# ZYM-PKU/UDiffText

Hardware: AMD Instinct MI355X
Metric: 512x512 50-step denoised images/sec (UDiffText hot path: conditioner + 50 CFG Euler steps + VAE decode) (higher is better)
Workload: dtype bf16; 1 GPU; 512x512, 50 Euler/DDIM(eta 0) steps, CFG 5.0, 9-char labels, noise_iters 0; global batch 4 per step sharded over 1 GPU(s) = 4 images per GPU in micro-batches of 4: every UNet call runs ONE batch of 4 (8 samples with CFG); 3 such batch(es) in flight per GPU on separate launch streams; BASELINE.json configs[1]; global_batch=4, weights=synthetic (name-keyed recipe), 1361.2 M parameters, launch=hipGraph replay of the sampler steps, in_flight=3, batches_per_unet_call=1

## Files before the change

### udifftext_amd/csrc/gemm.hip

```cpp
#include "common.h"
#include <stdio.h>
#include <stdlib.h>
#include <string.h>
#include <atomic>
#include <cmath>

hipError_t udt_lean_launch_gemm(int cfg, const void* lparams, int smem, int G, int geglu, int ln, hipStream_t s);
hipError_t udt_lean_launch_conv3(const void* c3params, hipStream_t s);

namespace {
#include "tile_common.h"

struct GemmParams {
  const uint16_t* a;
  const uint16_t* a2;
  const uint16_t* w;
  const uint16_t* zero;
  const float* bias;
  const uint16_t* res;
  const float* rowvec;
  void* out;
  const float* colscale;
  const float* in_scsh;
  float* colstats;
// ... 587 lines not shown

template <int WGM, int WGN, int TM, int TN, bool GN, bool STATS, bool UPS = false>
hipError_t launch3p(const c3p::CParams& cp, const TilePlan& t, hipStream_t s) {
  constexpr int BN = WGN * TN * 32;
  constexpr int smem = g8::NSTAGE * BN * ROW_BYTES + 2 * c3p::patch_rows(TN, GN) * ROW_BYTES + (GN ? c3p::SCSH_BYTES : 0);
  static_assert(smem <= 160 * 1024, "one workgroup per CU: at most the CU's 160 KiB of LDS");
  static AttrOnce once;
  auto kern = c3p::conv3p_kernel<WGM, WGN, TM, TN, GN, STATS, UPS>;
  hipError_t e = once.ensure(reinterpret_cast<const void*>(kern), smem);
  if (e != hipSuccess) return e;
  hipLaunchKernelGGL(kern, dim3(t.G), dim3(g8::NTHREADS), smem, s, cp);
  return hipGetLastError();
}

struct LeanPlan;
bool lean_stats_probe(const udt_gemm_desc* d, int& rows, int& slots);
int colstats_rows(const udt_gemm_desc* d) {
  if (d->flags & (UDT_GEMM_OUT_F32 | UDT_GEMM_GEGLU | UDT_GEMM_TRANSPOSED)) return 0;
  if ((d->batch > 1) || d->M <= 0 || d->N <= 0 || d->K <= 0 || d->K % BK != 0) return 0;
  int rows = 0, slots = 0;
  if (lean_stats_probe(d, rows, slots)) return rows;
  c3p::Geo ge;
  if (conv3p_geometry(d, ge, d->in_scsh != nullptr)) {
    rows = (d->N % 160 == 0 && d->N % 128 != 0) ? 32 : 64;
    if ((ge.TW * ge.TH) % rows != 0) return 0;
  } else if (use_gemm8(d) && g_rows_epi.load(std::memory_order_relaxed)) {
    rows = (plan_tiles8(d).bn == 160) ? 32 : 64;
  } else {
    return 0;
  }
  const int rpb = d->rows_per_batch > 0 ? d->rows_per_batch : d->M;
  return (rpb % rows == 0) ? rows : 0;
}

int colstats_slots(const udt_gemm_desc* d) {
  const int rows = colstats_rows(d);
  if (rows == 0) return 0;
  int lrows = 0, lslots = 0;
  if (lean_stats_probe(d, lrows, lslots)) return lslots;
  c3p::Geo ge;
  if (conv3p_geometry(d, ge, d->in_scsh != nullptr)) return ge.img_groups * ge.tiles_y * ge.tiles_x * (256 / rows);
  return ((d->M + 255) / 256) * (256 / rows);
}


std::atomic<int> g_lean{-1};
std::atomic<int> g_lean_splitk{-2};
int lean_splitk_knob() {
  int v = g_lean_splitk.load(std::memory_order_relaxed);
  if (v == -2) {
    const char* e = getenv("UDT_LEAN_SPLITK");
    v = e ? atoi(e) : -1;
    g_lean_splitk.store(v, std::memory_order_relaxed);
  }
  return v;
}
std::atomic<int> g_share_splitk{-2};
int share_splitk() {
  int v = g_share_splitk.load(std::memory_order_relaxed);
  if (v == -2) {
    const char* e = getenv("UDT_SHARE_SPLITK");
    v = e ? (atoi(e) != 0) : 1;
    g_share_splitk.store(v, std::memory_order_relaxed);
  }
  return v;
}
int share_of(const udt_gemm_desc* d) { return (share_splitk() && d->cu_share > 1) ? d->cu_share : 1; }
bool lean_stats_enabled() { return true; }

struct LeanPlan {
  int stats_rows = 0;
  int cfg;
  int bm, bn, nw, smem;
  int tiles_m, tiles_n, tiles, nkt, splitk, kt_per, G, n_block;
};

int lean_mode() {
  int v = g_lean.load(std::memory_order_relaxed);
  if (v == -1) {
    const char* e = getenv("UDT_LEAN");
    v = e ? atoi(e) : -2;
    g_lean.store(v, std::memory_order_relaxed);
  }
  return v;
}

std::atomic<int> g_rowres{-2};
bool rowres_on() {
  int v = g_rowres.load(std::memory_order_relaxed);
  if (v == -2) {
    const char* e = getenv("UDT_ROWRES");
    v = e ? (atoi(e) != 0) : 1;
    g_rowres.store(v, std::memory_order_relaxed);
  }
  return v != 0;
}
std::atomic<int> g_lean256_lanes{-2};
bool lean256_under_lanes() {
  int v = g_lean256_lanes.load(std::memory_order_relaxed);
  if (v == -2) {
    const char* e = getenv("UDT_LEAN256_LANES");
    v = e ? (atoi(e) != 0) : 1;
    g_lean256_lanes.store(v, std::memory_order_relaxed);
  }
  return v != 0;
}

std::atomic<int> g_conv_n4{-2};
bool conv_n4_applies(const udt_gemm_desc* d) {
  int v = g_conv_n4.load(std::memory_order_relaxed);
  if (v == -2) {
    const char* e = getenv("UDT_CONV_N4");
    v = e ? (atoi(e) != 0) : 1;
    g_conv_n4.store(v, std::memory_order_relaxed);
  }
  if (!v) return false;
  if (d->flags != (UDT_GEMM_CONV | UDT_GEMM_OUT_F32) || d->ksize != 3 || d->stride != 1 || d->pad_t != 1 || d->pad_l != 1 || d->upsample)
    return false;
  if (d->N != 4 || d->C2 != 0 || d->C1 % 64 != 0 || d->C1 > 512 || d->Hout != d->Hin || d->Wout != d->Win || d->ldo % 4 != 0) return false;
  if (d->residual || d->rowvec || d->in_scsh || d->colstats || d->colscale || d->batch > 1 || d->alpha != 1.0f) return false;
  if ((d->ldw > 0 ? d->ldw : d->K) % 8 != 0 || (d->ldw > 0 && d->ldw < d->K)) return false;
  if (d->K != 9 * d->C1 || (d->lda != 0 && d->lda != d->C1) || d->q8_out || d->q8_scale || d->rowstat_out || d->in_act != 0) return false;
  if ((reinterpret_cast<uintptr_t>(d->a) | reinterpret_cast<uintptr_t>(d->w) | reinterpret_cast<uintptr_t>(d->out)) & 15) return false;
  return true;
}

bool lean_plan(const udt_gemm_desc* d, LeanPlan& t, bool want_stats) {
  const int mode = lean_mode();
  if (mode == 0) return false;
  constexpr int unsupported = UDT_GEMM_OUT_F32 | UDT_GEMM_RELU | UDT_GEMM_TRANSPOSED | UDT_GEMM_SILU_OUT;
  if (d->flags & unsupported) return false;
  const bool conv1 = (d->flags & UDT_GEMM_CONV) != 0;
  if (conv1 && (d->ksize != 1 || d->stride != 1 || d->upsample || d->pad_t != 0 || d->pad_l != 0 || d->Hout != d->Hin ||
                d->Wout != d->Win || d->C1 % BK != 0 || d->C2 % BK != 0 || d->ln_colsum || (d->flags & UDT_GEMM_GEGLU)))
    return false;
  const bool mx8 = (d->flags & UDT_GEMM_MX8) != 0;
  const bool emit = d->q8_out != nullptr;
  if (d->batch > 1 || d->in_scsh || (d->colscale != nullptr) != mx8) return false;
  const bool geglu = (d->flags & UDT_GEMM_GEGLU) != 0;
  const bool ln = d->ln_colsum != nullptr;
  if (want_stats && (geglu || ln || !lean_stats_enabled())) return false;
  if (mx8 || emit) {
    if (conv1 || d->rowvec || mode == 0 || (mode > 0 && mode != 1)) return false;
    if (mx8 && (!d->a_scale || d->K % 128 != 0 || d->lda % 16 != 0 || (d->ldw > 0 && d->ldw % 16 != 0))) return false;
    if (mx8 && ln && (!d->rowstat_in || d->rowstat_in_parts <= 0)) return false;
    if (!mx8 && geglu) return false;
    if (mx8 && geglu && !(ln && emit)) return false;
    if (mx8 && !geglu && ln && emit && d->rowstat_out) return false;
    if (emit && (want_stats || !d->q8_scale || d->ld_q8 % 8 != 0 || d->N % (geglu ? 64 : 32) != 0)) return false;
    if (d->rowstat_out && (!emit || geglu)) return false;
    if (d->q8_fixed_col > 0 && (!emit || geglu || d->q8_fixed_col % 32 != 0 || !(d->q8_fixed_mul > 0.f))) return false;
    if ((reinterpret_cast<uintptr_t>(d->q8_out) | reinterpret_cast<uintptr_t>(d->colscale)) & 15) return false;
  } else if (d->rowstat_out || d->rowstat_in) {
    return false;
  }
  const int KT = mx8 ? 128 : BK;
  if (d->N <= 64 || d->N % 8 != 0 || d->K % KT != 0 || (!conv1 && d->lda % 8 != 0) || (d->ldo % 8 != 0 && d->out)) return false;
  if (d->residual && d->ldr % 8 != 0) return false;
  if (geglu && (d->N % 64 != 0 || d->residual || d->rowvec)) return false;
  const long long ldw = d->ldw > 0 ? d->ldw : d->K;
  const long long lda_eff = conv1 ? (d->C1 > d->C2 ? d->C1 : d->C2) : d->lda;
  if ((long long)d->M * lda_eff * 2 >= (1LL << 31) || (long long)d->N * ldw * 2 >= (1LL << 31)) return false;
  if (d->M >= (1 << 28)) return false;
  if ((reinterpret_cast<uintptr_t>(d->out) | reinterpret_cast<uintptr_t>(d->residual) | reinterpret_cast<uintptr_t>(d->bias) |
       reinterpret_cast<uintptr_t>(d->rowvec) | reinterpret_cast<uintptr_t>(d->ln_colsum)) & 15) return false;
  if (d->rowvec && ((d->ld_rowvec > 0 ? d->ld_rowvec : d->N) % 4 != 0)) return false;
  if (mode > 0 && mode != 1 && mode != 6 && mode != 7) return false;
  if (!mx8 && (!emit || (ln && !geglu && !d->rowstat_out)) && (mode == 7 || (mode < 0 && rowres_on()))) {
    const bool emit_fits = !emit || ((d->q8_fixed_col <= 0 || d->q8_fixed_col % 64 == 0) && (long long)d->M * d->ld_q8 < (1LL << 31) &&
                                     (long long)d->M * (d->out ? d->ldo : 0) * 2 < (1LL << 31) && (long long)((d->N + 127) / 128) * d->M * 4 < (1LL << 31));
    if (ln && !want_stats && d->K == 320 && d->N % 64 == 0 && !d->residual && !d->rowvec && !conv1 && emit_fits &&
        (reinterpret_cast<uintptr_t>(d->a) & 15) == 0) {
      const int tiles_m = (d->M + 255) / 256, chunks = d->N / 64;
      int ns = (device_cus() + tiles_m - 1) / tiles_m;
      if (ns > chunks / 4) ns = chunks / 4;
      const int cmax = geglu ? 20 : 16;
      const int ns_min = (chunks + cmax - 1) / cmax;
      if (ns < ns_min) ns = ns_min;
      const long long wgs = (long long)tiles_m * ns;
      if (ns >= 1 && (mode == 7 || emit || (geglu ? wgs * 4 >= 3LL * device_cus() : wgs >= device_cus()))) {
        t.cfg = 7; t.stats_rows = 0; t.nw = 4; t.bm = 256; t.bn = 64; t.smem = 0;
        t.tiles_m = tiles_m; t.kt_per = (chunks + ns - 1) / ns; t.tiles_n = (chunks + t.kt_per - 1) / t.kt_per;
        t.tiles = t.tiles_m * t.tiles_n; t.nkt = d->K / BK; t.splitk = 1; t.n_block = 1;
        t.G = round_workgroups(t.tiles);
        return true;
      }
    }
    if (mode == 7 || (emit && ln)) return false;
  }
  t.cfg = (mode > 0) ? mode : 1;
  if (!mx8 && !emit) {
  if (!geglu && d->N % 160 == 0 && d->N % 128 != 0 && t.cfg == 1) t.cfg = 5;
  if (mode <= 0 && d->N >= 768 && (long long)((d->M + 255) / 256) * ((d->N + 255) / 256) >= 2LL * device_cus() &&
      (d->cu_share <= 1 || lean256_under_lanes())) t.cfg = 6;
  }
  t.stats_rows = 0;
  if (want_stats) {
    if (t.cfg != 1 && t.cfg != 5) {
      if (mode > 0) return false;
      t.cfg = (d->N % 160 == 0 && d->N % 128 != 0) ? 5 : 1;
    }
    if (mx8) t.cfg = 1;
    t.stats_rows = t.cfg == 1 ? 64 : 32;
    const int rpb = d->rows_per_batch > 0 ? d->rows_per_batch : d->M;
    if (rpb % t.stats_rows != 0) return false;
  }
  switch (t.cfg) {
    case 1: t.nw = 4; t.bm = 128; t.bn = 128; t.smem = 2 * (128 + 128) * ROW_BYTES; break;
    case 5: t.nw = 4; t.bm = 128; t.bn = 160; t.smem = 128 * 160 * 4; break;
    case 6: t.nw = 8; t.bm = 256; t.bn = 256; t.smem = 2 * (256 + 256) * ROW_BYTES; break;
    default: return false;
  }
  {
    const int epi = (t.cfg == 6 ? t.bm * t.bn : t.bm * t.bn * 4) + ((ln && t.cfg != 5) ? t.bm * 8 : 0);
    if (t.smem < epi) t.smem = epi;
  }
  t.tiles_m = (d->M + t.bm - 1) / t.bm;
  t.tiles_n = (d->N + t.bn - 1) / t.bn;
  t.tiles = t.tiles_m * t.tiles_n;
  t.nkt = d->K / KT;
  int slots = device_cus() * ((t.cfg == 1 || t.cfg == 5) ? 2 : 1) / share_of(d);
  if (slots < 1) slots = 1;
  int sk = 1;
  const int knob = lean_splitk_knob();
  if (!ln && t.tiles <= 1023) {
    if (knob > 1) sk = knob;
    else if (knob < 0 && t.tiles * 2 <= slots && t.nkt >= (mx8 ? 20 : 40)) { sk = slots / t.tiles; if (sk > t.nkt / (mx8 ? 8 : 16)) sk = t.nkt / (mx8 ? 8 : 16); }
    if (sk > t.nkt / 4) sk = t.nkt / 4;
    while (sk > 1 && (long long)t.tiles * sk * t.bm * t.bn * 4 > (64LL << 20)) --sk;
    if (sk < 1) sk = 1;
  }
  t.kt_per = (t.nkt + sk - 1) / sk;
  t.splitk = (t.nkt + t.kt_per - 1) / t.kt_per;
  const int units = t.tiles * t.splitk;
  t.G = round_workgroups(units);
  int nb = g_n_block.load(std::memory_order_relaxed);
  if (nb <= 0) nb = (t.tiles_m <= 8) ? t.tiles_n : 8;
  if (nb > t.tiles_n) nb = t.tiles_n;
  t.n_block = nb;
  return true;
}

size_t lean_workspace(const LeanPlan& t) {
  return t.splitk > 1 ? G8_HEADER_BYTES + (size_t)t.tiles * t.splitk * t.bm * t.bn * sizeof(float) : 0;
}

std::atomic<int> g_lean_conv{-1};
std::atomic<int> g_wide_conv{-2};
int wide_conv_mode() {
  int v = g_wide_conv.load(std::memory_order_relaxed);
  if (v == -2) {
    const char* e = getenv("UDT_WIDE_CONV");
    v = e ? atoi(e) : -1;
    g_wide_conv.store(v, std::memory_order_relaxed);
  }
  return v;
}
#ifdef UDT_MEASURE
std::atomic<int> g_lconv_dbg{0};
#endif

std::atomic<int> g_wide_lanes_eff{-2};
double wide_lanes_eff() {
  int v = g_wide_lanes_eff.load(std::memory_order_relaxed);
  if (v == -2) {
    const char* e = getenv("UDT_WIDE_LANES_EFF");
    v = e ? atoi(e) : 70;
    g_wide_lanes_eff.store(v, std::memory_order_relaxed);
  }
  return v / 100.0;
}

int conv_chunk_slices(long long tiles, int slots, int chunks, int knob) {
  long long sk = 1;
  if (tiles <= 1023) {
    if (knob > 1) { sk = knob; if (sk > chunks) sk = chunks; }
    else if (knob < 0 && tiles * 2 <= slots && chunks >= 10) { sk = slots / tiles; if (sk > chunks / 4) sk = chunks / 4; }
    if (sk < 1) sk = 1;
  }
  return (int)sk;
}

bool lean_conv_plan(const udt_gemm_desc* d, lg::C3Params& c, bool want_stats) {
  int on = g_lean_conv.load(std::memory_order_relaxed);
  if (on < 0) {
    const char* e = getenv("UDT_LEAN_CONV");
    on = (e && e[0] == '0') ? 0 : 1;
    g_lean_conv.store(on, std::memory_order_relaxed);
  }
  if (!on || lean_mode() == 0) return false;
  if (d->flags != UDT_GEMM_CONV || d->ksize != 3 || d->stride != 1 || d->pad_t != 1 || d->pad_l != 1) return false;
  if (d->C2 != 0 || d->in_scsh || d->colscale || d->batch > 1) return false;
  if (want_stats && !lean_stats_enabled()) return false;
  if (d->N < 128 || d->N % 8 != 0 || d->C1 <= 0 || d->C1 % 64 != 0) return false;
  if (d->upsample != 0 && d->upsample != 1 && d->upsample != 2) return false;
  const bool phase = d->upsample == 2, ups = d->upsample == 1;
  const int nph = phase ? 4 : 1;
  if (d->Hout != (d->Hin << (d->upsample ? 1 : 0)) || d->Wout != (d->Win << (d->upsample ? 1 : 0))) return false;
  if (phase && d->ldw > 0 && d->ldw < 4 * d->C1) return false;
  const int Ht = phase ? d->Hin : d->Hout, Wt = phase ? d->Win : d->Wout;
  c.bn = 128; c.wgm = 2;
  bool wide = false;
  int wide_slots = device_cus();
  {
    const int wm = wide_conv_mode();
    if (wm != 0 && !ups && d->N % 160 == 0 && Wt % 16 == 0 && Ht % 16 == 0) {
      const int cus = device_cus(), share = d->cu_share > 1 ? d->cu_share : 1;
      wide_slots = cus / share > 0 ? cus / share : 1;
      const long long wt = (long long)(d->M / 256) * (d->N / 160);
      const long long sk = conv_chunk_slices(wt, wide_slots, d->C1 / 64, lean_splitk_knob());
      const long long units = wt * sk;
      const long long rounds = (units + cus - 1) / cus;
      const double eff = units > cus ? (double)units / (double)(rounds * cus) : ((double)units * share >= cus ? 1.0 : (double)units * share / cus);
      wide = (wm > 0) || (sk <= 2 && eff >= ((share >= 3 && share_of(d) >= 3) ? wide_lanes_eff() : 0.85));
    }
  }
  if (wide) { c.geo = phase ? 6 : 3; c.tw = 16; c.th = 16; c.bn = 160; c.wgm = 4; }
  else if (Wt % 16 == 0 && Ht % 8 == 0) { c.geo = ups ? 2 : phase ? 4 : 0; c.tw = 16; c.th = 8; }
  else if (!ups && Wt % 8 == 0 && Ht % 8 == 0) { c.geo = phase ? 5 : 1; c.tw = 8; c.th = 8; }
  else return false;
  if (d->ldo % 8 != 0 || (d->residual && d->ldr % 8 != 0)) return false;
  const long long ldw = d->ldw > 0 ? d->ldw : (phase ? 4LL * d->C1 : (long long)d->K);
  if (ldw % 8 != 0) return false;
  c.w_phase = phase ? (d->stride_w > 0 ? d->stride_w : (long long)d->N * ldw) : 0;
  if (phase && (c.w_phase < (long long)d->N * ldw || c.w_phase % 8 != 0)) return false;
  if ((long long)d->M * d->C1 * 2 >= (1LL << 31) || (long long)d->N * ldw * 2 >= (1LL << 31)) return false;
  if ((reinterpret_cast<uintptr_t>(d->out) | reinterpret_cast<uintptr_t>(d->residual) | reinterpret_cast<uintptr_t>(d->bias) |
       reinterpret_cast<uintptr_t>(d->rowvec)) & 15) return false;
  if (d->rowvec && ((d->ld_rowvec > 0 ? d->ld_rowvec : d->N) % 4 != 0)) return false;
  c.dbg = 0;
#ifdef UDT_MEASURE
  c.dbg = g_lconv_dbg.load(std::memory_order_relaxed);
#endif
  c.N = d->N; c.C = d->C1; c.H = d->Hin; c.W = d->Win; c.B = d->M / (d->Hout * d->Wout);
  c.ldw = (int)ldw; c.ldo = d->ldo; c.ldr = d->ldr; c.ldrv = d->ld_rowvec > 0 ? d->ld_rowvec : d->N;
  c.alpha = d->alpha;
  c.tiles_x = Wt / c.tw; c.tiles_y = Ht / c.th;
  c.tiles_m = c.B * c.tiles_x * c.tiles_y;
  c.tiles_n = (d->N + c.bn - 1) / c.bn;
  c.tiles = c.tiles_m * c.tiles_n;
  c.chunks = c.C / 64;
  const int slots = wide ? wide_slots : (2 * device_cus() / share_of(d) > 0 ? 2 * device_cus() / share_of(d) : 1);
  int sk = conv_chunk_slices((long long)c.tiles * nph, slots, c.chunks, lean_splitk_knob());
  while (sk > 1 && (long long)c.tiles * nph * sk * c.tw * c.th * c.bn * 4 > (64LL << 20)) --sk;
  c.ch_per = (c.chunks + sk - 1) / sk;
  c.splitk = (c.chunks + c.ch_per - 1) / c.ch_per;
  c.G = round_workgroups(c.tiles * nph * c.splitk);
  {
    const double patch = (double)((ups ? c.tw / 2 : c.tw) + 2) * ((ups ? c.th / 2 : c.th) + 2) * c.C * 2.0, wtile = (phase ? 4.0 : 9.0) * c.bn * c.C * 2.0;
    int nb = g_n_block.load(std::memory_order_relaxed);
    if (nb <= 0) nb = (int)(std::sqrt(64.0 * patch / wtile) + 0.5);
    if (nb < 1) nb = 1;
    if (nb > c.tiles_n) nb = c.tiles_n;
    c.n_block = nb;
  }
  c.a_bytes = (unsigned)((long long)c.B * d->Hin * d->Win * d->C1 * 2);
  c.w_bytes = (unsigned)((long long)d->N * ldw * 2);
  c.counters = nullptr; c.slabs = nullptr;
  return true;
}

int lean_conv_phases(const lg::C3Params& c) { return c.geo >= 4 ? 4 : 1; }

size_t lean_conv_workspace(const lg::C3Params& c) {
  return c.splitk > 1 ? G8_HEADER_BYTES + (size_t)c.tiles * lean_conv_phases(c) * c.splitk * c.tw * c.th * c.bn * sizeof(float) : 0;
}

bool lean_stats_probe(const udt_gemm_desc* d, int& rows, int& slots) {
  if (d->in_scsh) return false;
  {
    lg::C3Params c3;
    if (lean_conv_plan(d, c3, true)) {
      rows = c3.tw * c3.th / c3.wgm;
      slots = c3.tiles_m * c3.wgm * lean_conv_phases(c3);
      return true;
    }
  }
  if ((d->flags & UDT_GEMM_CONV) && d->ksize == 3) return false;
  LeanPlan lt;
  if (lean_plan(d, lt, true)) {
    rows = lt.stats_rows;
    slots = lt.tiles_m * (lt.bm / lt.stats_rows);
    return true;
  }
  return false;
}
}

extern "C" int udt_debug_set(const char* key, int32_t value) {
  if (!key) return UDT_ERR_BAD_ARG;
  if (!strcmp(key, "n_block")) { g_n_block.store(value); return UDT_OK; }
  if (!strcmp(key, "rows_epi")) { g_rows_epi.store(value ? 1 : 0); return UDT_OK; }
  if (!strcmp(key, "lean")) { g_lean.store(value < 0 ? -2 : value); return UDT_OK; }
  if (!strcmp(key, "rowres")) { g_rowres.store(value < 0 ? 1 : (value ? 1 : 0)); return UDT_OK; }
  if (!strcmp(key, "wide_lanes_eff")) { g_wide_lanes_eff.store(value < 0 ? -2 : value); return UDT_OK; }
  if (!strcmp(key, "conv_n4")) { g_conv_n4.store(value < 0 ? -2 : (value ? 1 : 0)); return UDT_OK; }
  if (!strcmp(key, "lean256_lanes")) { g_lean256_lanes.store(value < 0 ? -2 : (value ? 1 : 0)); return UDT_OK; }
  if (!strcmp(key, "lean_splitk")) { g_lean_splitk.store(value); return UDT_OK; }
  if (!strcmp(key, "share_splitk")) { g_share_splitk.store(value < 0 ? -2 : (value ? 1 : 0)); return UDT_OK; }
  if (!strcmp(key, "lean_conv")) { g_lean_conv.store(value < 0 ? -1 : (value ? 1 : 0)); return UDT_OK; }
  if (!strcmp(key, "wide_conv")) { g_wide_conv.store(value < 0 ? -1 : (value ? 1 : 0)); return UDT_OK; }
#ifdef UDT_MEASURE
  if (!strcmp(key, "lconv_dbg")) { g_lconv_dbg.store(value); return UDT_OK; }
  static const struct { const char* k; int bit; } bits[] = {{"no_xchg", 28}, {"no_epi", 27}, {"no_store", 26}, {"no_res", 25},
                                                            {"no_bias", 24}, {"no_fast", 22}};
  for (const auto& b : bits)
    if (!strcmp(key, b.k)) {
      int cur = g_dbg_bits.load();
      g_dbg_bits.store((cur & ~(1 << b.bit)) | (value ? (1 << b.bit) : 0));
      return UDT_OK;
    }
#endif
  return UDT_ERR_BAD_ARG;
}

extern "C" int udt_check_async_error(void* workspace, size_t workspace_bytes, void* stream) {
  if (!workspace || workspace_bytes < G8_HEADER_BYTES) return UDT_ERR_BAD_ARG;
  hipStream_t s = reinterpret_cast<hipStream_t>(stream);
  int err = 0;
  hipError_t e = hipMemcpyAsync(&err, reinterpret_cast<int*>(workspace) + 1023, sizeof(int), hipMemcpyDeviceToHost, s);
  if (e == hipSuccess) e = hipStreamSynchronize(s);
  if (e != hipSuccess) return udt_set_hip_error(e);
  if (err == 0) return UDT_OK;
  e = hipMemsetAsync(workspace, 0, G8_HEADER_BYTES, s);
  if (e == hipSuccess) e = hipStreamSynchronize(s);
  if (e != hipSuccess) return udt_set_hip_error(e);
  return UDT_ERR_ASYNC;
}

extern "C" int32_t udt_gemm_colstats_rows(const udt_gemm_desc* d) { return d ? colstats_rows(d) : 0; }
extern "C" int32_t udt_gemm_colstats_slots(const udt_gemm_desc* d) { return d ? colstats_slots(d) : 0; }
extern "C" int32_t udt_gemm_q8_ok(const udt_gemm_desc* d) {
  if (!d || !d->q8_out || d->M <= 0 || d->N <= 0 || d->K <= 0) return 0;
  LeanPlan lt;
  return lean_plan(d, lt, d->colstats != nullptr) ? 1 : 0;
}

extern "C" int32_t udt_gemm_rowstat_parts(const udt_gemm_desc* d) {
  if (!d || d->M <= 0 || d->N <= 0 || d->K <= 0) return 0;
  udt_gemm_desc t = *d;
  alignas(16) static const uint64_t probe_dst[2] = {0, 0};
  if (!t.q8_out) { t.q8_out = const_cast<uint64_t*>(probe_dst); t.q8_scale = const_cast<uint64_t*>(probe_dst); if (t.ld_q8 <= 0) t.ld_q8 = (t.N + 15) / 16 * 16; }
  LeanPlan lt;
  if (!lean_plan(&t, lt, false) || lt.cfg != 1 || (d->flags & UDT_GEMM_GEGLU)) return 0;
  return (d->N + 63) / 64;
}
extern "C" int32_t udt_gemm_in_scsh_ok(const udt_gemm_desc* d) {
  if (!d || d->K <= 0 || d->K % BK != 0) return 0;
  c3p::Geo ge;
  return conv3p_geometry(d, ge, true) ? 1 : 0;
}

extern "C" int32_t udt_gemm_up4_ok(const udt_gemm_desc* d) {
  if (!d || d->upsample != 2) return 0;
  lg::C3Params c3;
  return lean_conv_plan(d, c3, d->colstats != nullptr) ? 1 : 0;
}

extern "C" int udt_gn_silu_conv3x3_fwd(const udt_gemm_desc* d, void* workspace, size_t workspace_bytes, void* stream) {
  if (!d || !(d->flags & UDT_GEMM_CONV) || d->ksize != 3 || d->stride != 1 || d->pad_t != 1 || d->pad_l != 1 || !d->in_scsh)
    return UDT_ERR_BAD_ARG;
  return udt_gemm(d, workspace, workspace_bytes, stream);
}

extern "C" int udt_ln_gemm_fwd(const udt_gemm_desc* d, void* workspace, size_t workspace_bytes, void* stream) {
  if (!d || !d->ln_colsum || !d->bias || !(d->ln_eps > 0.f)) return UDT_ERR_BAD_ARG;
  LeanPlan lt;
  if (!lean_plan(d, lt, false)) return UDT_ERR_BAD_SHAPE;
  return udt_gemm(d, workspace, workspace_bytes, stream);
}

extern "C" size_t udt_gemm_workspace_bytes(const udt_gemm_desc* d) {
  if (!d || d->K <= 0 || d->M <= 0 || d->N <= 0 || d->K % k_tile(d) != 0) return 0;
  if (conv_n4_applies(d)) return 0;
  {
    LeanPlan lt;
    if (lean_plan(d, lt, d->colstats != nullptr)) return lean_workspace(lt);
    lg::C3Params c3;
    if (lean_conv_plan(d, c3, d->colstats != nullptr)) return lean_conv_workspace(c3);
  }
  {
    c3p::Geo ge;
    if (conv3p_geometry(d, ge, d->in_scsh != nullptr)) {
      TilePlan t3 = plan_tiles3p(d, ge);
      if (!t3.fixup) return 0;
      return G8_HEADER_BYTES + (size_t)t3.G * t3.bm * t3.bn * sizeof(float);
    }
  }
  if (use_gemm8(d)) {
    TilePlan t8 = plan_tiles8(d);
    if (!t8.fixup) return 0;
    return G8_HEADER_BYTES + (size_t)t8.G * t8.bm * t8.bn * sizeof(float);
  }
  TilePlan t = plan_tiles(d);
  if (t.bm != 256 || !t.fixup) return 0;
  return G8_HEADER_BYTES + (size_t)t.G * 2 * SLAB_FLOATS * sizeof(float);
}

extern "C" int udt_gemm(const udt_gemm_desc* d, void* workspace, size_t workspace_bytes, void* stream) {
  if (!d || !d->a || !d->w) return UDT_ERR_BAD_ARG;
  if (d->M <= 0 || d->N <= 0 || d->K <= 0) return UDT_ERR_BAD_SHAPE;
  if (d->K % k_tile(d) != 0) return UDT_ERR_BAD_SHAPE;
  if (d->N % 4 != 0) return UDT_ERR_BAD_SHAPE;
  const bool mx8 = (d->flags & UDT_GEMM_MX8) != 0;
  if (mx8 || d->q8_out || d->rowstat_out || d->rowstat_in) {
    LeanPlan lt8;
    if (!lean_plan(d, lt8, d->colstats != nullptr)) return UDT_ERR_BAD_ARG;
  } else if (d->colscale) {
    return UDT_ERR_BAD_ARG;
  }
  const bool conv = (d->flags & UDT_GEMM_CONV) != 0;
  const bool trans = (d->flags & UDT_GEMM_TRANSPOSED) != 0;
  const int batch = d->batch > 0 ? d->batch : 1;
  if (conv) {
    if (d->ksize != 1 && d->ksize != 3) return UDT_ERR_BAD_SHAPE;
    if (d->C1 <= 0 || d->C1 % BK != 0 || d->C2 % BK != 0) return UDT_ERR_BAD_SHAPE;
    if (d->C2 > 0 && !d->a2) return UDT_ERR_BAD_ARG;
    if (d->K != d->ksize * d->ksize * (d->C1 + d->C2)) return UDT_ERR_BAD_SHAPE;
    if (d->Hout <= 0 || d->Wout <= 0 || d->M % (d->Hout * d->Wout) != 0) return UDT_ERR_BAD_SHAPE;
    if (d->stride != 1 && d->stride != 2) return UDT_ERR_BAD_SHAPE;
    if (trans || batch != 1) return UDT_ERR_BAD_ARG;
  } else {
    if (d->lda < d->K || d->lda % 8 != 0) return UDT_ERR_BAD_SHAPE;
  }
  if (!d->out && !d->q8_out) return UDT_ERR_BAD_ARG;
  if (trans) {
    if (d->rows_per_batch <= 0 || d->rows_per_batch % 4 != 0 || d->M % d->rows_per_batch != 0)
      return UDT_ERR_BAD_SHAPE;
    if (d->flags & (UDT_GEMM_OUT_F32 | UDT_GEMM_GEGLU | UDT_GEMM_RELU | UDT_GEMM_SILU_OUT)) return UDT_ERR_BAD_ARG;
    if (d->residual || d->rowvec || batch != 1) return UDT_ERR_BAD_ARG;
  } else {
    if (d->ldo % 4 != 0) return UDT_ERR_BAD_SHAPE;
    if (d->residual && d->ldr % 4 != 0) return UDT_ERR_BAD_SHAPE;
  }
  if (d->flags & UDT_GEMM_GEGLU) {
    if (d->N % 64 != 0 || (d->flags & UDT_GEMM_OUT_F32) || d->residual || d->rowvec) return UDT_ERR_BAD_ARG;
  }
  if (d->rowvec && d->rows_per_batch <= 0) return UDT_ERR_BAD_ARG;

  hipStream_t s = reinterpret_cast<hipStream_t>(stream);
  if (conv_n4_applies(d)) {
    cn4::Params cp;
    cp.a = reinterpret_cast<const uint16_t*>(d->a); cp.w = reinterpret_cast<const uint16_t*>(d->w); cp.bias = d->bias;
    cp.out = reinterpret_cast<float*>(d->out);
    cp.B = d->M / (d->Hout * d->Wout); cp.H = d->Hin; cp.W = d->Win; cp.C = d->C1;
    cp.ldw = d->ldw > 0 ? d->ldw : d->K; cp.ldo = d->ldo;
    cp.tiles_x = (d->Win + 7) / 8; cp.tiles_y = (d->Hin + 7) / 8;
    const size_t smem = (size_t)100 * (d->C1 + 8) * 2 + (size_t)4 * 9 * d->C1 * 2;
    static AttrOnce once;
    hipError_t ea = once.ensure(reinterpret_cast<const void*>(cn4::conv3x3_n4_kernel), 100 * (512 + 8) * 2 + 4 * 9 * 512 * 2);
    if (ea != hipSuccess) return udt_set_hip_error(ea);
    UdtProfScope profn(0, s);
    if (profn.rec) {
      char tag[96];
      snprintf(tag, sizeof(tag), "conv_n4 M=%d N=%d K=%d %dx%d", d->M, d->N, d->K, d->Hin, d->Win);
      udt_prof_tag(profn.rec, tag);
    }
    hipLaunchKernelGGL(cn4::conv3x3_n4_kernel, dim3((unsigned)(cp.B * cp.tiles_x * cp.tiles_y)), dim3(256), smem, s, cp);
    UDT_CHECK_LAUNCH();
    return UDT_OK;
  }
  TilePlan t = plan_tiles(d);

  GemmParams p;
  p.a = reinterpret_cast<const uint16_t*>(d->a);
  p.a2 = reinterpret_cast<const uint16_t*>(d->a2);
  p.w = reinterpret_cast<const uint16_t*>(d->w);
  p.zero = udt_zero_page();
  if (!p.zero) return UDT_ERR_HIP;
  p.bias = d->bias;
  p.res = reinterpret_cast<const uint16_t*>(d->residual);
  p.rowvec = d->rowvec;
  p.out = d->out;
  p.colscale = d->colscale;
  p.in_scsh = d->in_scsh;
  p.in_act = d->in_act;
  p.colstats = d->colstats;
  p.slabs = nullptr;
  if (d->colstats && colstats_rows(d) == 0) return UDT_ERR_BAD_ARG;
  if (d->in_scsh && !udt_gemm_in_scsh_ok(d)) return UDT_ERR_BAD_ARG;
  if (d->in_act != 0 && d->in_act != 1) return UDT_ERR_BAD_ARG;
  p.M = d->M; p.N = d->N; p.K = d->K;
  p.lda = d->lda; p.ldo = d->ldo; p.ldr = d->ldr;
  p.ldw = d->ldw > 0 ? d->ldw : d->K;
  if (d->upsample == 2) {
    if (!udt_gemm_up4_ok(d)) return UDT_ERR_BAD_SHAPE;
  } else if (p.ldw < d->K || p.ldw % 8 != 0) return UDT_ERR_BAD_SHAPE;
  if (mx8 && d->lda < d->K) return UDT_ERR_BAD_SHAPE;
  p.sA = d->stride_a; p.sW = d->stride_w; p.sO = d->stride_out; p.sR = d->stride_res;
  p.Hin = d->Hin; p.Win = d->Win; p.C1 = d->C1; p.C2 = d->C2; p.Hout = d->Hout; p.Wout = d->Wout;
  p.ksz = d->ksize; p.stride = d->stride; p.pad_t = d->pad_t; p.pad_l = d->pad_l; p.ups = d->upsample ? 1 : 0;
  p.rows_per_batch = d->rows_per_batch > 0 ? d->rows_per_batch : d->M;
  p.ldrv = d->ld_rowvec > 0 ? d->ld_rowvec : d->N;
// ... 206 lines not shown
```

### udifftext_amd/csrc/lean.h

```cpp
#pragma once

namespace lg {

using g8::wait_vm;
UDT_DEVINL void raw_barrier() {
  asm volatile("s_waitcnt lgkmcnt(0)" ::: "memory");
  __builtin_amdgcn_s_barrier();
  asm volatile("" ::: "memory");
}
using g8::buf_lds16;
using g8::OOB;

typedef __attribute__((ext_vector_type(2))) __bf16 bf2_t;
UDT_DEVINL float dot2_bf16(uint32_t a, uint32_t b, float c) {
  return __builtin_amdgcn_fdot2_f32_bf16(__builtin_bit_cast(bf2_t, a), __builtin_bit_cast(bf2_t, b), c, false);
}

template <int CPR, int RPI>
UDT_DEVINL void wave_colstats(char* wl, int lane, const float (&cs)[8], const float (&cq)[8], float* dst, bool col_ok) {
#pragma unroll
  for (int h = 0; h < 2; ++h) {
    f32x4 a = {cs[4 * h + 0], cs[4 * h + 1], cs[4 * h + 2], cs[4 * h + 3]};
    f32x4 b = {cq[4 * h + 0], cq[4 * h + 1], cq[4 * h + 2], cq[4 * h + 3]};
    *reinterpret_cast<f32x4*>(wl + lane * 64 + h * 16) = a;
    *reinterpret_cast<f32x4*>(wl + lane * 64 + 32 + h * 16) = b;
  }
  asm volatile("s_waitcnt lgkmcnt(0)" ::: "memory");
  if (lane < CPR && col_ok) {
    float ts[8], tq[8];
#pragma unroll
    for (int j = 0; j < 8; ++j) ts[j] = tq[j] = 0.f;
#pragma unroll
    for (int r = 0; r < RPI; ++r) {
      const char* src = wl + (r * CPR + lane) * 64;
#pragma unroll
      for (int h = 0; h < 2; ++h) {
        const f32x4 a = *reinterpret_cast<const f32x4*>(src + h * 16);
        const f32x4 b = *reinterpret_cast<const f32x4*>(src + 32 + h * 16);
#pragma unroll
        for (int e = 0; e < 4; ++e) { ts[4 * h + e] += a[e]; tq[4 * h + e] += b[e]; }
      }
    }
#pragma unroll
    for (int h = 0; h < 4; ++h) {
      f32x4 v = {ts[2 * h], tq[2 * h], ts[2 * h + 1], tq[2 * h + 1]};
      *reinterpret_cast<f32x4*>(dst + h * 4) = v;
    }
  }
}

template <int NW, int WGM, int WGN, int TM, int TN, int NST, bool GEGLU, bool LN, int TMB = TM, bool STATS = false, bool FP8 = false,
          bool EMIT = false>
__global__ void __launch_bounds__(NW * 64, 2) lgemm_kernel(const LParams p) {
  static_assert(!STATS || (!GEGLU && !LN), "statistics-emitting epilogue: plain linears / 1x1 convolutions");
  static_assert(!FP8 || NST == 2, "the fp8 loop is written for the two-stage ring");
  static_assert(!EMIT || (TN * 4) % 4 == 0, "a 32-column block = 4 lanes of the row layout");
  constexpr int EB = FP8 ? 1 : 2;
  static_assert(TM % TMB == 0, "epilogue passes of TMB row tiles");
  static_assert(WGM * WGN == NW, "wave grid");
  static_assert(!GEGLU || TN == 2, "GEGLU pairs the two 32-column tiles of a wave");
  constexpr int BM = WGM * TM * 32, BN = WGN * TN * 32;
  constexpr int A_BYTES = BM * ROW_BYTES, B_BYTES = BN * ROW_BYTES, STAGE_BYTES = A_BYTES + B_BYTES;
  constexpr int A_PIECES = BM / 8, B_PIECES = BN / 8;
  constexpr int A_INSTR = (A_PIECES + NW - 1) / NW, B_INSTR = (B_PIECES + NW - 1) / NW;
  constexpr int LPT = A_INSTR + B_INSTR;
  constexpr int WROWS = TM * 32, WCOLS = TN * 32;
  constexpr int EROW = WCOLS * 4;
  constexpr int EPI_WAVE = TMB * 32 * EROW;
  extern __shared__ __attribute__((aligned(16))) char smem[];

  const int tid = threadIdx.x;
  const int wave = __builtin_amdgcn_readfirstlane(tid >> 6);
  const int lane = tid & 63;
  const int l31 = lane & 31;
  const int hi = lane >> 5;
  const int l3 = lane >> 3;
  const int pslot = lane & 7;
  const int wm = wave / WGN;
  const int wn = wave - wm * WGN;
  const int row0 = wm * WROWS;
  const int col0 = wn * WCOLS;
  const int swz = (l31 >> 1) & 7;

  const int unit = range_index(blockIdx.x, p.G);
  if (unit >= p.tiles * p.splitk) return;
  const int tile = unit / p.splitk;
  const int slice = unit - tile * p.splitk;
  int m0, n0;
  {
    const int per_block = p.tiles_m * p.n_block;
    const int blk = tile / per_block;
    const int r = tile - blk * per_block;
    int nbw = p.tiles_n - blk * p.n_block;
    if (nbw > p.n_block) nbw = p.n_block;
    const int tmi = r / nbw;
    m0 = tmi * BM;
    n0 = (blk * p.n_block + (r - tmi * nbw)) * BN;
  }
  const int kt0 = slice * p.kt_per;
  int kt1 = kt0 + p.kt_per;
  if (kt1 > p.nkt) kt1 = p.nkt;
  const int nk = kt1 - kt0;
  auto kreal = [&](int i) { return kt0 + i; };
  const __amdgpu_buffer_rsrc_t rsrc_a = __builtin_amdgcn_make_buffer_rsrc(const_cast<uint16_t*>(p.a), 0, p.a_bytes, 0x00020000);
  const __amdgpu_buffer_rsrc_t rsrc_w = __builtin_amdgcn_make_buffer_rsrc(const_cast<uint16_t*>(p.w), 0, p.w_bytes, 0x00020000);
  const __amdgpu_buffer_rsrc_t rsrc_a2 =
      __builtin_amdgcn_make_buffer_rsrc(const_cast<uint16_t*>(p.a2 ? p.a2 : p.a), 0, p.a2 ? p.a2_bytes : 0u, 0x00020000);
  unsigned a_voff[A_INSTR], a2_voff[A_INSTR], w_voff[B_INSTR];
  int a_piece[A_INSTR], w_piece[B_INSTR];
#pragma unroll
  for (int i = 0; i < A_INSTR; ++i) {
    int idx = wave + NW * i;
    while (idx >= A_PIECES) idx -= NW;
    a_piece[i] = idx;
    const int row = idx * 8 + l3;
    const int koff = (pslot ^ ((row >> 1) & 7)) * 8;
    const int m = m0 + row;
    a_voff[i] = (m < p.M) ? (unsigned)((long long)m * p.lda * EB + koff * 2) : OOB;
    a2_voff[i] = (m < p.M) ? (unsigned)(((long long)m * p.lda2 + koff) * 2) : OOB;
  }
#pragma unroll
  for (int i = 0; i < B_INSTR; ++i) {
    int idx = wave + NW * i;
    while (idx >= B_PIECES) idx -= NW;
    w_piece[i] = idx;
    const int row = idx * 8 + l3;
    const int koff = (pslot ^ ((row >> 1) & 7)) * 8;
    const int n = n0 + row;
    w_voff[i] = (n < p.N) ? (unsigned)((long long)n * p.ldw * EB + koff * 2) : OOB;
  }
  auto stage = [&](int st, int kt) {
    char* abuf = smem + st * STAGE_BYTES;
    char* bbuf = abuf + A_BYTES;
    if (kt < p.kt_split) {
#pragma unroll
      for (int i = 0; i < A_INSTR; ++i) buf_lds16(rsrc_a, abuf + a_piece[i] * 1024, a_voff[i], kt * ROW_BYTES);
    } else {
#pragma unroll
      for (int i = 0; i < A_INSTR; ++i) buf_lds16(rsrc_a2, abuf + a_piece[i] * 1024, a2_voff[i], (kt - p.kt_split) * ROW_BYTES);
    }
#pragma unroll
    for (int i = 0; i < B_INSTR; ++i) buf_lds16(rsrc_w, bbuf + w_piece[i] * 1024, w_voff[i], kt * ROW_BYTES);
  };

#pragma unroll
  for (int s = 0; s < NST - 1; ++s)
    if (s < nk) stage(s, kreal(s));
  const uint32_t* asp[TM];
  uint32_t asc_nxt[TM];
  if constexpr (FP8) {
#pragma unroll
    for (int tm = 0; tm < TM; ++tm) {
      int m = m0 + row0 + tm * 32 + l31;
      if (m >= p.M) m = p.M - 1;
      asp[tm] = p.a_scale + m;
      asc_nxt[tm] = (nk > 0) ? asp[tm][(long long)kreal(0) * p.M] : 0x7f7f7f7fu;
    }
  }

  f32x16 acc[TM][TN];
#pragma unroll
  for (int i = 0; i < TM; ++i)
#pragma unroll
    for (int j = 0; j < TN; ++j)
#pragma unroll
      for (int r = 0; r < 16; ++r) acc[i][j][r] = 0.f;
  float rs[TM], rq[TM];
#pragma unroll
  for (int i = 0; i < TM; ++i) rs[i] = rq[i] = 0.f;
  if constexpr (LN && FP8) {
    if (WGN == 1 || wn == 0) {
#pragma unroll
      for (int tm = 0; tm < TM; ++tm) {
        int m = m0 + row0 + tm * 32 + l31;
        if (m >= p.M) m = p.M - 1;
        const f32x2* sp = reinterpret_cast<const f32x2*>(p.rowstat_in) + m;
        for (int pp = hi; pp < p.rowstat_in_parts; pp += 2) {
          const f32x2 v = sp[(long long)pp * p.M];
          rs[tm] += v[0];
          rq[tm] += v[1];
        }
      }
    }
  }

  const int a_frag_row = (row0 + l31) * ROW_BYTES;
  const int b_frag_row = (col0 + l31) * ROW_BYTES;
  int st = 0;
  for (int kt = 0; kt < nk; ++kt) {
    if (NST > 2 && kt + NST - 2 < nk) wait_vm<LPT*(NST > 2 ? NST - 2 : 0)>();
    else wait_vm<0>();
    raw_barrier();
    int asc[TM];
    if constexpr (FP8) {
#pragma unroll
      for (int tm = 0; tm < TM; ++tm) asc[tm] = (int)(asc_nxt[tm] >> (8 * hi));
    }
    if (kt + NST - 1 < nk) {
      int s2 = st + NST - 1;
      if (s2 >= NST) s2 -= NST;
      const int kn = kreal(kt + NST - 1);
      stage(s2, kn);
      if constexpr (FP8) {
#pragma unroll
        for (int tm = 0; tm < TM; ++tm) asc_nxt[tm] = asp[tm][(long long)kn * p.M];
      }
    }
    const char* abuf = smem + st * STAGE_BYTES;
    const char* bbuf = abuf + A_BYTES;
    if constexpr (FP8) {
      i32x8_t xf[2][TM], wf[2][TN];
#pragma unroll
      for (int ks = 0; ks < 2; ++ks) {
        const int slot0 = ((ks * 4 + hi) ^ swz) << 4, slot1 = ((ks * 4 + 2 + hi) ^ swz) << 4;
#pragma unroll
        for (int t = 0; t < TM; ++t)
          xf[ks][t] = lds_read_frag32(abuf + a_frag_row + t * 32 * ROW_BYTES + slot0, abuf + a_frag_row + t * 32 * ROW_BYTES + slot1);
#pragma unroll
        for (int t = 0; t < TN; ++t)
          wf[ks][t] = lds_read_frag32(bbuf + b_frag_row + t * 32 * ROW_BYTES + slot0, bbuf + b_frag_row + t * 32 * ROW_BYTES + slot1);
      }
#pragma unroll
      for (int tm = 0; tm < TM; ++tm)
#pragma unroll
        for (int tn = 0; tn < TN; ++tn) acc[tm][tn] = mfma32_mx8<0>(wf[0][tn], xf[0][tm], acc[tm][tn], asc[tm]);
#pragma unroll
      for (int tm = 0; tm < TM; ++tm)
#pragma unroll
        for (int tn = 0; tn < TN; ++tn) acc[tm][tn] = mfma32_mx8<2>(wf[1][tn], xf[1][tm], acc[tm][tn], asc[tm]);
      if constexpr (TM * TN <= 5) {
        __builtin_amdgcn_sched_group_barrier(0x100, 4 * (TM + TN), 0);
        __builtin_amdgcn_sched_group_barrier(0x008, 2 * TM * TN, 0);
      }
    } else {
    bf16x8_t xf[4][TM], wf[4][TN];
#pragma unroll
    for (int ks = 0; ks < 4; ++ks) {
      const int slot = ((ks * 2 + hi) ^ swz) << 4;
#pragma unroll
      for (int t = 0; t < TM; ++t) xf[ks][t] = lds_read_frag(abuf + a_frag_row + t * 32 * ROW_BYTES + slot);
#pragma unroll
      for (int t = 0; t < TN; ++t) wf[ks][t] = lds_read_frag(bbuf + b_frag_row + t * 32 * ROW_BYTES + slot);
    }
#pragma unroll
    for (int ks = 0; ks < 4; ++ks) {
#pragma unroll
      for (int tm = 0; tm < TM; ++tm)
#pragma unroll
        for (int tn = 0; tn < TN; ++tn) acc[tm][tn] = mfma32(wf[ks][tn], xf[ks][tm], acc[tm][tn]);
      if constexpr (LN) {
        if (wn == 0) {
#pragma unroll
          for (int tm = 0; tm < TM; ++tm) {
            const u32x4 v = __builtin_bit_cast(u32x4, xf[ks][tm]);
#pragma unroll
            for (int j = 0; j < 4; ++j) {
              rs[tm] = dot2_bf16(v[j], 0x3f803f80u, rs[tm]);
              rq[tm] = dot2_bf16(v[j], v[j], rq[tm]);
            }
          }
        }
      }
    }
    if constexpr (TM * TN <= 5) {
      __builtin_amdgcn_sched_group_barrier(0x100, 4 * (TM + TN), 0);
      __builtin_amdgcn_sched_group_barrier(0x008, 4 * TM * TN, 0);
    }
    }
    st = st + 1;
    if (st >= NST) st = 0;
  }
  raw_barrier();

  if (p.splitk > 1) {
    f32x4* slab = reinterpret_cast<f32x4*>(p.slabs + (long long)unit * (BM * BN));
#pragma unroll
    for (int tm = 0; tm < TM; ++tm)
#pragma unroll
      for (int tn = 0; tn < TN; ++tn)
#pragma unroll
        for (int q = 0; q < 4; ++q) {
          f32x4 v = {acc[tm][tn][q * 4 + 0], acc[tm][tn][q * 4 + 1], acc[tm][tn][q * 4 + 2], acc[tm][tn][q * 4 + 3]};
          store16_sc1(slab + ((tm * TN + tn) * 4 + q) * (NW * 64) + tid, v);
        }
    asm volatile("s_waitcnt vmcnt(0)" ::: "memory");
    __syncthreads();
    int* const bcast = reinterpret_cast<int*>(smem);
    if (tid == 0) {
      const int t = __hip_atomic_fetch_add(p.counters + tile, 1, __ATOMIC_RELAXED, __HIP_MEMORY_SCOPE_AGENT);
      const int last = (t == p.splitk - 1) ? 1 : 0;
      if (last) {
        __builtin_amdgcn_fence(__ATOMIC_ACQUIRE, "agent");
        __hip_atomic_store(p.counters + tile, 0, __ATOMIC_RELAXED, __HIP_MEMORY_SCOPE_AGENT);
      }
      *bcast = last;
    }
    __syncthreads();
    const bool last = *bcast != 0;
    __syncthreads();
    if (!last) return;
#pragma unroll
    for (int i = 0; i < TM; ++i)
#pragma unroll
      for (int j = 0; j < TN; ++j)
#pragma unroll
        for (int r = 0; r < 16; ++r) acc[i][j][r] = 0.f;
    for (int s = 0; s < p.splitk; ++s) {
      const f32x4* sl = reinterpret_cast<const f32x4*>(p.slabs + ((long long)tile * p.splitk + s) * (BM * BN));
#pragma unroll
      for (int tm = 0; tm < TM; ++tm)
#pragma unroll
        for (int tn = 0; tn < TN; ++tn)
#pragma unroll
          for (int q = 0; q < 4; ++q) {
            const f32x4 v = sl[((tm * TN + tn) * 4 + q) * (NW * 64) + tid];
#pragma unroll
            for (int r = 0; r < 4; ++r) acc[tm][tn][q * 4 + r] += v[r];
          }
    }
  }

  float ln_mean[TM], ln_rstd[TM];
#pragma unroll
  for (int tm = 0; tm < TM; ++tm) ln_mean[tm] = 0.f, ln_rstd[tm] = 1.f;
  if constexpr (LN) {
    float* const rst = reinterpret_cast<float*>(smem + NW * EPI_WAVE);
    if (WGN == 1 || wn == 0) {
#pragma unroll
      for (int tm = 0; tm < TM; ++tm) {
        const float s = xor32_sum(rs[tm]), q = xor32_sum(rq[tm]);
        const float mean = s / (float)p.K;
        const float var = fmaxf(q / (float)p.K - mean * mean, 0.f);
        ln_mean[tm] = mean;
        ln_rstd[tm] = __builtin_amdgcn_rsqf(var + p.ln_eps);
        if constexpr (WGN > 1) {
          if (hi == 0) {
            f32x2 o = {ln_mean[tm], ln_rstd[tm]};
            *reinterpret_cast<f32x2*>(rst + (row0 + tm * 32 + l31) * 2) = o;
          }
        }
      }
    }
    if constexpr (WGN > 1) __syncthreads();
  }
  auto row_stats = [&](int row, float& mean, float& rstd) {
    if constexpr (WGN == 1) {
      mean = __shfl(ln_mean[0], row & 31);
      rstd = __shfl(ln_rstd[0], row & 31);
#pragma unroll
      for (int tm = 1; tm < TM; ++tm) {
        const float m2 = __shfl(ln_mean[tm], row & 31), r2 = __shfl(ln_rstd[tm], row & 31);
        if ((row >> 5) == tm) mean = m2, rstd = r2;
      }
    } else {
      const f32x2 ms = *reinterpret_cast<const f32x2*>(reinterpret_cast<const float*>(smem + NW * EPI_WAVE) + (row0 + row) * 2);
      mean = ms[0];
      rstd = ms[1];
    }
  };

  if constexpr (GEGLU) {
    if constexpr (LN && WGN > 1) {
      if (wn != 0) {
        const float* rst = reinterpret_cast<const float*>(smem + NW * EPI_WAVE);
#pragma unroll
        for (int tm = 0; tm < TM; ++tm) {
          const f32x2 ms = *reinterpret_cast<const f32x2*>(rst + (row0 + tm * 32 + l31) * 2);
          ln_mean[tm] = ms[0];
          ln_rstd[tm] = ms[1];
        }
      }
    }
    char* const wb = smem + wave * (WROWS * 64);
#pragma unroll
    for (int q = 0; q < 4; ++q) {
      const int n = n0 + col0 + q * 8 + hi * 4;
      f32x4 bx = {0.f, 0.f, 0.f, 0.f}, bg = bx, sx = bx, sg = bx;
      f32x4 wx = {1.f, 1.f, 1.f, 1.f}, wg = wx;
      if (n < p.N) {
        if constexpr (FP8) {
          wx = *reinterpret_cast<const f32x4*>(p.colscale + n);
          wg = *reinterpret_cast<const f32x4*>(p.colscale + n + 32);
        }
        if (p.bias) {
          bx = *reinterpret_cast<const f32x4*>(p.bias + n);
          bg = *reinterpret_cast<const f32x4*>(p.bias + n + 32);
        }
        if constexpr (LN) {
          sx = *reinterpret_cast<const f32x4*>(p.ln_s + n);
          sg = *reinterpret_cast<const f32x4*>(p.ln_s + n + 32);
        }
      }
#pragma unroll
      for (int r = 0; r < 4; ++r) bx[r] *= GEGLU_XS, bg[r] *= GEGLU_GS;
#pragma unroll
      for (int tm = 0; tm < TM; ++tm) {
        const int row = tm * 32 + l31;
        const float xm = ln_rstd[tm] * p.alpha * GEGLU_XS, gm = ln_rstd[tm] * p.alpha * GEGLU_GS;
        const float xa = -ln_mean[tm] * xm, ga = -ln_mean[tm] * gm;
        float o[4];
#pragma unroll
        for (int r = 0; r < 4; ++r) {
          float x, g;
// ... 21 lines not shown
      const int m = m0 + row0 + row;
      const u32x4 v = *reinterpret_cast<const u32x4*>(wb + row * 64 + ((ch ^ (row & 3)) << 4));
      if constexpr (EMIT) {
        const float f[8] = {bf16_lo(v[0]), bf16_hi(v[0]), bf16_lo(v[1]), bf16_hi(v[1]), bf16_lo(v[2]), bf16_hi(v[2]), bf16_lo(v[3]), bf16_hi(v[3])};
        uint32_t sb;
        const u32x2 q8 = mx8_quant_row8(f, sb);
        if (m < p.M && col_ok) {
          *reinterpret_cast<u32x2*>(p.q8_out + (long long)m * p.ld_q8 + n_out) = q8;
          if (ch == 0) reinterpret_cast<uint8_t*>(p.q8_scale)[((long long)(n_out >> 7) * p.M + m) * 4 + ((n_out >> 5) & 3)] = (uint8_t)sb;
          if (p.out) *reinterpret_cast<u32x4*>(p.out + (long long)m * p.ldo + n_out) = v;
        }
      } else {
        if (m < p.M && col_ok) *reinterpret_cast<u32x4*>(p.out + (long long)m * p.ldo + n_out) = v;
      }
    }
  } else {
    char* const wl = smem + wave * EPI_WAVE;
    constexpr int PROWS = TMB * 32;
    constexpr int CPR = TN * 4;
    constexpr int RPI = 64 / CPR;
    constexpr int NIT = (PROWS + RPI - 1) / RPI;
    const int rl = lane / CPR;
    const int c8 = lane - rl * CPR;
    const int n = n0 + col0 + c8 * 8;
    const bool col_ok = (rl < RPI) && (n < p.N);
    f32x4 b0 = {0.f, 0.f, 0.f, 0.f}, b1 = b0, s0 = b0, s1 = b0;
    if (p.bias && col_ok) {
      b0 = *reinterpret_cast<const f32x4*>(p.bias + n);
      b1 = *reinterpret_cast<const f32x4*>(p.bias + n + 4);
    }
    if constexpr (LN) {
      if (col_ok) {
        s0 = *reinterpret_cast<const f32x4*>(p.ln_s + n);
        s1 = *reinterpret_cast<const f32x4*>(p.ln_s + n + 4);
      }
    }
    f32x4 w0 = {1.f, 1.f, 1.f, 1.f}, w1 = w0;
    if constexpr (FP8) {
      if (col_ok) {
        w0 = *reinterpret_cast<const f32x4*>(p.colscale + n);
        w1 = *reinterpret_cast<const f32x4*>(p.colscale + n + 4);
      }
    }
    float cs[8], cq[8];
#pragma unroll
    for (int j = 0; j < 8; ++j) cs[j] = cq[j] = 0.f;
#pragma unroll
    for (int pass = 0; pass < TM / TMB; ++pass) {
      const int prow0 = pass * PROWS;
      u32x4 rv[NIT];
      if (p.res) {
#pragma unroll
        for (int i = 0; i < NIT; ++i) {
          const int row = i * RPI + rl;
          const int m = m0 + row0 + prow0 + row;
          u32x4 z = {0u, 0u, 0u, 0u};
          rv[i] = z;
          if (col_ok && row < PROWS && m < p.M) rv[i] = *reinterpret_cast<const u32x4*>(p.res + (long long)m * p.ldr + n);
        }
      }
#pragma unroll
      for (int tb = 0; tb < TMB; ++tb) {
        const int row = tb * 32 + l31;
#pragma unroll
        for (int tn = 0; tn < TN; ++tn)
#pragma unroll
          for (int q = 0; q < 4; ++q) {
            const int chunk = (tn * 8 + q * 2 + hi) ^ (row & 7);
            const f32x16& a16 = acc[pass * TMB + tb][tn];
            f32x4 v = {a16[q * 4 + 0], a16[q * 4 + 1], a16[q * 4 + 2], a16[q * 4 + 3]};
            *reinterpret_cast<f32x4*>(wl + row * EROW + chunk * 16) = v;
          }
      }
#pragma unroll
      for (int i = 0; i < NIT; ++i) {
        const int row = i * RPI + rl;
        const int m = m0 + row0 + prow0 + row;
        const bool ok = col_ok && row < PROWS && m < p.M;
        const int rr = row < PROWS ? row : 0;
        const char* rp = wl + rr * EROW;
        const int sw = rr & 7;
        const f32x4 v0 = *reinterpret_cast<const f32x4*>(rp + (((2 * c8) ^ sw) << 4));
        const f32x4 v1 = *reinterpret_cast<const f32x4*>(rp + (((2 * c8 + 1) ^ sw) << 4));
        float o[8];
#pragma unroll
        for (int j = 0; j < 4; ++j) {
          o[j] = v0[j];
          o[4 + j] = v1[j];
        }
        if constexpr (FP8) {
#pragma unroll
          for (int j = 0; j < 4; ++j) o[j] *= w0[j], o[4 + j] *= w1[j];
        }
        if constexpr (LN) {
          float mean, rstd;
          row_stats(prow0 + rr, mean, rstd);
#pragma unroll
          for (int j = 0; j < 4; ++j) {
            o[j] = rstd * (o[j] - mean * s0[j]);
            o[4 + j] = rstd * (o[4 + j] - mean * s1[j]);
          }
        }
#pragma unroll
        for (int j = 0; j < 4; ++j) {
          o[j] = o[j] * p.alpha + b0[j];
          o[4 + j] = o[4 + j] * p.alpha + b1[j];
        }
        if (p.rowvec && ok) {
          const float* rvp = p.rowvec + (long long)(m / p.rows_per_batch) * p.ldrv + n;
          const f32x4 r0 = *reinterpret_cast<const f32x4*>(rvp);
          const f32x4 r1 = *reinterpret_cast<const f32x4*>(rvp + 4);
#pragma unroll
          for (int j = 0; j < 4; ++j) {
            o[j] += r0[j];
            o[4 + j] += r1[j];
          }
        }
        if (p.res) {
#pragma unroll
          for (int j = 0; j < 4; ++j) {
            o[2 * j] += bf16_lo(rv[i][j]);
            o[2 * j + 1] += bf16_hi(rv[i][j]);
          }
        }
        if constexpr (EMIT) {
          {
            const u32x4 rb = {pack_bf16x2(o[0], o[1]), pack_bf16x2(o[2], o[3]), pack_bf16x2(o[4], o[5]), pack_bf16x2(o[6], o[7])};
#pragma unroll
            for (int j = 0; j < 4; ++j) o[2 * j] = bf16_lo(rb[j]), o[2 * j + 1] = bf16_hi(rb[j]);
          }
          uint32_t sb;
          u32x2 q8 = mx8_quant_row8(o, sb);
          if (n >= p.q8_fixed_col) {
            q8 = e4m3_fixed_row8(o, p.q8_fixed_mul);
            sb = 127u;
          }
          float ps = 0.f, pq = 0.f;
          if (p.rowstat_out) {
            static_assert(CPR == 8 || CPR == 16, "row statistics: 64- or 128-column wave blocks");
#pragma unroll
            for (int j = 0; j < 8; ++j) ps += o[j], pq += o[j] * o[j];
            ps = dpp_add<0xB1>(ps); pq = dpp_add<0xB1>(pq);
            ps = dpp_add<0x4E>(ps); pq = dpp_add<0x4E>(pq);
            ps = dpp_add<0x141>(ps); pq = dpp_add<0x141>(pq);
            if constexpr (CPR == 16) { ps = dpp_add<0x140>(ps); pq = dpp_add<0x140>(pq); }
          }
          if (ok) {
            *reinterpret_cast<u32x2*>(p.q8_out + (long long)m * p.ld_q8 + n) = q8;
            if ((c8 & 3) == 0) reinterpret_cast<uint8_t*>(p.q8_scale)[((long long)(n >> 7) * p.M + m) * 4 + ((n >> 5) & 3)] = (uint8_t)sb;
            if (p.rowstat_out && c8 == 0) {
              f32x2 st2 = {ps, pq};
              reinterpret_cast<f32x2*>(p.rowstat_out)[(long long)((n0 + col0) / WCOLS) * p.M + m] = st2;
            }
          }
        }
        if (ok) {
          u32x4 pk = {pack_bf16x2(o[0], o[1]), pack_bf16x2(o[2], o[3]), pack_bf16x2(o[4], o[5]), pack_bf16x2(o[6], o[7])};
          if (!EMIT || p.out) *reinterpret_cast<u32x4*>(p.out + (long long)m * p.ldo + n) = pk;
          if constexpr (STATS) {
#pragma unroll
            for (int j = 0; j < 4; ++j) {
              const float a = bf16_lo(pk[j]), bb = bf16_hi(pk[j]);
              cs[2 * j] += a; cq[2 * j] += a * a;
              cs[2 * j + 1] += bb; cq[2 * j + 1] += bb * bb;
            }
          }
        }
      }
    }
    if constexpr (STATS) {
      const int slot = (m0 + row0) / WROWS;
      wave_colstats<CPR, RPI>(wl, lane, cs, cq, p.colstats + ((long long)slot * p.N + n) * 2, col_ok);
    }
  }
}


template <int MAXN>
UDT_DEVINL void wait_vm_upto(int n) {
  if constexpr (MAXN == 0) wait_vm<0>();
  else {
    if (n >= MAXN) wait_vm<MAXN>();
    else wait_vm_upto<MAXN - 1>(n);
  }
}

template <int TW, int TH, bool UPS>
struct C3Geo {
  static constexpr int PX = TW * TH;
  static constexpr int TM = PX / 64;
  static constexpr int PW = (UPS ? TW / 2 : TW) + 2, PH = (UPS ? TH / 2 : TH) + 2;
  static constexpr int PROWS = PW * PH;
  static constexpr int PIECES = (PROWS + 7) / 8;
  static constexpr int PATCH_BYTES = PIECES * 1024;
  static constexpr int W_BYTES = 128 * ROW_BYTES;
  static constexpr int NRING = (3 * W_BYTES + 2 * PATCH_BYTES <= 80 * 1024) ? 3 : 2;
  static constexpr int RING = NRING * W_BYTES + 2 * PATCH_BYTES;
  static constexpr int STAGING = 4 * TM * 32 * 256;
  static constexpr int SMEM = RING > STAGING ? RING : STAGING;
  static_assert(PX == 128 || PX == 64, "128 or 64 output pixels per workgroup");
  static_assert(SMEM <= 80 * 1024, "two workgroups per CU");
};

template <int TW, int TH, bool UPS, bool STATS = false, bool PHASE = false>
__global__ void __launch_bounds__(256, 2) lconv3_kernel(const C3Params p) {
  static_assert(!(UPS && PHASE), "the phase form runs on the low-resolution geometries");
  using Geo = C3Geo<TW, TH, UPS>;
  constexpr int NT = PHASE ? 4 : 9;
  constexpr int NW = 4, TM = Geo::TM, TN = 2, BN = 128, BMPX = Geo::PX;
  constexpr int C3_PW = Geo::PW, C3_PROWS = Geo::PROWS, C3_PIECES = Geo::PIECES, C3_PATCH_BYTES = Geo::PATCH_BYTES;
  constexpr int C3_W_BYTES = Geo::W_BYTES, C3_TW = TW, C3_TH = TH;
  constexpr int WROWS = TM * 32;
  constexpr int WP = 4;
  constexpr int PP = (C3_PIECES + NW - 1) / NW;
  constexpr int EROW = 64 * 4;
  extern __shared__ __attribute__((aligned(16))) char smem[];
  char* const wring = smem;
  constexpr int NR = Geo::NRING;
  char* const patches = smem + NR * C3_W_BYTES;

  const int tid = threadIdx.x;
  const int wave = __builtin_amdgcn_readfirstlane(tid >> 6);
  const int lane = tid & 63;
  const int l31 = lane & 31;
  const int hi = lane >> 5;
  const int l3 = lane >> 3;
  const int pslot = lane & 7;
  const int wm = wave >> 1, wn = wave & 1;
  const int row0 = wm * WROWS, col0 = wn * 64;
  const int swz_w = (l31 >> 1) & 7;
  const int w_frag_row = (col0 + l31) * ROW_BYTES;

  const int unit = range_index(blockIdx.x, p.G);
  if (unit >= p.tiles * p.splitk * (PHASE ? 4 : 1)) return;
  const int phase = PHASE ? unit / (p.tiles * p.splitk) : 0;
  const int pha = phase >> 1, phb = phase & 1;
  const int ptile = unit / p.splitk;
  const int slice = unit - ptile * p.splitk;
  const int tile = ptile - phase * p.tiles;
  int tile_m, n0;
  {
    const int per_block = p.tiles_m * p.n_block;
    const int blk = tile / per_block;
    const int r = tile - blk * per_block;
    int nbw = p.tiles_n - blk * p.n_block;
    if (nbw > p.n_block) nbw = p.n_block;
    tile_m = r / nbw;
    n0 = (blk * p.n_block + (r - tile_m * nbw)) * BN;
  }
  const int per_img = p.tiles_x * p.tiles_y;
  const int b = tile_m / per_img;
  const int rt = tile_m - b * per_img;
  const int ty = rt / p.tiles_x;
  const int y0 = ty * C3_TH, x0 = (rt - ty * p.tiles_x) * C3_TW;
  const int c0 = slice * p.ch_per;
  int c1 = c0 + p.ch_per;
  if (c1 > p.chunks) c1 = p.chunks;

  const __amdgpu_buffer_rsrc_t rsrc_a = __builtin_amdgcn_make_buffer_rsrc(const_cast<uint16_t*>(p.a), 0, p.a_bytes, 0x00020000);
  const __amdgpu_buffer_rsrc_t rsrc_w =
      __builtin_amdgcn_make_buffer_rsrc(const_cast<uint16_t*>(p.w) + (PHASE ? (long long)phase * p.w_phase : 0LL), 0, p.w_bytes, 0x00020000);
  auto patch_swz = [](int prow, int yy) { return ((prow - 2 * yy) >> 1) & 7; };
  unsigned w_voff[WP], p_voff[PP];
  int p_piece[PP];
#pragma unroll
  for (int i = 0; i < WP; ++i) {
    const int row = (wave + NW * i) * 8 + l3;
    const int kw = (pslot ^ ((row >> 1) & 7)) * 8;
    const int n = n0 + row;
    w_voff[i] = (n < p.N) ? (unsigned)(((long long)n * p.ldw + kw) * 2) : OOB;
  }
#pragma unroll
  for (int i = 0; i < PP; ++i) {
    int idx = wave + NW * i;
    while (idx >= C3_PIECES) idx -= NW;
    p_piece[i] = idx;
    const int prow = idx * 8 + l3;
    const int yy = prow / C3_PW;
    const int xx = prow - yy * C3_PW;
    const int gy = (UPS ? (y0 >> 1) : y0) + yy - 1, gx = (UPS ? (x0 >> 1) : x0) + xx - 1;
    const bool ok = (prow < C3_PROWS) && ((unsigned)gy < (unsigned)p.H) && ((unsigned)gx < (unsigned)p.W);
    const int koff = (pslot ^ patch_swz(prow, yy)) * 8;
    p_voff[i] = ok ? (unsigned)(((((long long)b * p.H + gy) * p.W + gx) * p.C + koff) * 2) : OOB;
  }
  int a_prow[TM], a_py[TM];
#pragma unroll
  for (int tm = 0; tm < TM; ++tm) {
    const int ml = row0 + tm * 32 + l31;
    const int py = ml / TW, px = ml - py * TW;
    a_py[tm] = PHASE ? py + pha : py;
    a_prow[tm] = UPS ? (py | (px << 16)) : PHASE ? ((py + pha) * C3_PW + px + phb) : (py * C3_PW + px);
  }
  auto issue_w = [&](int st, int c, int tap) {
    const int soff = (tap * p.C + c * 64) * 2;
    char* wbuf = wring + st * C3_W_BYTES;
#pragma unroll
    for (int i = 0; i < WP; ++i) buf_lds16(rsrc_w, wbuf + (wave + NW * i) * 1024, w_voff[i], soff);
  };
  auto issue_patch = [&](int c) {
    char* pbuf = patches + (c & 1) * C3_PATCH_BYTES;
#pragma unroll
    for (int i = 0; i < PP; ++i) buf_lds16(rsrc_a, pbuf + p_piece[i] * 1024, p_voff[i], c * 128);
  };

  f32x16 acc[TM][TN];
#pragma unroll
// ... 217 lines not shown
```

### udifftext_amd/csrc/lean.hip

```cpp
#include "common.h"
#include <stdio.h>
#include <stdlib.h>
#include <atomic>

namespace {
#include "tile_common.h"
#include "lean_params.h"
#include "lean.h"
#include "wide.h"
#include "rowres.h"

template <int NW, int WGM, int WGN, int TM, int TN, int NST, int TMB = TM>
hipError_t launch_lean(const lg::LParams& lp, int smem, int G, bool geglu, bool ln, hipStream_t s) {
  static AttrOnce once[5];
  const void* fn;
  const bool stats = lp.colstats != nullptr;
  if constexpr (NW == 4 && NST == 2) {
    if (stats) {
      fn = (const void*)lg::lgemm_kernel<NW, WGM, WGN, TM, TN, NST, false, false, TMB, true>;
      hipError_t e = once[4].ensure(fn, smem);
      if (e != hipSuccess) return e;
      void* args[] = {const_cast<lg::LParams*>(&lp)};
      return hipLaunchKernel(fn, dim3(G), dim3(NW * 64), args, smem, s);
    }
  }
  if (stats) return hipErrorInvalidValue;
  if constexpr (TN == 2) {
    fn = geglu ? (ln ? (const void*)lg::lgemm_kernel<NW, WGM, WGN, TM, TN, NST, true, true, TMB> : (const void*)lg::lgemm_kernel<NW, WGM, WGN, TM, TN, NST, true, false, TMB>)
               : (ln ? (const void*)lg::lgemm_kernel<NW, WGM, WGN, TM, TN, NST, false, true, TMB> : (const void*)lg::lgemm_kernel<NW, WGM, WGN, TM, TN, NST, false, false, TMB>);
  } else {
    fn = ln ? (const void*)lg::lgemm_kernel<NW, WGM, WGN, TM, TN, NST, false, true, TMB> : (const void*)lg::lgemm_kernel<NW, WGM, WGN, TM, TN, NST, false, false, TMB>;
  }
  hipError_t e = once[(geglu ? 2 : 0) + (ln ? 1 : 0)].ensure(fn, smem);
  if (e != hipSuccess) return e;
  void* args[] = {const_cast<lg::LParams*>(&lp)};
  return hipLaunchKernel(fn, dim3(G), dim3(NW * 64), args, smem, s);
}

template <bool GEGLU, bool LN, bool STATS, bool FP8, bool EMIT>
hipError_t launch_lean_mx8_k(const lg::LParams& lp, int smem, int G, hipStream_t s) {
  static AttrOnce once;
  const void* fn = (const void*)lg::lgemm_kernel<4, 2, 2, 2, 2, 2, GEGLU, LN, 2, STATS, FP8, EMIT>;
  hipError_t e = once.ensure(fn, smem);
  if (e != hipSuccess) return e;
  void* args[] = {const_cast<lg::LParams*>(&lp)};
  return hipLaunchKernel(fn, dim3(G), dim3(256), args, smem, s);
}
hipError_t launch_lean_mx8(const lg::LParams& lp, int smem, int G, bool geglu, bool ln, bool fp8, bool emit, hipStream_t s) {
  const bool stats = lp.colstats != nullptr;
  if (!fp8) {
    if (emit && !geglu && !ln && !stats) return launch_lean_mx8_k<false, false, false, false, true>(lp, smem, G, s);
    return hipErrorInvalidValue;
  }
  if (geglu) return (ln && emit && !stats) ? launch_lean_mx8_k<true, true, false, true, true>(lp, smem, G, s) : hipErrorInvalidValue;
  if (ln) return stats ? hipErrorInvalidValue
                 : emit ? launch_lean_mx8_k<false, true, false, true, true>(lp, smem, G, s)
                        : launch_lean_mx8_k<false, true, false, true, false>(lp, smem, G, s);
  if (stats) return emit ? hipErrorInvalidValue : launch_lean_mx8_k<false, false, true, true, false>(lp, smem, G, s);
  return emit ? launch_lean_mx8_k<false, false, false, true, true>(lp, smem, G, s) : launch_lean_mx8_k<false, false, false, true, false>(lp, smem, G, s);
}

template <int TW, int TH, bool UPS, bool STATS, bool PHASE>
hipError_t launch_lconv3s(const lg::C3Params& c3, hipStream_t s) {
  static AttrOnce once;
  constexpr int smem = lg::C3Geo<TW, TH, UPS>::SMEM;
  hipError_t e = once.ensure(reinterpret_cast<const void*>(lg::lconv3_kernel<TW, TH, UPS, STATS, PHASE>), smem);
  if (e != hipSuccess) return e;
  hipLaunchKernelGGL((lg::lconv3_kernel<TW, TH, UPS, STATS, PHASE>), dim3(c3.G), dim3(256), smem, s, c3);
  return hipGetLastError();
}
template <int TW, int TH, bool UPS, bool PHASE = false>
hipError_t launch_lconv3(const lg::C3Params& c3, hipStream_t s) {
  return c3.colstats ? launch_lconv3s<TW, TH, UPS, true, PHASE>(c3, s) : launch_lconv3s<TW, TH, UPS, false, PHASE>(c3, s);
}

template <bool STATS, bool PHASE>
hipError_t launch_wconv3s(const lg::C3Params& c3, hipStream_t s) {
  static AttrOnce once;
  constexpr int smem = wd::WGeo::SMEM;
  hipError_t e = once.ensure(reinterpret_cast<const void*>(wd::wconv3_kernel<STATS, PHASE>), smem);
  if (e != hipSuccess) return e;
  hipLaunchKernelGGL((wd::wconv3_kernel<STATS, PHASE>), dim3(c3.G), dim3(256), smem, s, c3);
  return hipGetLastError();
}
template <int KT, bool GEGLU, bool EMIT = false>
hipError_t launch_rowres(const lg::LParams& lp, int G, hipStream_t s) {
  static AttrOnce once;
  constexpr int smem = rr::RGeo<KT, GEGLU>::SMEM;
  hipError_t e = once.ensure(reinterpret_cast<const void*>(rr::rgemm_kernel<KT, GEGLU, EMIT>), smem);
  if (e != hipSuccess) return e;
  hipLaunchKernelGGL((rr::rgemm_kernel<KT, GEGLU, EMIT>), dim3(G), dim3(256), smem, s, lp);
  return hipGetLastError();
}

template <bool PHASE>
hipError_t launch_wconv3(const lg::C3Params& c3, hipStream_t s) {
  return c3.colstats ? launch_wconv3s<true, PHASE>(c3, s) : launch_wconv3s<false, PHASE>(c3, s);
}

}

hipError_t udt_lean_launch_gemm(int cfg, const void* lparams, int smem, int G, int geglu, int ln, hipStream_t s) {
  const lg::LParams& lp = *static_cast<const lg::LParams*>(lparams);
  const bool fp8 = lp.a_scale != nullptr, emit = lp.q8_out != nullptr;
  if (cfg == 7 && emit && !fp8 && !geglu && ln && lp.K == 320) return launch_rowres<5, false, true>(lp, G, s);
  if (fp8 || emit) return cfg == 1 ? launch_lean_mx8(lp, smem, G, geglu != 0, ln != 0, fp8, emit, s) : hipErrorInvalidValue;
  switch (cfg) {
    case 1: return launch_lean<4, 2, 2, 2, 2, 2>(lp, smem, G, geglu != 0, ln != 0, s);
    case 6: return launch_lean<8, 2, 4, 4, 2, 2, 1>(lp, smem, G, geglu != 0, ln != 0, s);
    case 5: return geglu ? hipErrorInvalidValue : launch_lean<4, 4, 1, 1, 5, 2>(lp, smem, G, false, ln != 0, s);
    case 7:
      if (!ln || lp.K != 320) return hipErrorInvalidValue;
      return geglu ? launch_rowres<5, true>(lp, G, s) : launch_rowres<5, false>(lp, G, s);
    default: return hipErrorInvalidValue;
  }
}

hipError_t udt_lean_launch_conv3(const void* c3params, hipStream_t s) {
  const lg::C3Params& c3 = *static_cast<const lg::C3Params*>(c3params);
  return c3.geo == 3 ? launch_wconv3<false>(c3, s) : c3.geo == 6 ? launch_wconv3<true>(c3, s) : c3.geo == 2 ? launch_lconv3<16, 8, true>(c3, s)
         : c3.geo == 4 ? launch_lconv3<16, 8, false, true>(c3, s) : c3.geo == 5 ? launch_lconv3<8, 8, false, true>(c3, s)
         : c3.geo == 1 ? launch_lconv3<8, 8, false>(c3, s) : launch_lconv3<16, 8, false>(c3, s);
}
```

### udifftext_amd/csrc/tattn.hip

```cpp
#include "common.h"
#include <stdio.h>
#include <stdlib.h>

namespace {

constexpr int TA_THREADS = 512;
constexpr int TA_WAVES = TA_THREADS / 64;

struct TattnParams {
  const uint16_t* x;
  uint16_t* out;
  const uint16_t* A;
  const float* sc;
  const uint16_t* BmT;
  const float* bias;
  const uint16_t* zero;
  int M, C, hp, n_tok, zero_samples;
  int nsplit;
  float eps;
  uint8_t* q8_out;
  uint32_t* q8_scale;
  float* rowstat_out;
};

UDT_DEVINL f32x16 zero16() {
  f32x16 z;
#pragma unroll
  for (int r = 0; r < 16; ++r) z[r] = 0.f;
  return z;
}

template <int TT, int NKT, int NKS, bool Q8 = false>
__global__ void __launch_bounds__(TA_THREADS) tattn_fused_kernel(const TattnParams p) {
  extern __shared__ __attribute__((aligned(16))) char smem[];
  constexpr int C = NKT * 64, hp = NKS * 16;
  constexpr int nkt = NKT;
  constexpr int TA_AHEAD = NKT <= 10 ? NKT : 8;
  char* const xs = smem;
  float* const stats = reinterpret_cast<float*>(smem + (size_t)nkt * TT * 128);
  const int prs = hp * 2 + 16;
  char* const pl = reinterpret_cast<char*>(stats + TT * 2);
  const int tid = threadIdx.x;
  const int wave = __builtin_amdgcn_readfirstlane(tid >> 6);
  const int lane = tid & 63;
  const int l31 = lane & 31, hi = lane >> 5;
  const long long tok0 = (long long)blockIdx.x * TT;
  const int b = (int)(tok0 / p.n_tok);
  const uint16_t* xg = p.x + tok0 * C;
  uint16_t* og = p.out + tok0 * C;
  float* const rst = reinterpret_cast<float*>(pl + (size_t)TT * prs);
  const int ct_lo = (int)blockIdx.y * (C >> 5) / p.nsplit, ct_hi = ((int)blockIdx.y + 1) * (C >> 5) / p.nsplit;
  auto q8_row_stats = [&]() {
    __syncthreads();
    if (tid < TT && tok0 + tid < p.M) {
      float s = 0.f, q = 0.f;
      for (int ct = ct_lo; ct < ct_hi; ++ct) {
        const f32x2 v = *reinterpret_cast<const f32x2*>(rst + ((size_t)tid * (C >> 5) + ct) * 2);
        s += v[0];
        q += v[1];
      }
      f32x2 o = {s, q};
      reinterpret_cast<f32x2*>(p.rowstat_out)[(long long)blockIdx.y * p.M + tok0 + tid] = o;
    }
  };


  const uint16_t* Ab = p.A + (long long)b * hp * C;
  constexpr int jt = hp >> 5;
  constexpr int tiles1 = jt * (TT / 32);
  bf16x8_t ar[TA_AHEAD][4];
  const bool live = b >= p.zero_samples;
  if (live && wave < tiles1) {
    const uint16_t* arow = Ab + (long long)(wave / (TT / 32)) * (32 * C) + lane * 8;
#pragma unroll
    for (int u = 0; u < TA_AHEAD; ++u)
#pragma unroll
      for (int ks = 0; ks < 4; ++ks) ar[u][ks] = *reinterpret_cast<const bf16x8_t*>(arow + (u * 4 + ks) * 512);
  }

  {
    const int pieces = nkt * (TT / 8);
    const int l3 = lane >> 3, ps = lane & 7;
    for (int pc = wave; pc < pieces; pc += TA_WAVES) {
      const int kt = pc / (TT / 8), rg = pc - kt * (TT / 8);
      const int row = rg * 8 + l3;
      const int slot = ps ^ ((row >> 1) & 7);
      const uint16_t* src = (tok0 + row < p.M) ? (xg + (long long)row * C + kt * 64 + slot * 8) : p.zero;
      glds16(src, xs + (size_t)pc * 1024);
    }
    wait_vmcnt0();
  }
  __syncthreads();

  if (b < p.zero_samples) {
    const int ch_lo = ct_lo * 4, ch_hi = ct_hi * 4;
    const int nch = ch_hi - ch_lo;
    for (int i0 = 0; i0 < TT * nch; i0 += TA_THREADS) {
      const int i = i0 + tid;
      const bool act = i < TT * nch;
      const int row = act ? i / nch : 0, ch = ch_lo + (act ? i - row * nch : 0);
      const bool ok = act && tok0 + row < p.M;
      const int kt = ch >> 3, s = ch & 7;
      const u32x4 v = *reinterpret_cast<const u32x4*>(xs + ((size_t)kt * TT + row) * 128 + ((s ^ ((row >> 1) & 7)) << 4));
      const f32x4 b0 = *reinterpret_cast<const f32x4*>(p.bias + ch * 8), b1 = *reinterpret_cast<const f32x4*>(p.bias + ch * 8 + 4);
      const float f[8] = {bf16_lo(v[0]) + b0[0], bf16_hi(v[0]) + b0[1], bf16_lo(v[1]) + b0[2], bf16_hi(v[1]) + b0[3],
                          bf16_lo(v[2]) + b1[0], bf16_hi(v[2]) + b1[1], bf16_lo(v[3]) + b1[2], bf16_hi(v[3]) + b1[3]};
      u32x4 o = {pack_bf16x2(f[0], f[1]), pack_bf16x2(f[2], f[3]), pack_bf16x2(f[4], f[5]), pack_bf16x2(f[6], f[7])};
      if (ok) *reinterpret_cast<u32x4*>(og + (long long)row * C + ch * 8) = o;
      if constexpr (Q8) {
        uint32_t sb;
        const u32x2 q8 = mx8_quant_row8(f, sb);
        float ps = 0.f, pq = 0.f;
#pragma unroll
        for (int j = 0; j < 8; ++j) ps += f[j], pq += f[j] * f[j];
        ps = dpp_add<0xB1>(ps); pq = dpp_add<0xB1>(pq);
        ps = dpp_add<0x4E>(ps); pq = dpp_add<0x4E>(pq);
        if (ok) {
          const long long m = tok0 + row;
          *reinterpret_cast<u32x2*>(p.q8_out + m * C + ch * 8) = q8;
          if ((ch & 3) == 0) {
            reinterpret_cast<uint8_t*>(p.q8_scale)[((long long)(ch >> 4) * p.M + m) * 4 + ((ch >> 2) & 3)] = (uint8_t)sb;
            f32x2 st2 = {ps, pq};
            *reinterpret_cast<f32x2*>(rst + ((size_t)row * (C >> 5) + (ch >> 2)) * 2) = st2;
          }
        }
      }
    }
    if constexpr (Q8) q8_row_stats();
    return;
  }

  {
    constexpr int TPR = TA_THREADS / TT;
    const int row = tid / TPR, part = tid - row * TPR;
    const int swz = (row >> 1) & 7;
    float s = 0.f, q = 0.f;
    for (int ch = part; ch < nkt * 8; ch += TPR) {
      const int kt = ch >> 3, sl = ch & 7;
      const u32x4 v = *reinterpret_cast<const u32x4*>(xs + ((size_t)kt * TT + row) * 128 + ((sl ^ swz) << 4));
#pragma unroll
      for (int j = 0; j < 4; ++j) {
        const float a = bf16_lo(v[j]), bb = bf16_hi(v[j]);
        s += a + bb;
        q += a * a + bb * bb;
      }
    }
    s = dpp_add<0xB1>(s); q = dpp_add<0xB1>(q);
    s = dpp_add<0x4E>(s); q = dpp_add<0x4E>(q);
    s += __shfl_xor(s, 4); q += __shfl_xor(q, 4);
    if (TPR == 16) { s += __shfl_xor(s, 8); q += __shfl_xor(q, 8); }
    if (part == 0) {
      const float mean = s / (float)C;
      float var = q / (float)C - mean * mean;
      if (var < 0.f) var = 0.f;
      stats[row * 2] = mean;
      stats[row * 2 + 1] = rsqrtf(var + p.eps);
    }
  }
  __syncthreads();

  const float* scb = p.sc + (long long)b * hp * 2;
  for (int t = wave; t < tiles1; t += TA_WAVES) {
    const int rt = t % (TT / 32), ct = t / (TT / 32);
    const int row = rt * 32 + l31;
    const int swz = (l31 >> 1) & 7;
    const uint16_t* arow = Ab + (long long)ct * (32 * C) + lane * 8;
    f32x16 acc = zero16();
    if (t != wave) {
#pragma unroll
      for (int u = 0; u < TA_AHEAD; ++u)
#pragma unroll
        for (int ks = 0; ks < 4; ++ks) ar[u][ks] = *reinterpret_cast<const bf16x8_t*>(arow + (u * 4 + ks) * 512);
    }
#pragma unroll
    for (int kt = 0; kt < nkt; ++kt) {
      const int u = kt % TA_AHEAD;
      const char* xrow = xs + ((size_t)kt * TT + row) * 128;
      bf16x8_t af[4], xf[4];
#pragma unroll
      for (int ks = 0; ks < 4; ++ks) {
        af[ks] = ar[u][ks];
        xf[ks] = lds_read_frag(xrow + (((ks * 2 + hi) ^ swz) << 4));
      }
      if (kt + TA_AHEAD < nkt) {
#pragma unroll
        for (int ks = 0; ks < 4; ++ks) ar[u][ks] = *reinterpret_cast<const bf16x8_t*>(arow + ((kt + TA_AHEAD) * 4 + ks) * 512);
      }
#pragma unroll
      for (int ks = 0; ks < 4; ++ks) acc = mfma32(af[ks], xf[ks], acc);
    }
    const float mean = stats[row * 2], rstd = stats[row * 2 + 1];
    float sv[16];
#pragma unroll
    for (int r4 = 0; r4 < 4; ++r4) {
      const int j = ct * 32 + 8 * r4 + 4 * hi;
      const f32x4 c0 = *reinterpret_cast<const f32x4*>(scb + j * 2), c1 = *reinterpret_cast<const f32x4*>(scb + j * 2 + 4);
      sv[r4 * 4 + 0] = rstd * (acc[r4 * 4 + 0] - mean * c0[0]) + c0[1];
      sv[r4 * 4 + 1] = rstd * (acc[r4 * 4 + 1] - mean * c0[2]) + c0[3];
      sv[r4 * 4 + 2] = rstd * (acc[r4 * 4 + 2] - mean * c1[0]) + c1[1];
      sv[r4 * 4 + 3] = rstd * (acc[r4 * 4 + 3] - mean * c1[2]) + c1[3];
    }
#pragma unroll
    for (int h2 = 0; h2 < 2; ++h2) {
      float mx = sv[h2 * 8];
#pragma unroll
      for (int r = 1; r < 8; ++r) mx = fmaxf(mx, sv[h2 * 8 + r]);
      mx = fmaxf(mx, __shfl_xor(mx, 32));
      float sum = 0.f;
#pragma unroll
      for (int r = 0; r < 8; ++r) {
        sv[h2 * 8 + r] = __expf(sv[h2 * 8 + r] - mx);
        sum += sv[h2 * 8 + r];
      }
      sum += __shfl_xor(sum, 32);
      const float inv = 1.0f / sum;
#pragma unroll
      for (int r = 0; r < 8; ++r) sv[h2 * 8 + r] *= inv;
    }
#pragma unroll
    for (int r4 = 0; r4 < 4; ++r4) {
      const int j = ct * 32 + 8 * r4 + 4 * hi;
      u32x2 pk = {pack_bf16x2(sv[r4 * 4], sv[r4 * 4 + 1]), pack_bf16x2(sv[r4 * 4 + 2], sv[r4 * 4 + 3])};
      *reinterpret_cast<u32x2*>(pl + (size_t)row * prs + j * 2) = pk;
    }
  }
  __syncthreads();

  const uint16_t* Bb = p.BmT + (long long)b * C * hp;
  const int tiles2 = (ct_hi - ct_lo) * (TT / 32);
  constexpr int nks = NKS;
  for (int t = wave; t < tiles2; t += TA_WAVES) {
    const int rt = t % (TT / 32), ct = ct_lo + t / (TT / 32);
    const int row = rt * 32 + l31;
    const uint16_t* brow = Bb + (long long)ct * (32 * hp) + lane * 8;
    const char* prow = pl + (size_t)row * prs + hi * 16;
    f32x16 acc = zero16();
    bf16x8_t bn[NKS];
#pragma unroll
    for (int i = 0; i < NKS; ++i) bn[i] = *reinterpret_cast<const bf16x8_t*>(brow + i * 512);
#pragma unroll
    for (int ks = 0; ks < nks; ++ks) {
      const bf16x8_t pf = *reinterpret_cast<const bf16x8_t*>(prow + ks * 32);
      acc = mfma32(bn[ks], pf, acc);
    }
    {
      const bool rok = tok0 + row < p.M;
      const int swz = (row >> 1) & 7;
      float v[16];
#pragma unroll
      for (int r4 = 0; r4 < 4; ++r4) {
        const int c = ct * 32 + 8 * r4 + 4 * hi;
        const f32x4 bv = *reinterpret_cast<const f32x4*>(p.bias + c);
        const int kt = c >> 6, sl = (c & 63) >> 3;
        const u32x2 xr = *reinterpret_cast<const u32x2*>(xs + ((size_t)kt * TT + row) * 128 + ((sl ^ swz) << 4) + (c & 7) * 2);
        v[r4 * 4 + 0] = acc[r4 * 4 + 0] + bv[0] + bf16_lo(xr[0]);
        v[r4 * 4 + 1] = acc[r4 * 4 + 1] + bv[1] + bf16_hi(xr[0]);
        v[r4 * 4 + 2] = acc[r4 * 4 + 2] + bv[2] + bf16_lo(xr[1]);
        v[r4 * 4 + 3] = acc[r4 * 4 + 3] + bv[3] + bf16_hi(xr[1]);
        u32x2 pk = {pack_bf16x2(v[r4 * 4 + 0], v[r4 * 4 + 1]), pack_bf16x2(v[r4 * 4 + 2], v[r4 * 4 + 3])};
        if (rok) *reinterpret_cast<u32x2*>(og + (long long)row * C + c) = pk;
      }
      if constexpr (Q8) {
        uint32_t q[4], sb;
        mx8_quant_acc16(v, q, sb);
        float ps = 0.f, pq = 0.f;
#pragma unroll
        for (int r = 0; r < 16; ++r) ps += v[r], pq += v[r] * v[r];
        ps = xor32_sum(ps);
        pq = xor32_sum(pq);
        if (rok) {
          const long long m = tok0 + row;
#pragma unroll
          for (int r4 = 0; r4 < 4; ++r4) *reinterpret_cast<uint32_t*>(p.q8_out + m * C + ct * 32 + 8 * r4 + 4 * hi) = q[r4];
          if (hi == 0) {
            reinterpret_cast<uint8_t*>(p.q8_scale)[((long long)(ct >> 2) * p.M + m) * 4 + (ct & 3)] = (uint8_t)sb;
            f32x2 st2 = {ps, pq};
            *reinterpret_cast<f32x2*>(rst + ((size_t)row * (C >> 5) + ct) * 2) = st2;
          }
        }
      }
    }
  }
  if constexpr (Q8) q8_row_stats();
}

__global__ void __launch_bounds__(256) tattn_prepare_a_kernel(const uint16_t* __restrict__ kv, int ldkv, const uint16_t* __restrict__ wq,
                                                              int ldwq, const float* __restrict__ gamma, const float* __restrict__ beta,
                                                              uint16_t* __restrict__ A, float* __restrict__ sc, int L, int C, int hp,
                                                              int heads, float scale) {
  __shared__ float kvec[64];
  __shared__ float red[2][4];
  const int j = blockIdx.x, b = blockIdx.y, t = threadIdx.x;
  const int h = j >> 4, i = j & 15;
  uint16_t* const Ab = A + (long long)b * hp * C;
  const int nkt = C >> 6;
  auto aoff = [&](int k) {
    return ((((long long)(j >> 5) * nkt + (k >> 6)) * 4 + ((k >> 4) & 3)) * 64 + ((k >> 3) & 1) * 32 + (j & 31)) * 8 + (k & 7);
  };
  float* scj = sc + ((long long)b * hp + j) * 2;
  if (h >= heads || i >= L) {
    for (int k = t; k < C; k += 256) Ab[aoff(k)] = 0;
    if (t == 0) { scj[0] = 0.f; scj[1] = -1e30f; }
    return;
  }
  if (t < 64) kvec[t] = bf16_bits_to_f32(kv[((long long)b * L + i) * ldkv + h * 64 + t]) * scale;
  __syncthreads();
  float s = 0.f, c = 0.f;
  for (int k = t; k < C; k += 256) {
    float a = 0.f;
#pragma unroll 8
    for (int d = 0; d < 64; ++d) a += bf16_bits_to_f32(wq[(long long)(h * 64 + d) * ldwq + k]) * kvec[d];
    const uint32_t pk = pack_bf16x2(a * gamma[k], 0.f);
    Ab[aoff(k)] = (uint16_t)(pk & 0xffffu);
    s += bf16_lo(pk);
    c += beta[k] * a;
  }
#pragma unroll
  for (int off = 32; off > 0; off >>= 1) { s += __shfl_xor(s, off); c += __shfl_xor(c, off); }
  if ((t & 63) == 0) { red[0][t >> 6] = s; red[1][t >> 6] = c; }
  __syncthreads();
  if (t == 0) {
    scj[0] = red[0][0] + red[0][1] + red[0][2] + red[0][3];
    scj[1] = red[1][0] + red[1][1] + red[1][2] + red[1][3];
  }
}

__global__ void __launch_bounds__(256) tattn_prepare_b_kernel(const uint16_t* __restrict__ kv, int ldkv, int v_off,
                                                              const uint16_t* __restrict__ wo, int ldwo, uint16_t* __restrict__ BmT,
                                                              int B, int L, int C, int hp, int heads) {
  const long long idx = (long long)blockIdx.x * 256 + threadIdx.x;
  if (idx >= (long long)B * C * hp) return;
  const int j = (int)(idx % hp);
  const long long bc = idx / hp;
  const int c = (int)(bc % C), b = (int)(bc / C);
  const int h = j >> 4, i = j & 15;
  float a = 0.f;
  if (h < heads && i < L) {
    const uint16_t* vr = kv + ((long long)b * L + i) * ldkv + v_off + h * 64;
    const uint16_t* wr = wo + (long long)c * ldwo + h * 64;
#pragma unroll 8
    for (int d = 0; d < 64; ++d) a += bf16_bits_to_f32(vr[d]) * bf16_bits_to_f32(wr[d]);
  }
  const long long off = ((((long long)(c >> 5) * (hp >> 4) + (j >> 4)) * 64) + ((j >> 3) & 1) * 32 + (c & 31)) * 8 + (j & 7);
  BmT[(long long)b * C * hp + off] = (uint16_t)(pack_bf16x2(a, 0.f) & 0xffffu);
}

}

extern "C" int32_t udt_tattn_hp(int32_t heads) { return ((heads * 16 + 31) / 32) * 32; }

extern "C" int udt_tattn_prepare(const void* kv, int32_t ldkv, const void* wq, int32_t ldwq, const void* wo, int32_t ldwo,
                                 const float* gamma, const float* beta, void* A, float* sc, void* BmT, int32_t B, int32_t L,
                                 int32_t C, int32_t heads, float scale, void* stream) {
  if (!kv || !wq || !wo || !gamma || !beta || !A || !sc || !BmT) return UDT_ERR_BAD_ARG;
  if (B <= 0 || L <= 0 || L > 12 || heads <= 0 || C != heads * 64 || ldkv < 2 * C || ldwq < C || ldwo < C) return UDT_ERR_BAD_SHAPE;
  const int hp = udt_tattn_hp(heads);
  hipStream_t s = reinterpret_cast<hipStream_t>(stream);
  UdtProfScope prof(3, s);
  hipLaunchKernelGGL(tattn_prepare_a_kernel, dim3(hp, B), dim3(256), 0, s, reinterpret_cast<const uint16_t*>(kv), ldkv,
                     reinterpret_cast<const uint16_t*>(wq), ldwq, gamma, beta, reinterpret_cast<uint16_t*>(A), sc, L, C, hp, heads, scale);
  UDT_CHECK_LAUNCH();
  const long long n = (long long)B * C * hp;
  hipLaunchKernelGGL(tattn_prepare_b_kernel, dim3((unsigned)((n + 255) / 256)), dim3(256), 0, s,
                     reinterpret_cast<const uint16_t*>(kv), ldkv, C, reinterpret_cast<const uint16_t*>(wo), ldwo,
                     reinterpret_cast<uint16_t*>(BmT), B, L, C, hp, heads);
  UDT_CHECK_LAUNCH();
  return UDT_OK;
}

namespace {
int tattn_tt(int C) { return C >= 640 ? 32 : 64; }
int tattn_nsplit(int M, int TT) {
  const unsigned grid = (unsigned)(M / TT);
  constexpr unsigned target = 256u;
  int nsplit = 1;
  while (nsplit < 8 && grid * nsplit < target) nsplit *= 2;
  return nsplit;
}

int tattn_launch(const void* x, void* out, const void* A, const float* sc, const void* BmT, const float* bias, int32_t B, int32_t n_tok,
                 int32_t C, int32_t heads, int32_t zero_samples, float eps, void* q8_out, void* q8_scale, float* rowstat_out, void* stream) {
  if (!x || !out || !bias || (zero_samples < B && (!A || !sc || !BmT))) return UDT_ERR_BAD_ARG;
  if (B <= 0 || n_tok <= 0 || heads <= 0 || C != heads * 64 || C > 1280 || zero_samples < 0 || zero_samples > B) return UDT_ERR_BAD_SHAPE;
  const int TT = tattn_tt(C);
  if (n_tok % TT != 0) return UDT_ERR_BAD_SHAPE;
  const bool q8 = q8_out != nullptr;
  if (q8 && (!q8_scale || !rowstat_out || C % 128 != 0)) return UDT_ERR_BAD_ARG;
  TattnParams p;
  p.x = reinterpret_cast<const uint16_t*>(x); p.out = reinterpret_cast<uint16_t*>(out);
  p.A = reinterpret_cast<const uint16_t*>(A); p.sc = sc; p.BmT = reinterpret_cast<const uint16_t*>(BmT); p.bias = bias;
  p.zero = udt_zero_page();
  if (!p.zero) return UDT_ERR_HIP;
  p.M = B * n_tok; p.C = C; p.hp = udt_tattn_hp(heads); p.n_tok = n_tok; p.zero_samples = zero_samples; p.eps = eps;
  p.q8_out = reinterpret_cast<uint8_t*>(q8_out); p.q8_scale = reinterpret_cast<uint32_t*>(q8_scale); p.rowstat_out = rowstat_out;
  const size_t smem = (size_t)TT * C * 2 + (size_t)TT * 2 * sizeof(float) + (size_t)TT * (p.hp * 2 + 16) + (q8 ? (size_t)TT * (C / 32) * 8 : 0);
  hipStream_t s = reinterpret_cast<hipStream_t>(stream);
  UdtProfScope prof(3, s);
  if (prof.rec) {
    char tag[96];
    snprintf(tag, sizeof(tag), "tattn_fused%s B=%d n=%d C=%d zero=%d", q8 ? "+q8" : "", B, n_tok, C, zero_samples);
    udt_prof_tag(prof.rec, tag);
  }
  static bool attr_done[5] = {false, false, false, false, false};
  const unsigned grid = (unsigned)(p.M / TT);
  p.nsplit = tattn_nsplit(p.M, TT);
  const void* fn = nullptr;
  int which = -1;
  if (C == 320 && p.hp == 96 && !q8) { fn = reinterpret_cast<const void*>(tattn_fused_kernel<64, 5, 6>); which = 0; }
  else if (C == 640 && p.hp == 160) { fn = q8 ? reinterpret_cast<const void*>(tattn_fused_kernel<32, 10, 10, true>) : reinterpret_cast<const void*>(tattn_fused_kernel<32, 10, 10>); which = q8 ? 3 : 1; }
  else if (C == 1280 && p.hp == 320) { fn = q8 ? reinterpret_cast<const void*>(tattn_fused_kernel<32, 20, 20, true>) : reinterpret_cast<const void*>(tattn_fused_kernel<32, 20, 20>); which = q8 ? 4 : 2; }
  else return UDT_ERR_BAD_SHAPE;
  if (!attr_done[which]) {
    hipError_t e = hipFuncSetAttribute(fn, hipFuncAttributeMaxDynamicSharedMemorySize, 128 * 1024);
    if (e != hipSuccess) return udt_set_hip_error(e);
    attr_done[which] = true;
  }
  void* args[] = {&p};
  hipError_t el = hipLaunchKernel(fn, dim3(grid, p.nsplit), dim3(TA_THREADS), args, smem, s);
  if (el != hipSuccess) return udt_set_hip_error(el);
  UDT_CHECK_LAUNCH();
  return UDT_OK;
}
}

extern "C" int udt_tattn_fused(const void* x, void* out, const void* A, const float* sc, const void* BmT, const float* bias,
                               int32_t B, int32_t n_tok, int32_t C, int32_t heads, int32_t zero_samples, float eps, void* stream) {
  return tattn_launch(x, out, A, sc, BmT, bias, B, n_tok, C, heads, zero_samples, eps, nullptr, nullptr, nullptr, stream);
}

extern "C" int32_t udt_tattn_rowstat_parts(int32_t B, int32_t n_tok, int32_t C) {
  if (B <= 0 || n_tok <= 0 || (C != 640 && C != 1280)) return 0;
  const int TT = tattn_tt(C);
  if (n_tok % TT != 0) return 0;
  return tattn_nsplit(B * n_tok, TT);
}

extern "C" int udt_tattn_fused_q8(const void* x, void* out, const void* A, const float* sc, const void* BmT, const float* bias,
                                  int32_t B, int32_t n_tok, int32_t C, int32_t heads, int32_t zero_samples, float eps, void* q8_out,
                                  void* q8_scale, float* rowstat_out, void* stream) {
  if (!q8_out) return UDT_ERR_BAD_ARG;
  return tattn_launch(x, out, A, sc, BmT, bias, B, n_tok, C, heads, zero_samples, eps, q8_out, q8_scale, rowstat_out, stream);
}
```

### udifftext_amd/ops.py

```python
from __future__ import annotations

import contextlib
import ctypes as C
import os
import threading
from typing import NamedTuple, Optional, Sequence

import torch

from . import lib as L

WORKSPACE_BYTES = 96 << 20


class Workspace:

    def __init__(self, device, nbytes: int = WORKSPACE_BYTES):
        if torch.device(device).type != "cuda":
            raise L.UdtError("udifftext_amd workspaces live on the GPU (no CPU fallback)")
        self.buf = torch.zeros(nbytes, dtype=torch.uint8, device=device)

    def check(self, stream: Optional[int] = None) -> None:
        L.check(L.load().udt_check_async_error(self.buf.data_ptr(), self.buf.numel(), _stream() if stream is None else stream),
                "udt_check_async_error")


class _Ctx(threading.local):
    cu_share = 1
    workspace: Optional[Workspace] = None


_ctx = _Ctx()
_default_ws: dict = {}


@contextlib.contextmanager
def launch_context(cu_share: Optional[int] = None, workspace: Optional[Workspace] = None):
    prev = (_ctx.cu_share, _ctx.workspace)
    if cu_share is not None:
        _ctx.cu_share = max(1, int(cu_share))
    if workspace is not None:
        _ctx.workspace = workspace
    try:
        yield
    finally:
        _ctx.cu_share, _ctx.workspace = prev


def _stream() -> int:
    return torch.cuda.current_stream().cuda_stream


def _ptr(t: Optional[torch.Tensor]) -> Optional[int]:
    if t is None:
        return None
    if not t.is_cuda:
        raise L.UdtError("udifftext_amd ops need device tensors (no CPU fallback)")
    return t.data_ptr()


def _ws(nbytes: int, device) -> torch.Tensor:
    ws = _ctx.workspace
    if ws is None:
        key = (device.type, device.index, _stream())
        ws = _default_ws.get(key)
        if ws is None:
            ws = _default_ws[key] = Workspace(device)
    if ws.buf.numel() < nbytes:
        raise L.UdtError(f"stream-K workspace of {ws.buf.numel()} bytes is too small for this launch ({nbytes})")
    return ws.buf


def check_async_errors() -> None:
    for (_, _, stream), ws in list(_default_ws.items()):
        ws.check(stream)


WORK_COUNTER: Optional[dict] = None


def count_work(kind: str, amount: float) -> None:
    if WORK_COUNTER is not None:
        WORK_COUNTER[kind] = WORK_COUNTER.get(kind, 0.0) + amount


def _bf16(t: torch.Tensor) -> None:
    if t.dtype != torch.bfloat16:
        raise ValueError(f"expected bf16 tensor, got {t.dtype}")


def gemm_desc(**kw) -> L.GemmDesc:
    d = L.GemmDesc()
    d.batch = 1
    d.alpha = 1.0
    d.cu_share = _ctx.cu_share
    for k, v in kw.items():
        setattr(d, k, v)
    return d


def run_gemm(d: L.GemmDesc, device, fused_gn: bool = False) -> None:
    lib = L.load()
    need = lib.udt_gemm_workspace_bytes(C.byref(d))
    ws_ptr, ws_bytes = None, 0
    if need:
        ws = _ws(need, device)
        ws_ptr, ws_bytes = ws.data_ptr(), ws.numel()
    if fused_gn:
        L.check(lib.udt_gn_silu_conv3x3_fwd(C.byref(d), ws_ptr, ws_bytes, _stream()), "udt_gn_silu_conv3x3_fwd")
    else:
        L.check(lib.udt_gemm(C.byref(d), ws_ptr, ws_bytes, _stream()), "udt_gemm")


GN_STRIP = True


class GnStats(NamedTuple):
    data: torch.Tensor
    slots_per_sample: int


def gn_stats_of(t: Optional[torch.Tensor]) -> Optional[GnStats]:
    return getattr(t, "gn_stats", None) if t is not None else None


def _attach_colstats(d: L.GemmDesc, out: torch.Tensor, n_cols: int, rows_per_batch: int) -> bool:
    lib = L.load()
    rows = lib.udt_gemm_colstats_rows(C.byref(d))
    if rows <= 0:
        return False
    slots = lib.udt_gemm_colstats_slots(C.byref(d))
    st = torch.empty((slots, n_cols, 2), dtype=torch.float32, device=out.device)
    d.colstats = st.data_ptr()
    out.gn_stats = GnStats(st, rows_per_batch // rows)
    return True


def _drop_stale_stats(out: Optional[torch.Tensor]) -> None:
    if out is not None and getattr(out, "gn_stats", None) is not None:
        del out.gn_stats


class Mx8Act(NamedTuple):
    data: torch.Tensor
    scale: torch.Tensor
    stats: Optional[torch.Tensor] = None


def mx8_of(t: Optional[torch.Tensor]) -> Optional[Mx8Act]:
    return getattr(t, "mx8", None) if t is not None else None


def _mx8_alloc(M: int, cols: int, device) -> Mx8Act:
    return Mx8Act(torch.empty((M, cols), dtype=torch.uint8, device=device),
                  torch.empty(((cols + 127) // 128, M), dtype=torch.int32, device=device))


def _attach_q8(d: L.GemmDesc, M: int, cols: int, device, rowstats: bool, fixed: Optional[tuple] = None) -> Optional[Mx8Act]:
    q = _mx8_alloc(M, cols, device)
    d.q8_out, d.q8_scale, d.ld_q8 = q.data.data_ptr(), q.scale.data_ptr(), cols
    if fixed is not None:
        d.q8_fixed_col, d.q8_fixed_mul = int(fixed[0]), float(fixed[1])
    lib = L.load()
    parts = lib.udt_gemm_rowstat_parts(C.byref(d)) if rowstats else 0
    if not lib.udt_gemm_q8_ok(C.byref(d)) or (rowstats and parts <= 0):
        d.q8_out, d.q8_scale, d.ld_q8, d.q8_fixed_col = None, None, 0, 0
        return None
    if rowstats:
        st = torch.empty((parts, M, 2), dtype=torch.float32, device=device)
        d.rowstat_out = st.data_ptr()
        q = Mx8Act(q.data, q.scale, st)
    return q


def linear(x: torch.Tensor, w: torch.Tensor, bias: Optional[torch.Tensor] = None, *, out: Optional[torch.Tensor] = None,
           residual: Optional[torch.Tensor] = None, rowvec: Optional[torch.Tensor] = None, rows_per_batch: int = 0,
           flags: int = 0, alpha: float = 1.0, n_out: Optional[int] = None, colstats: bool = False,
           emit_q8: bool = False, emit_rowstats: bool = False) -> torch.Tensor:
    _bf16(x); _bf16(w)
    K = x.shape[-1]
    x2 = x.reshape(-1, K) if x.is_contiguous() else x
    assert x2.dim() == 2 and x2.stride(1) == 1
    M = x2.shape[0]
    N = w.shape[0] if n_out is None else n_out
    assert w.shape[1] == K and w.is_contiguous()
    n_cols = N // 2 if (flags & L.GEMM_GEGLU) else N
    if out is None:
        dt = torch.float32 if (flags & L.GEMM_OUT_F32) else torch.bfloat16
        if flags & L.GEMM_TRANSPOSED:
            assert rows_per_batch > 0
            out = torch.empty((M // rows_per_batch, N, rows_per_batch), dtype=dt, device=x.device)
        else:
            out = torch.empty((M, n_cols), dtype=dt, device=x.device)
    ldo = out.stride(0) if not (flags & L.GEMM_TRANSPOSED) else 0
    d = gemm_desc(a=_ptr(x2), w=_ptr(w), bias=_ptr(bias), residual=_ptr(residual), rowvec=_ptr(rowvec), out=_ptr(out),
                  M=M, N=N, K=K, lda=x2.stride(0), ldo=ldo, ldr=(residual.stride(0) if residual is not None else 0),
                  rows_per_batch=rows_per_batch, ld_rowvec=(rowvec.stride(0) if rowvec is not None else 0), flags=flags,
                  alpha=alpha)
    if not (colstats and rows_per_batch > 0 and out.is_contiguous() and _attach_colstats(d, out, n_cols, rows_per_batch)):
        _drop_stale_stats(out)
    q8 = None
    if emit_q8 and not (flags & (L.GEMM_OUT_F32 | L.GEMM_TRANSPOSED | L.GEMM_GEGLU)) and d.colstats is None and rowvec is None:
        q8 = _attach_q8(d, M, n_cols, x.device, emit_rowstats)
    run_gemm(d, x.device)
    if getattr(out, "mx8", None) is not None:
        del out.mx8
    if q8 is not None:
        out.mx8 = q8
    if WORK_COUNTER is not None:
        count_work("gemm", 2.0 * M * N * K)
        count_work("gemm_bytes", 2.0 * (M * K + N * K) + out.numel() * out.element_size()
                   + (2.0 * M * n_cols if residual is not None else 0.0))
        count_work("gemm_launches", 1.0)
    return out


def linear_mx8(x: Mx8Act, wq: torch.Tensor, colscale: torch.Tensor, bias: Optional[torch.Tensor] = None, *,
               out: Optional[torch.Tensor] = None, residual: Optional[torch.Tensor] = None, rows_per_batch: int = 0,
               flags: int = 0, n_out: Optional[int] = None, colstats: bool = False, emit_q8: bool = False,
               emit_rowstats: bool = False, ln_c: Optional[torch.Tensor] = None, ln_s: Optional[torch.Tensor] = None,
               eps: float = 1e-5, want_bf16: bool = True, q8_fixed: Optional[tuple] = None):
    xq = x.data
    assert xq.dtype == torch.uint8 and wq.dtype == torch.uint8 and xq.is_contiguous() and wq.is_contiguous()
    M, K = xq.shape
    N = wq.shape[0] if n_out is None else n_out
    assert wq.shape[1] == K and K % 128 == 0 and colscale.dtype == torch.float32 and colscale.numel() >= N
    assert x.scale.dtype == torch.int32 and x.scale.shape == (K // 128, M) and x.scale.is_contiguous()
    geglu = bool(flags & L.GEMM_GEGLU)
    n_cols = N // 2 if geglu else N
    only_q8 = emit_q8 and not want_bf16
    if out is None and not only_q8:
        out = torch.empty((M, n_cols), dtype=torch.bfloat16, device=xq.device)
    d = gemm_desc(a=_ptr(xq), w=_ptr(wq), bias=_ptr(ln_c if ln_c is not None else bias), residual=_ptr(residual),
                  out=_ptr(out), M=M, N=N, K=K, lda=K, ldo=(out.stride(0) if out is not None else 0),
                  ldr=(residual.stride(0) if residual is not None else 0), rows_per_batch=rows_per_batch,
                  flags=flags | L.GEMM_MX8, colscale=_ptr(colscale), a_scale=_ptr(x.scale))
    if ln_s is not None:
        if x.stats is None:
            raise L.UdtError("linear_mx8: a LayerNorm-folded MX8 GEMM needs the row statistics of its input (Mx8Act.stats)")
        assert x.stats.dtype == torch.float32 and x.stats.is_contiguous() and x.stats.shape[1:] == (M, 2)
        d.ln_colsum, d.ln_eps = _ptr(ln_s), eps
        d.rowstat_in, d.rowstat_in_parts = _ptr(x.stats), x.stats.shape[0]
    if out is not None and not (colstats and rows_per_batch > 0 and out.is_contiguous()
                                and _attach_colstats(d, out, n_cols, rows_per_batch)):
        _drop_stale_stats(out)
    q8 = None
    if emit_q8:
        q8 = _attach_q8(d, M, n_cols, xq.device, emit_rowstats and not geglu, fixed=q8_fixed)
        if q8 is None:
            raise L.UdtError(f"udt_gemm has no MX8-emitting plan for M={M} N={N} K={K} flags={flags:#x}")
    run_gemm(d, xq.device)
    if out is not None and getattr(out, "mx8", None) is not None:
        del out.mx8
    if WORK_COUNTER is not None:
        count_work("gemm_fp8", 2.0 * M * N * K)
        count_work("gemm_fp8_launches", 1.0)
    if only_q8:
        return q8
    if q8 is not None:
        out.mx8 = q8
    return out


def ln_linear(x: torch.Tensor, w_folded: torch.Tensor, c: torch.Tensor, s: torch.Tensor, *, eps: float = 1e-5,
              out: Optional[torch.Tensor] = None, residual: Optional[torch.Tensor] = None, flags: int = 0,
              n_out: Optional[int] = None, emit_q8: bool = False, want_bf16: bool = True, q8_fixed: Optional[tuple] = None,
              q8_or_none: bool = False):
    _bf16(x); _bf16(w_folded)
    K = x.shape[-1]
    x2 = x.reshape(-1, K) if x.is_contiguous() else x
    assert x2.dim() == 2 and x2.stride(1) == 1 and w_folded.shape[1] == K and w_folded.is_contiguous()
    M = x2.shape[0]
    N = w_folded.shape[0] if n_out is None else n_out
    n_cols = N // 2 if (flags & L.GEMM_GEGLU) else N
    only_q8 = emit_q8 and not want_bf16
    if out is None and not only_q8:
        out = torch.empty((M, n_cols), dtype=torch.bfloat16, device=x.device)
    d = gemm_desc(a=_ptr(x2), w=_ptr(w_folded), bias=_ptr(c), residual=_ptr(residual), out=_ptr(out), M=M, N=N, K=K,
                  lda=x2.stride(0), ldo=(out.stride(0) if out is not None else 0),
                  ldr=(residual.stride(0) if residual is not None else 0), flags=flags, ln_colsum=_ptr(s), ln_eps=eps)
    q8 = None
    if emit_q8:
        q8 = _attach_q8(d, M, n_cols, x.device, False, fixed=q8_fixed)
        if q8 is None:
            if q8_or_none:
                return None
            raise L.UdtError(f"udt_ln_gemm_fwd has no MX8-emitting plan for M={M} N={N} K={K}")
    lib = L.load()
    need = lib.udt_gemm_workspace_bytes(C.byref(d))
    ws_ptr, ws_bytes = None, 0
    if need:
        ws = _ws(need, x.device)
        ws_ptr, ws_bytes = ws.data_ptr(), ws.numel()
    rc = lib.udt_ln_gemm_fwd(C.byref(d), ws_ptr, ws_bytes, _stream())
    if rc in (-1, -2) and x.is_cuda:
        raise L.UdtError(f"udt_ln_gemm_fwd declined M={M} N={N} K={K} flags={flags:#x} (status {rc}): the LayerNorm-folded GEMM "
                         "needs the lean kernel family (UDT_LEAN / udt_debug_set('lean') != 0) and 16-byte aligned operands; "
                         "set UDT_LN_GEMM=0 to run layernorm + GEMM instead")
    L.check(rc, "udt_ln_gemm_fwd")
    if WORK_COUNTER is not None:
        count_work("gemm", 2.0 * M * N * K)
        count_work("gemm_bytes", 2.0 * (M * K + N * K) + (2.0 if out is not None else 0.0) * M * n_cols
                   + (1.0 * M * n_cols if q8 is not None else 0.0) + (2.0 * M * n_cols if residual is not None else 0.0))
        count_work("gemm_launches", 1.0)
    if only_q8:
        return q8
    if q8 is not None:
        out.mx8 = q8
    return out


def bmm_nt(a: torch.Tensor, w: torch.Tensor, *, out: Optional[torch.Tensor] = None, alpha: float = 1.0) -> torch.Tensor:
    _bf16(a); _bf16(w)
    B, M, K = a.shape
    N = w.shape[1]
    assert a.stride(2) == 1 and w.stride(2) == 1 and w.shape[0] == B and w.shape[2] == K
    if out is None:
        out = torch.empty((B, M, N), dtype=torch.bfloat16, device=a.device)
    d = gemm_desc(a=_ptr(a), w=_ptr(w), out=_ptr(out), M=M, N=N, K=K, lda=a.stride(1), ldw=w.stride(1),
                  ldo=out.stride(1), batch=B, stride_a=a.stride(0), stride_w=w.stride(0), stride_out=out.stride(0),
                  alpha=alpha)
    run_gemm(d, a.device)
    if WORK_COUNTER is not None:
        count_work("gemm", 2.0 * B * M * N * K)
        count_work("gemm_bytes", 2.0 * B * (M * K + N * K + M * N))
        count_work("gemm_launches", 1.0)
    return out


def conv2d(x: torch.Tensor, w: torch.Tensor, bias: Optional[torch.Tensor] = None, *, ksize: int = 3, stride: int = 1,
           pad: Optional[tuple] = None, upsample: bool = False, x2: Optional[torch.Tensor] = None,
           out_hw: Optional[tuple] = None, residual: Optional[torch.Tensor] = None,
           rowvec: Optional[torch.Tensor] = None, flags: int = 0, n_out: Optional[int] = None,
           out: Optional[torch.Tensor] = None, colstats: bool = False, in_scsh: Optional[torch.Tensor] = None,
           in_act: int = 0, probe_in_scsh: bool = False, w_up4: Optional[torch.Tensor] = None):
    _bf16(x); _bf16(w)
    assert x.is_contiguous() and w.is_contiguous()
    B, H, W_, C1 = x.shape
    C2 = 0
    if x2 is not None:
        _bf16(x2)
        assert x2.is_contiguous() and x2.shape[:3] == x.shape[:3]
        C2 = x2.shape[3]
    Hv, Wv = (H * 2, W_ * 2) if upsample else (H, W_)
    if pad is None:
        pad = (ksize // 2, ksize // 2)
    if out_hw is None:
        out_hw = ((Hv + 2 * pad[0] - ksize) // stride + 1, (Wv + 2 * pad[1] - ksize) // stride + 1)
    Ho, Wo = out_hw
    N = w.shape[0] if n_out is None else n_out
    K = ksize * ksize * (C1 + C2)
    assert w.shape[1] == K, (w.shape, K)
    M = B * Ho * Wo
    if out is None and not probe_in_scsh:
        dt = torch.float32 if (flags & L.GEMM_OUT_F32) else torch.bfloat16
        out = torch.empty((B, Ho, Wo, N), dtype=dt, device=x.device)
    d = gemm_desc(a=_ptr(x), a2=_ptr(x2), w=_ptr(w), bias=_ptr(bias), residual=_ptr(residual), rowvec=_ptr(rowvec),
                  out=_ptr(out), M=M, N=N, K=K, lda=0, ldo=(out.stride(2) if out is not None else N),
                  ldr=(residual.stride(2) if residual is not None else 0),
                  Hin=H, Win=W_, C1=C1, C2=C2, Hout=Ho, Wout=Wo, ksize=ksize, stride=stride, pad_t=pad[0], pad_l=pad[1],
                  upsample=1 if upsample else 0, rows_per_batch=Ho * Wo,
                  ld_rowvec=(rowvec.stride(0) if rowvec is not None else 0), flags=flags | L.GEMM_CONV)
    if probe_in_scsh:
        return bool(L.load().udt_gemm_in_scsh_ok(C.byref(d)))
    if w_up4 is not None and upsample and ksize == 3 and x2 is None and in_scsh is None:
        _bf16(w_up4)
        assert w_up4.is_contiguous() and w_up4.dim() == 3 and w_up4.shape[0] == 4 and w_up4.shape[1] >= N and w_up4.shape[2] == 4 * C1, \
            (w_up4.shape, N, C1)
        d.upsample, d.w, d.ldw, d.stride_w = 2, _ptr(w_up4), w_up4.shape[2], w_up4.stride(0)
        if not L.load().udt_gemm_up4_ok(C.byref(d)):
            d.upsample, d.w, d.ldw, d.stride_w = 1, _ptr(w), 0, 0
    if in_scsh is not None:
        assert in_scsh.dtype == torch.float32 and in_scsh.is_contiguous() and in_scsh.numel() == B * (C1 + C2) * 2
        d.in_scsh = in_scsh.data_ptr()
        d.in_act = int(in_act)
    if not (colstats and _attach_colstats(d, out, N, Ho * Wo)):
        _drop_stale_stats(out)
    if in_scsh is not None:
        run_gemm(d, x.device, fused_gn=True)
    else:
        run_gemm(d, x.device)
    return out


def attention(q: torch.Tensor, k: torch.Tensor, vt: torch.Tensor, heads: int, scale: float,
              out: Optional[torch.Tensor] = None) -> torch.Tensor:
    _bf16(q); _bf16(k); _bf16(vt)
    B, Nq = q.shape[0], q.shape[1]
    Nk = k.shape[1]
    assert q.stride(2) == 1 and k.stride(2) == 1 and vt.stride(2) == 1
    if out is None:
        out = torch.empty((B, Nq, heads * 64), dtype=torch.bfloat16, device=q.device)
    L.check(L.load().udt_attn_fwd(_ptr(q), _ptr(k), _ptr(vt), _ptr(out), B, heads, Nq, Nk,
                                  q.stride(1), k.stride(1), vt.stride(1), out.stride(1),
                                  q.stride(0), k.stride(0), vt.stride(0), out.stride(0), scale, _stream()),
            "udt_attn_fwd")
    if WORK_COUNTER is not None:
        count_work("attn", 4.0 * B * heads * Nq * Nk * 64)
        count_work("attn_bytes", 2.0 * B * heads * 64 * (2 * Nq + 2 * Nk))
        count_work("attn_launches", 1.0)
    return out


def attention_rowv(q: torch.Tensor, k: torch.Tensor, v: torch.Tensor, heads: int, scale: float,
                   out: Optional[torch.Tensor] = None, emit_q8: bool = False) -> torch.Tensor:
    _bf16(q); _bf16(k); _bf16(v)
    B, Nq = q.shape[0], q.shape[1]
    Nk = k.shape[1]
    assert q.stride(2) == 1 and k.stride(2) == 1 and v.stride(2) == 1 and v.shape[1] == Nk
    if out is None:
        out = torch.empty((B, Nq, heads * 64), dtype=torch.bfloat16, device=q.device)
    if getattr(out, "mx8", None) is not None:
        del out.mx8
    if emit_q8 and heads % 2 == 0 and out.is_contiguous():
        q8 = _mx8_alloc(B * Nq, heads * 64, q.device)
        L.check(L.load().udt_attn_rowv_q8_fwd(_ptr(q), _ptr(k), _ptr(v), _ptr(out), B, heads, Nq, Nk,
                                              q.stride(1), k.stride(1), v.stride(1), out.stride(1),
                                              q.stride(0), k.stride(0), v.stride(0), out.stride(0), scale,
                                              _ptr(q8.data), _ptr(q8.scale), heads * 64, _stream()), "udt_attn_rowv_q8_fwd")
        out.mx8 = q8
    else:
        L.check(L.load().udt_attn_rowv_fwd(_ptr(q), _ptr(k), _ptr(v), _ptr(out), B, heads, Nq, Nk,
                                           q.stride(1), k.stride(1), v.stride(1), out.stride(1),
                                           q.stride(0), k.stride(0), v.stride(0), out.stride(0), scale, _stream()),
                "udt_attn_rowv_fwd")
    if WORK_COUNTER is not None:
        count_work("attn", 4.0 * B * heads * Nq * Nk * 64)
        count_work("attn_bytes", 2.0 * B * heads * 64 * (2 * Nq + 2 * Nk))
        count_work("attn_launches", 1.0)
    return out


def attention_mx8(qkv: Mx8Act, batch: int, heads: int, scale: float, v_mul: float, out: Optional[torch.Tensor] = None,
                  emit_q8: bool = False) -> torch.Tensor:
    C_ = heads * 64
    M, ld8 = qkv.data.shape
    assert qkv.data.dtype == torch.uint8 and qkv.data.is_contiguous() and ld8 >= 3 * C_ and M % batch == 0
    assert qkv.scale.dtype == torch.int32 and qkv.scale.is_contiguous() and qkv.scale.shape == ((ld8 + 127) // 128, M)
    N = M // batch
    if out is None:
        out = torch.empty((batch, N, C_), dtype=torch.bfloat16, device=qkv.data.device)
    assert out.is_contiguous()
    if getattr(out, "mx8", None) is not None:
        del out.mx8
    q8 = _mx8_alloc(M, C_, qkv.data.device) if emit_q8 else None
    L.check(L.load().udt_attn_mx8_fwd(_ptr(qkv.data), _ptr(qkv.scale), _ptr(out), batch, heads, N, ld8, out.stride(1), scale,
                                      1.0 / v_mul, _ptr(q8.data) if q8 else None, _ptr(q8.scale) if q8 else None, C_, _stream()),
            "udt_attn_mx8_fwd")
    if q8 is not None:
        out.mx8 = q8
    if WORK_COUNTER is not None:
        count_work("attn_fp8", 4.0 * batch * heads * N * N * 64)
        count_work("attn_fp8_bytes", 1.0 * batch * heads * 64 * 3 * N + 2.0 * batch * heads * 64 * N)
        count_work("attn_fp8_launches", 1.0)
    return out


def attention_d512(q: torch.Tensor, k: torch.Tensor, v: torch.Tensor, scale: float,
                   out: Optional[torch.Tensor] = None, key_split: bool = True) -> torch.Tensor:
    _bf16(q); _bf16(k); _bf16(v)
    B, Nq = q.shape[0], q.shape[1]
    Nk = k.shape[1]
    assert q.shape[2] == 512 and k.shape[2] == 512 and v.shape[2] == 512 and v.shape[1] == Nk
    assert q.stride(2) == 1 and k.stride(2) == 1 and v.stride(2) == 1
    if out is None:
        out = torch.empty((B, Nq, 512), dtype=torch.bfloat16, device=q.device)
    lib = L.load()
    need = int(lib.udt_attn512_workspace_bytes(B, Nq, Nk)) if key_split else 0
    if need:
        scratch = torch.empty((need,), dtype=torch.uint8, device=q.device)
        L.check(lib.udt_attn512_split_fwd(_ptr(q), _ptr(k), _ptr(v), _ptr(out), B, Nq, Nk,
                                          q.stride(1), k.stride(1), v.stride(1), out.stride(1),
                                          q.stride(0), k.stride(0), v.stride(0), out.stride(0), scale, _ptr(scratch), need, _stream()),
                "udt_attn512_split_fwd")
    else:
        L.check(lib.udt_attn512_fwd(_ptr(q), _ptr(k), _ptr(v), _ptr(out), B, Nq, Nk,
                                    q.stride(1), k.stride(1), v.stride(1), out.stride(1),
                                    q.stride(0), k.stride(0), v.stride(0), out.stride(0), scale, _stream()),
                "udt_attn512_fwd")
    if WORK_COUNTER is not None:
        count_work("attn", 4.0 * B * Nq * Nk * 512)
        count_work("attn_bytes", 2.0 * B * 512 * (2 * Nq + 2 * Nk))
        count_work("attn_launches", 1.0)
    return out


def xattention(q: torch.Tensor, k: torch.Tensor, v: torch.Tensor, heads: int, head_dim: int, scale: float,
               probs: Optional[torch.Tensor] = None, out: Optional[torch.Tensor] = None) -> torch.Tensor:
    _bf16(q); _bf16(k); _bf16(v)
    B, Nq = q.shape[0], q.shape[1]
    Lc = k.shape[1]
    assert q.is_contiguous() or (q.stride(2) == 1 and q.stride(0) == Nq * q.stride(1))
    assert k.stride(2) == 1 and v.stride(2) == 1 and k.stride(1) == v.stride(1)
    assert k.stride(0) == Lc * k.stride(1) and v.stride(0) == Lc * v.stride(1)
    if out is None:
        out = torch.empty((B, Nq, heads * head_dim), dtype=torch.bfloat16, device=q.device)
    if probs is not None:
        assert probs.dtype == torch.float32 and probs.is_contiguous() and probs.numel() == B * heads * Nq * Lc
    L.check(L.load().udt_xattn_fwd(_ptr(q), _ptr(k), _ptr(v), _ptr(out), _ptr(probs), B, heads, head_dim, Nq, Lc,
                                   q.stride(1), k.stride(1), out.stride(1), scale, _stream()), "udt_xattn_fwd")
    return out


def masked_attention(q: torch.Tensor, k: torch.Tensor, v: torch.Tensor, heads: int, scale: float,
                     mask: Optional[torch.Tensor] = None, key_padding_mask: Optional[torch.Tensor] = None,
                     out: Optional[torch.Tensor] = None) -> torch.Tensor:
    _bf16(q); _bf16(k); _bf16(v)
    B, Nq, Cq = q.shape
    Lk = k.shape[1]
    D = Cq // heads
    assert q.stride(2) == 1 and k.stride(2) == 1 and v.stride(2) == 1
    if out is None:
        out = torch.empty((B, Nq, heads * D), dtype=torch.bfloat16, device=q.device)
    if mask is not None:
        mask = mask.float().contiguous()
        assert mask.shape == (Nq, Lk)
    if key_padding_mask is not None:
        key_padding_mask = key_padding_mask.to(torch.uint8).contiguous()
        assert key_padding_mask.shape == (B, Lk)
    L.check(L.load().udt_mattn_fwd(_ptr(q), _ptr(k), _ptr(v), _ptr(out), _ptr(mask), _ptr(key_padding_mask), B, heads, D,
                                   Nq, Lk, q.stride(1), k.stride(1), v.stride(1), out.stride(1), Lk,
                                   q.stride(0), k.stride(0), v.stride(0), out.stride(0), scale, _stream()), "udt_mattn_fwd")
    return out


class TattnTables(NamedTuple):
    A: torch.Tensor
    sc: torch.Tensor
    BmT: torch.Tensor

    def rows(self, begin: int, end: Optional[int] = None) -> "TattnTables":
        return TattnTables(self.A[begin:end], self.sc[begin:end], self.BmT[begin:end])


def tattn_prepare(kv: torch.Tensor, wq: torch.Tensor, wo: torch.Tensor, gamma: torch.Tensor, beta: torch.Tensor, heads: int,
                  scale: float, out: Optional[TattnTables] = None) -> TattnTables:
    _bf16(kv); _bf16(wq); _bf16(wo)
    B, Lc, two_c = kv.shape
    Cc = heads * 64
    assert two_c == 2 * Cc and kv.is_contiguous() and wq.is_contiguous() and wo.is_contiguous()
    hp = L.load().udt_tattn_hp(heads)
    if out is None:
        out = TattnTables(torch.empty((B, hp, Cc), dtype=torch.bfloat16, device=kv.device),
                          torch.empty((B, hp, 2), dtype=torch.float32, device=kv.device),
                          torch.empty((B, Cc, hp), dtype=torch.bfloat16, device=kv.device))
    L.check(L.load().udt_tattn_prepare(_ptr(kv), two_c, _ptr(wq), wq.stride(0), _ptr(wo), wo.stride(0), _ptr(gamma), _ptr(beta),
                                       _ptr(out.A), _ptr(out.sc), _ptr(out.BmT), B, Lc, Cc, heads, scale, _stream()),
            "udt_tattn_prepare")
    return out


def tattn_fused(x: torch.Tensor, tables: Optional[TattnTables], bias: torch.Tensor, heads: int, zero_samples: int, eps: float,
                out: Optional[torch.Tensor] = None, emit_q8: bool = False) -> torch.Tensor:
    _bf16(x)
    assert x.is_contiguous()
    B, N, Cc = x.shape
    if out is None:
        out = torch.empty_like(x)
    assert out.is_contiguous()
    if tables is not None:
        assert tables.A.is_contiguous() and tables.sc.is_contiguous() and tables.BmT.is_contiguous() and tables.A.shape[0] == B
    if getattr(out, "mx8", None) is not None:
        del out.mx8
    parts = L.load().udt_tattn_rowstat_parts(B, N, Cc) if emit_q8 else 0
    if parts > 0:
        q = _mx8_alloc(B * N, Cc, x.device)
        q = Mx8Act(q.data, q.scale, torch.empty((parts, B * N, 2), dtype=torch.float32, device=x.device))
        L.check(L.load().udt_tattn_fused_q8(_ptr(x), _ptr(out), _ptr(tables.A) if tables else None, _ptr(tables.sc) if tables else None,
                                            _ptr(tables.BmT) if tables else None, _ptr(bias), B, N, Cc, heads, zero_samples, eps,
                                            _ptr(q.data), _ptr(q.scale), _ptr(q.stats), _stream()), "udt_tattn_fused_q8")
        out.mx8 = q
        return out
    L.check(L.load().udt_tattn_fused(_ptr(x), _ptr(out), _ptr(tables.A) if tables else None, _ptr(tables.sc) if tables else None,
                                     _ptr(tables.BmT) if tables else None, _ptr(bias), B, N, Cc, heads, zero_samples, eps, _stream()),
            "udt_tattn_fused")
    return out


def softmax_rows_(x: torch.Tensor) -> torch.Tensor:
    _bf16(x)
    assert x.is_contiguous()
    cols = x.shape[-1]
    L.check(L.load().udt_softmax_rows(_ptr(x), x.numel() // cols, cols, cols, _stream()), "udt_softmax_rows")
    return x


def group_norm(x: torch.Tensor, gamma: torch.Tensor, beta: torch.Tensor, groups: int, eps: float, silu: bool,
               out: Optional[torch.Tensor] = None, x2: Optional[torch.Tensor] = None) -> torch.Tensor:
    _bf16(x)
    assert x.is_contiguous()
    B, C1 = x.shape[0], x.shape[-1]
    C2 = 0
    if x2 is not None:
        _bf16(x2)
        assert x2.is_contiguous() and x2.shape[:-1] == x.shape[:-1]
        C2 = x2.shape[-1]
    HW = x.numel() // (B * C1)
    lib = L.load()
    if out is None:
        out = torch.empty(x.shape[:-1] + (C1 + C2,), dtype=torch.bfloat16, device=x.device)
    if GN_STRIP and lib.udt_gn_strip_ok(B, HW, C1, C2, groups):
        L.check(lib.udt_gn_strip(_ptr(x), _ptr(x2), _ptr(out), _ptr(gamma), _ptr(beta), B, HW, C1, C2, groups, eps,
                                 1 if silu else 0, _stream()), "udt_gn_strip")
        return out
    nch = lib.udt_gn_nchunks(HW, C1 + C2)
    part = torch.empty((B, nch, groups, 2), dtype=torch.float32, device=x.device)
    L.check(lib.udt_gn_stats(_ptr(x), _ptr(x2), _ptr(part), B, HW, C1, C2, groups, _stream()), "udt_gn_stats")
    L.check(lib.udt_gn_apply(_ptr(x), _ptr(x2), _ptr(out), _ptr(part), _ptr(gamma), _ptr(beta), B, HW, C1, C2, groups,
                             eps, 1 if silu else 0, _stream()), "udt_gn_apply")
    return out


def gn_finalize(st1: GnStats, C1: int, st2: Optional[GnStats], C2: int, gamma: torch.Tensor, beta: torch.Tensor, B: int,
                HW: int, groups: int, eps: float) -> torch.Tensor:
    Ct = C1 + C2
    scsh = torch.empty((B, Ct // 64, 2, 64), dtype=torch.float32, device=st1.data.device)
    L.check(L.load().udt_gn_finalize(_ptr(st1.data), st1.slots_per_sample, C1, _ptr(st2.data) if st2 is not None else None,
                                     st2.slots_per_sample if st2 is not None else 0, C2, _ptr(gamma), _ptr(beta), _ptr(scsh),
                                     B, HW, groups, eps, _stream()), "udt_gn_finalize")
    return scsh


def gn_strip_ok(B: int, HW: int, C1: int, C2: int, groups: int) -> bool:
    return bool(GN_STRIP and L.load().udt_gn_strip_ok(B, HW, C1, C2, groups))


def group_norm_from_stats(x: torch.Tensor, st1: GnStats, gamma: torch.Tensor, beta: torch.Tensor, groups: int, eps: float,
                          silu: bool, x2: Optional[torch.Tensor] = None, st2: Optional[GnStats] = None,
                          out: Optional[torch.Tensor] = None) -> torch.Tensor:
    _bf16(x)
    assert x.is_contiguous()
    B, C1 = x.shape[0], x.shape[-1]
    C2 = 0
    if x2 is not None:
        _bf16(x2)
        assert x2.is_contiguous() and x2.shape[:-1] == x.shape[:-1] and st2 is not None
        C2 = x2.shape[-1]
    HW = x.numel() // (B * C1)
    if out is None:
        out = torch.empty(x.shape[:-1] + (C1 + C2,), dtype=torch.bfloat16, device=x.device)
    if gn_strip_ok(B, HW, C1, C2, groups):
        L.check(L.load().udt_gn_strip_stats(_ptr(x), _ptr(x2), _ptr(out), _ptr(st1.data), st1.slots_per_sample,
                                            _ptr(st2.data) if st2 is not None else None,
                                            st2.slots_per_sample if st2 is not None else 0, _ptr(gamma), _ptr(beta), B, HW, C1, C2,
                                            groups, eps, 1 if silu else 0, _stream()), "udt_gn_strip_stats")
        return out
    scsh = gn_finalize(st1, C1, st2, C2, gamma, beta, B, HW, groups, eps)
    L.check(L.load().udt_gn_apply_scsh(_ptr(x), _ptr(x2), _ptr(out), _ptr(scsh), B, HW, C1, C2, 1 if silu else 0, _stream()),
            "udt_gn_apply_scsh")
    return out


def layer_norm(x: torch.Tensor, gamma: torch.Tensor, beta: torch.Tensor, eps: float = 1e-5,
               out: Optional[torch.Tensor] = None) -> torch.Tensor:
    _bf16(x)
    assert x.is_contiguous()
    Cc = x.shape[-1]
    if out is None:
        out = torch.empty_like(x)
    L.check(L.load().udt_layernorm(_ptr(x), _ptr(out), _ptr(gamma), _ptr(beta), x.numel() // Cc, Cc, eps, _stream()),
            "udt_layernorm")
    return out


def unet_input(x: torch.Tensor, xin: torch.Tensor, c_in: float) -> None:
    B, _, h, w = x.shape
    L.check(L.load().udt_unet_input(_ptr(x), _ptr(xin), B, h * w, xin.shape[-1], c_in, _stream()), "udt_unet_input")


def unet_input_churn(x: torch.Tensor, noise: torch.Tensor, xin: torch.Tensor, c_in: float, kn: float) -> None:
    B, _, h, w = x.shape
    for t in (x, noise):
        assert t.dtype == torch.float32 and t.is_contiguous() and tuple(t.shape) == (B, 4, h, w), "fp32 NCHW [B,4,h,w]"
    L.check(L.load().udt_unet_input_churn(_ptr(x), _ptr(noise), _ptr(xin), B, h * w, xin.shape[-1], c_in, kn, _stream()),
            "udt_unet_input_churn")


def cfg_euler_step(x: torch.Tensor, eps: torch.Tensor, sigma: float, sigma_next: float, scale: float,
                   denoised: Optional[torch.Tensor] = None, c_out: Optional[float] = None) -> None:
    B, _, h, w = x.shape
    assert x.dtype == torch.float32 and eps.dtype == torch.float32 and x.is_contiguous() and eps.is_contiguous()
    L.check(L.load().udt_cfg_euler_step(_ptr(x), _ptr(eps), _ptr(denoised), B, h * w, eps.shape[-1],
                                        -sigma if c_out is None else c_out, sigma, sigma_next, scale, _stream()),
            "udt_cfg_euler_step")


def cfg_sampler_step(xin: torch.Tensor, eps: torch.Tensor, c_out: float, scale: float, kx: float = 0.0, kd: float = 0.0,
                     aux: Optional[torch.Tensor] = None, ka: float = 0.0, prev: Optional[torch.Tensor] = None, kp: float = 0.0,
                     noise: Optional[torch.Tensor] = None, kn: float = 0.0, out: Optional[torch.Tensor] = None,
                     denoised: Optional[torch.Tensor] = None) -> torch.Tensor:
    B, _, h, w = xin.shape
    out = xin if out is None else out
    for t in (xin, aux, prev, noise, out, denoised):
        if t is not None:
            assert t.dtype == torch.float32 and t.is_contiguous() and tuple(t.shape) == (B, 4, h, w), "fp32 NCHW [B,4,h,w]"
    assert eps.dtype == torch.float32 and eps.is_contiguous() and tuple(eps.shape[:-1]) == (2 * B, h, w) and eps.shape[-1] >= 4
    k = L.SamplerCoefs(kx, kd, ka, kp, kn, c_out, scale)
    L.check(L.load().udt_cfg_sampler_step(_ptr(xin), _ptr(eps), _ptr(aux), _ptr(prev), _ptr(noise), _ptr(out), _ptr(denoised),
                                          B, h * w, eps.shape[-1], k, _stream()), "udt_cfg_sampler_step")
    return out


def cfg_multistep_step(xin: torch.Tensor, eps: torch.Tensor, c_out: float, scale: float, sigma: float, coefs: Sequence[float],
                       hist: Sequence[torch.Tensor] = (), d_out: Optional[torch.Tensor] = None,
                       out: Optional[torch.Tensor] = None) -> torch.Tensor:
    B, _, h, w = xin.shape
    out = xin if out is None else out
    n = len(coefs)
    assert 1 <= n <= L.MULTISTEP_MAX and len(hist) == n - 1, "n = len(coefs) in 1..8 and len(hist) = n - 1"
    assert d_out is not None, "d_out is required"
    for t in (xin, out, d_out, *hist):
        assert t.dtype == torch.float32 and t.is_contiguous() and tuple(t.shape) == (B, 4, h, w), "fp32 NCHW [B,4,h,w]"
    assert eps.dtype == torch.float32 and eps.is_contiguous() and tuple(eps.shape[:-1]) == (2 * B, h, w) and eps.shape[-1] >= 4
    k = L.MultistepCoefs(c_out, scale, sigma, n)
    for j, c in enumerate(coefs):
        k.k[j] = c
    for j, t in enumerate(hist):
        k.hist[j + 1] = _ptr(t)
    L.check(L.load().udt_cfg_multistep_step(_ptr(xin), _ptr(eps), _ptr(out), _ptr(d_out), B, h * w, eps.shape[-1], k,
                                            _stream()), "udt_cfg_multistep_step")
    return out


def _check_step_args(xin: torch.Tensor, f: torch.Tensor, pair: bool, what: str, *others) -> tuple:
# ... 587 lines not shown
```

### udifftext_amd/sgm/modules/attention.py

```python
from __future__ import annotations

import os
from typing import List, Optional

import torch
import torch.nn as nn

from udifftext_amd import ops, packing

from . import hipnn as H
from .diffusionmodules.util import zero_module


TATTN_FUSED = True

FF_PROJ = os.environ.get("UDT_FF_PROJ", "1") != "0"


class GEGLU(H._Packed):
    def __init__(self, dim_in: int, dim_out: int):
        super().__init__()
        self.proj = H.Linear(dim_in, dim_out * 2)

    def _sources(self):
        return self.proj._sources()

    def fused_children(self):
        return [self.proj]

    def _pack(self):
        return packing.pack_geglu(self.proj.weight, self.proj.bias)

    def _pack_ln(self, gamma, beta):
        return packing.pack_ln_linear(self.proj.weight, self.proj.bias, gamma, beta, geglu=True)

    def _pack_ln_mx8(self, gamma, beta):
        return packing.pack_ln_linear_mx8(self.proj.weight, self.proj.bias, gamma, beta, geglu=True)

    def forward(self, x, ln=None, x8=None):
        if ln is not None and x8 is not None:
            wq, cs, c, s = self.packed_ln_mx8(ln)
            return ops.linear_mx8(x8, wq, cs, ln_c=c, ln_s=s, eps=ln.eps, flags=H.GEMM_GEGLU, emit_q8=True, want_bf16=False)
        if ln is not None:
            wf, c, s = self.packed_ln(ln)
            return ops.ln_linear(x, wf, c, s, eps=ln.eps, flags=H.GEMM_GEGLU)
        w, b = self.packed()
        return ops.linear(x, w, b, flags=H.GEMM_GEGLU)


class FeedForward(nn.Module):
    def __init__(self, dim, dim_out=None, mult=4, glu=True, dropout=0.0):
        super().__init__()
        if not glu:
            raise NotImplementedError("only the gated (GEGLU) feed-forward is on the UDiffText path")
        inner = int(dim * mult)
        self.net = nn.Sequential(GEGLU(dim, inner), nn.Identity(), H.Linear(inner, dim_out or dim))

    def forward(self, x, residual=None, ln=None, x8=None, emit_q8: bool = False, emit_rowstats: bool = False):
        h = self.net[0](x, ln=ln, x8=x8)
        if isinstance(h, ops.Mx8Act):
            return self.net[2](None, residual=residual, x8=h, emit_q8=emit_q8, emit_rowstats=emit_rowstats)
        return self.net[2](h, residual=residual)


def map_hw(n_tokens: int, hw=None) -> tuple:
    if hw is None:
        s = int(n_tokens ** 0.5)
        hw = (s, s)
    h, w = int(hw[0]), int(hw[1])
    if h <= 0 or w <= 0 or h * w != n_tokens:
        raise ValueError(f"a t_attn map of {n_tokens} tokens is not {h} x {w}: pass hw=(h, w)")
    return h, w


class CrossAttention(H._Packed):

    def __init__(self, query_dim, context_dim=None, heads=8, dim_head=64, dropout=0.0):
        super().__init__()
        inner = dim_head * heads
        context_dim = context_dim or query_dim
        self.scale = dim_head ** -0.5
        self.heads, self.dim_head = heads, dim_head
        self.to_q = H.Linear(query_dim, inner, bias=False)
        self.to_k = H.Linear(context_dim, inner, bias=False)
        self.to_v = H.Linear(context_dim, inner, bias=False)
        self.to_out = zero_module(nn.Sequential(H.Linear(inner, query_dim), nn.Identity()))
        self.attn_map_cache = None

    def _sources(self):
        return self.to_k.weight, self.to_v.weight

    def fused_children(self):
        return [self.to_k, self.to_v]

    def _pack(self):
        return H.fuse_rows(self.to_k.weight, self.to_v.weight)

    def project_context(self, context_bf16: torch.Tensor) -> torch.Tensor:
        B, Lc, Dc = context_bf16.shape
        return ops.linear(context_bf16.reshape(B * Lc, Dc), self.packed()).reshape(B, Lc, -1)

    def forward(self, x, context=None, kv=None, residual=None, emit_map: bool = False, out=None, hw=None):
        inner = self.heads * self.dim_head
        B, N, _ = x.shape
        q = self.to_q(x.reshape(B * N, -1)).reshape(B, N, inner)
        if kv is None:
            kv = self.project_context(context)
        probs = None
        if emit_map and self.attn_map_cache is not None:
            probs = torch.empty((B * self.heads, N, kv.shape[1]), dtype=torch.float32, device=q.device)
            self.attn_map_cache["size"] = int(N ** 0.5)
            self.attn_map_cache["hw"] = map_hw(N, hw)
            self.attn_map_cache["attn_map"] = probs
        o = ops.xattention(q, kv[..., :inner], kv[..., inner:], self.heads, self.dim_head, self.scale, probs=probs)
        res = residual.reshape(B * N, -1) if residual is not None else None
        out2 = out.reshape(B * N, -1) if out is not None else None
        return self.to_out[0](o.reshape(B * N, inner), residual=res, out=out2).reshape(B, N, -1)

    def prepare_fused(self, kv: torch.Tensor, t_norm, out=None):
        if kv.shape[1] < 2 or kv.shape[1] > 12 or self.dim_head != 64 or not TATTN_FUSED:
            return None
        wq, _ = self.to_q.packed()
        wo, _ = self.to_out[0].packed()
        return ops.tattn_prepare(kv.contiguous(), wq, wo, t_norm.weight, t_norm.bias, self.heads, self.scale, out=out)

    def zero_context_residual(self, x, out):
        _, b = self.to_out[0].packed()
        return ops.bias_add(x, b, out=out)




class MemoryEfficientCrossAttention(H._Packed):

    def __init__(self, query_dim, context_dim=None, heads=8, dim_head=64, dropout=0.0, **kwargs):
        super().__init__()
        if dim_head != 64:
            raise NotImplementedError("udt_attn_fwd is specialised for head_dim 64 (num_head_channels: 64)")
        inner = dim_head * heads
        context_dim = context_dim or query_dim
        self.heads, self.dim_head = heads, dim_head
        self.to_q = H.Linear(query_dim, inner, bias=False)
        self.to_k = H.Linear(context_dim, inner, bias=False)
        self.to_v = H.Linear(context_dim, inner, bias=False)
        self.to_out = nn.Sequential(H.Linear(inner, query_dim), nn.Identity())

    def _sources(self):
        return self.to_q.weight, self.to_k.weight, self.to_v.weight

    def fused_children(self):
        return [self.to_q, self.to_k, self.to_v]

    def _pack(self):
        return H.fuse_rows(self.to_q.weight, self.to_k.weight, self.to_v.weight), None

    def _pack_ln(self, gamma, beta):
        pk = packing.pack_ln_linear(torch.cat([self.to_q.weight, self.to_k.weight, self.to_v.weight], 0), None, gamma, beta)
        inner = self.heads * self.dim_head
        self.v_mul = H.v_fixed_mul(pk[0][2 * inner:3 * inner], pk[1][2 * inner:3 * inner])
        return pk

    def _pack_ln_mx8(self, gamma, beta):
        pk = packing.pack_ln_linear_mx8(torch.cat([self.to_q.weight, self.to_k.weight, self.to_v.weight], 0), None, gamma, beta)
        inner = self.heads * self.dim_head
        wv = pk[0][2 * inner:3 * inner].view(torch.float8_e4m3fn).float() * pk[1][2 * inner:3 * inner, None]
        self.v_mul8 = H.v_fixed_mul(wv, pk[2][2 * inner:3 * inner])
        return pk

    def forward(self, x, context=None, mask=None, residual=None, ln=None, x8=None):
        if context is not None or mask is not None:
            raise NotImplementedError("attn1 is pure self-attention on this path (reference attention.py:251-252)")
        inner = self.heads * self.dim_head
        B, N, C = x.shape
        x2 = x.reshape(B * N, C)
        mx = ln is not None and x8 is not None
        a8 = ln is not None and H.fp8_attention() and N % 4 == 0
        scale = self.dim_head ** -0.5
        o = None
        if mx:
            wq, cs, c, sv = self.packed_ln_mx8(ln)
            if a8:
                qkv8 = ops.linear_mx8(x8, wq, cs, ln_c=c, ln_s=sv, eps=ln.eps, emit_q8=True, want_bf16=False,
                                      q8_fixed=(2 * inner, self.v_mul8))
                o = ops.attention_mx8(qkv8, B, self.heads, scale, self.v_mul8, emit_q8=True)
            else:
                qkv = ops.linear_mx8(x8, wq, cs, ln_c=c, ln_s=sv, eps=ln.eps).reshape(B, N, 3 * inner)
        elif ln is not None:
            wf, c, sv = self.packed_ln(ln)
            qkv8 = None
            if a8 and C == 320:
                qkv8 = ops.ln_linear(x2, wf, c, sv, eps=ln.eps, emit_q8=True, want_bf16=False, q8_fixed=(2 * inner, self.v_mul),
                                     q8_or_none=True)
            if qkv8 is not None:
                o = ops.attention_mx8(qkv8, B, self.heads, scale, self.v_mul)
            else:
                qkv = ops.ln_linear(x2, wf, c, sv, eps=ln.eps).reshape(B, N, 3 * inner)
        else:
            qkv = ops.linear(x2, self.packed()[0]).reshape(B, N, 3 * inner)
        if o is None:
            o = ops.attention_rowv(qkv[..., :inner], qkv[..., inner:2 * inner], qkv[..., 2 * inner:], self.heads, scale, emit_q8=mx)
        res = residual.reshape(B * N, -1) if residual is not None else None
        return self.to_out[0](o.reshape(B * N, inner), residual=res, x8=ops.mx8_of(o) if mx else None).reshape(B, N, -1)


class BasicTransformerBlock(nn.Module):
    def __init__(self, dim, n_heads, d_head, dropout=0.0, t_context_dim=None, v_context_dim=None, gated_ff=True):
        super().__init__()
        self.attn1 = MemoryEfficientCrossAttention(query_dim=dim, heads=n_heads, dim_head=d_head)
        if t_context_dim is not None and t_context_dim > 0:
            self.t_attn = CrossAttention(query_dim=dim, context_dim=t_context_dim, heads=n_heads, dim_head=d_head)
            self.t_norm = H.LayerNorm(dim)
        if v_context_dim is not None and v_context_dim > 0:
            raise NotImplementedError("v_attn is not configured in UDiffText (v_context_dim unset)")
        self.norm1 = H.LayerNorm(dim)
        self.norm3 = H.LayerNorm(dim)
        self.ff = FeedForward(dim, dropout=dropout, glu=gated_ff)

    def fused_tattn_ok(self, n_tokens: int) -> bool:
        C = self.t_attn.heads * self.t_attn.dim_head
        return (TATTN_FUSED and self.t_attn.dim_head == 64 and C in (320, 640, 1280) and self.t_attn.heads * 64 == C
                and n_tokens % (32 if C >= 640 else 64) == 0)

    def forward(self, x, t_context=None, v_context=None, t_kv=None, emit_map: bool = False, zero_ctx_rows: int = 0,
                t_fused=None, x8=None, emit_rowstats: bool = False, defer_ff_out: bool = False, hw=None):
        fold = H.LN_GEMM
        mx = fold and x8 is not None and H.mx8_width(x.shape[-1])
        x = self.attn1(x, residual=x, ln=self.norm1, x8=x8 if mx else None) if fold else self.attn1(self.norm1(x), residual=x)
        if hasattr(self, "t_attn"):
            n0 = 0 if emit_map else min(int(zero_ctx_rows), x.shape[0])
            if t_fused is not None and not emit_map and n0 < x.shape[0] and self.fused_tattn_ok(x.shape[1]):
                _, bo = self.t_attn.to_out[0].packed()
                x = ops.tattn_fused(x, t_fused, bo, self.t_attn.heads, n0, self.t_norm.eps, emit_q8=mx)
            elif n0 > 0 and t_kv is not None:
                y = torch.empty_like(x)
                self.t_attn.zero_context_residual(x[:n0], y[:n0])
                if n0 < x.shape[0]:
                    xc = x[n0:]
                    self.t_attn(self.t_norm(xc), kv=t_kv[n0:], residual=xc, out=y[n0:])
                x = y
            else:
                x = self.t_attn(self.t_norm(x), context=t_context, kv=t_kv, residual=x, emit_map=emit_map, hw=hw)
        B, N, C = x.shape
        x2 = x.reshape(B * N, C)
        if fold:
            x8b = ops.mx8_of(x) if mx else None
            if defer_ff_out and x8b is None:
                return self.ff.net[0](x2, ln=self.norm3), x2
            out = self.ff(x2, residual=x2, ln=self.norm3, x8=x8b, emit_q8=x8b is not None, emit_rowstats=emit_rowstats)
            return H.carry_mx8(out.reshape(B, N, C), out)
        return self.ff(self.norm3(x2), residual=x2).reshape(B, N, C)

    def prepare_ln(self) -> int:
        folded = ((self.attn1, self.norm1), (self.ff.net[0], self.norm3))
        pks = [mod.packed_ln(norm) for mod, norm in folded]
        if H.mx8_width(self.norm1.dim):
            pks += [mod.packed_ln_mx8(norm) for mod, norm in folded]
            pks += [lin.packed_fp8() for lin in (self.attn1.to_out[0], self.ff.net[2])]
        return H.nbytes(*pks)


class SpatialTransformer(nn.Module):
    def __init__(self, in_channels, n_heads, d_head, depth=1, dropout=0.0, t_context_dim=None, v_context_dim=None,
                 use_linear=False):
        super().__init__()
        if not use_linear:
            raise NotImplementedError("use_linear_in_transformer: True is the UDiffText configuration")
        self.in_channels = in_channels
        inner = n_heads * d_head
        self.norm = H.GroupNorm(32, in_channels, eps=1e-6)
        self.proj_in = H.Linear(in_channels, inner)
        self.transformer_blocks = nn.ModuleList(
            [BasicTransformerBlock(inner, n_heads, d_head, dropout=dropout, t_context_dim=t_context_dim,
                                   v_context_dim=v_context_dim) for _ in range(depth)])
        self.proj_out = zero_module(H.Linear(inner, in_channels))
        self.use_linear = use_linear

    def project_context(self, context_bf16) -> List[torch.Tensor]:
        return [blk.t_attn.project_context(context_bf16) for blk in self.transformer_blocks]

    def prepare_fused(self, kv_list, out=None) -> list:
        return [blk.t_attn.prepare_fused(kv, blk.t_norm, out=(out[i] if out is not None else None))
                for i, (blk, kv) in enumerate(zip(self.transformer_blocks, kv_list))]

    def forward(self, x, t_context=None, v_context=None, t_kv: Optional[list] = None, emit_map: bool = False,
                zero_ctx_rows: int = 0, t_fused: Optional[list] = None):
        B, Hh, Ww, C = x.shape
        N = Hh * Ww
        mx = H.mx8_width(self.proj_in.out_features)
        t2 = self.proj_in(self.norm(x).reshape(B * N, C), emit_q8=mx, emit_rowstats=mx)
        t = H.carry_mx8(t2.reshape(B, N, -1), t2)
        nb = len(self.transformer_blocks)
        defer = FF_PROJ and H.LN_GEMM and not mx
        for i, blk in enumerate(self.transformer_blocks):
            t = blk(t, t_context=t_context, t_kv=(t_kv[i] if t_kv is not None else None), emit_map=emit_map,
                    zero_ctx_rows=zero_ctx_rows, t_fused=(t_fused[i] if t_fused is not None else None),
                    x8=ops.mx8_of(t) if mx else None, emit_rowstats=(i + 1 < nb), defer_ff_out=(defer and i + 1 == nb),
                    hw=(Hh, Ww))
        if isinstance(t, tuple):
            hid, t3 = t
            w, b = self.packed_ffproj()
            st = H.want_stats(B, N, w.shape[0])
            out = ops.conv2d(hid.reshape(B, Hh, Ww, -1), w, b, x2=t3.reshape(B, Hh, Ww, -1), ksize=1, pad=(0, 0), residual=x,
                             n_out=w.shape[0], colstats=st)
            if ops.WORK_COUNTER is not None:
                inner = hid.shape[-1]
                H.count_flops("gemm", 2.0 * B * N * C * (inner + C))
                H.count_flops("gemm_bytes", 2.0 * B * N * (inner + 3 * C) + 2.0 * C * (inner + C))
                H.count_flops("gemm_launches", 1.0)
            return out
        out = self.proj_out(t.reshape(B * N, -1), residual=x.reshape(B * N, C), rows_per_batch=N, colstats=True,
                            x8=ops.mx8_of(t) if mx else None)
        return H.carry_stats(out.reshape(B, Hh, Ww, C), out)

    def _sources(self):
        lin2, po = self.transformer_blocks[-1].ff.net[2], self.proj_out
        return lin2.weight, lin2.bias, po.weight, po.bias

    def _pack_ffproj(self):
        lin2, po = self.transformer_blocks[-1].ff.net[2], self.proj_out
        w2, wpo = lin2.weight.float(), po.weight.float()
        wf = torch.cat([wpo @ w2, wpo], dim=1)
        bias = wpo @ lin2.bias.float() + po.bias.float()
        return packing.pack_conv(wf[:, :, None, None], [w2.shape[1], wpo.shape[1]]), packing.pad_bias(bias)

    def packed_ffproj(self):
        return H.layout(self, "ffproj", self._pack_ffproj)

    def prepare_ffproj(self) -> int:
        return H.nbytes(self.packed_ffproj()) if FF_PROJ and H.LN_GEMM else 0

    def prepare_mx8(self) -> int:
        return H.nbytes(self.proj_out.packed_fp8()) if H.mx8_width(self.proj_in.out_features) else 0
```

### udifftext_amd/sgm/modules/hipnn.py

```python
from __future__ import annotations

import math
import os
from typing import Optional

import torch
import torch.nn as nn

from udifftext_amd import lib as L
from udifftext_amd import ops, packing

from ..util import init_skipped


def count_flops(kind: str, flops: float) -> None:
    ops.count_work(kind, flops)


FUSE_GN = os.environ.get("UDT_FUSE_GN", "0") != "0"

GN_EPI = os.environ.get("UDT_GN_EPI", "1") != "0" and os.environ.get("UDT_LEAN", "") != "0"
EMIT_STATS = FUSE_GN or GN_EPI


def want_stats(B: int, HW: int, C: int) -> bool:
    return FUSE_GN or (GN_EPI and C % 8 == 0)


FP8_LINEARS = os.environ.get("UDT_FP8", "0") != "0"


FP8_ATTENTION = os.environ.get("UDT_FP8_ATTN", "1") != "0"


def fp8_attention() -> bool:
    return FP8_LINEARS and LN_GEMM and FP8_ATTENTION


def v_fixed_mul(w_v: torch.Tensor, c_v: torch.Tensor) -> float:
    bound = 12.0 * float(w_v.float().norm(dim=1).max()) + float(c_v.float().abs().max())
    return float(2.0 ** math.floor(math.log2(448.0 / max(bound, 1e-20))))


def mx8_width(c: int) -> bool:
    return FP8_LINEARS and LN_GEMM and c % 128 == 0

LN_GEMM = os.environ.get("UDT_LN_GEMM", "1") != "0" and os.environ.get("UDT_LEAN", "") != "0"


def carry_stats(dst: torch.Tensor, src: torch.Tensor) -> torch.Tensor:
    st = ops.gn_stats_of(src)
    if st is not None:
        dst.gn_stats = st
    return dst


def carry_mx8(dst: torch.Tensor, src: torch.Tensor) -> torch.Tensor:
    q = ops.mx8_of(src)
    if q is not None:
        dst.mx8 = q
    return dst


def _init_uniform_(p: torch.Tensor, fan_in: int) -> None:
    if init_skipped():
        return
    bound = 1.0 / math.sqrt(max(fan_in, 1))
    with torch.no_grad():
        p.uniform_(-bound, bound)


class _Layouts(dict):
    frozen = False


def _layouts(mod: nn.Module) -> _Layouts:
    store = mod.__dict__.get("_layouts")
    if store is None:
        store = mod.__dict__["_layouts"] = _Layouts()
    return store


def layout(mod: nn.Module, tag: str, build, *inputs):
    store = _layouts(mod)
    hit = store.get(tag)
    if store.frozen:
        if hit is None:
            raise L.UdtError(f"{type(mod).__name__}: layout {tag!r} was not built before prepare(free_masters=True) released the "
                             "fp32 masters; reload the checkpoint into a fresh engine to change the launch path")
        return hit[1]
    key = [(t.data_ptr(), t._version, t.device) if isinstance(t, torch.Tensor) else t for t in (*mod._sources(), *inputs)]
    if hit is None or hit[0] != key:
        with torch.no_grad():
            hit = store[tag] = (key, build())
    return hit[1]


def has_layout(mod: nn.Module, tag: str) -> bool:
    return tag in mod.__dict__.get("_layouts", ())


def freeze_layouts(mod: nn.Module) -> None:
    _layouts(mod).frozen = True


def drop_layouts(root: nn.Module) -> None:
    for m in root.modules():
        store = m.__dict__.get("_layouts")
        if store is not None and not store.frozen:
            store.clear()


def nbytes(*layouts) -> int:
    ts = [t for pk in layouts for t in (pk if isinstance(pk, (tuple, list)) else (pk,))]
    return sum(t.numel() * t.element_size() for t in ts if isinstance(t, torch.Tensor))


class _Packed(nn.Module):

    def _sources(self):
        return self._parameters.values()

    def fused_children(self):
        return []

    def packed(self):
        return layout(self, "plain", self._pack)

    def packed_fp8(self):
        return layout(self, "fp8", self._pack_fp8)

    def packed_ln(self, norm):
        return layout(self, "ln", lambda: self._pack_ln(norm.weight, norm.bias), norm.weight, norm.bias)

    def packed_ln_mx8(self, norm):
        return layout(self, "ln_mx8", lambda: self._pack_ln_mx8(norm.weight, norm.bias), norm.weight, norm.bias)


class Linear(_Packed):
    def __init__(self, in_features: int, out_features: int, bias: bool = True):
        super().__init__()
        self.in_features, self.out_features = in_features, out_features
        self.weight = nn.Parameter(torch.empty(out_features, in_features))
        _init_uniform_(self.weight, in_features)
        if bias:
            self.bias = nn.Parameter(torch.empty(out_features))
            _init_uniform_(self.bias, in_features)
        else:
            self.register_parameter("bias", None)

    def _pack(self):
        return packing.pack_linear(self.weight), packing.pad_bias(self.bias)

    def _pack_fp8(self):
        wq, cs = packing.pack_linear_fp8(self.weight)
        return wq, cs, packing.pad_bias(self.bias)

    def forward(self, x, residual=None, flags: int = 0, out=None, rowvec=None, rows_per_batch: int = 0,
                colstats: bool = False, x8=None, emit_q8: bool = False, emit_rowstats: bool = False):
        if x8 is not None:
            wq, cs, b = self.packed_fp8()
            M = x8.data.shape[0]
            if colstats:
                rpb = rows_per_batch if rows_per_batch > 0 else M
                colstats = want_stats(M // rpb, rpb, wq.shape[0])
            return ops.linear_mx8(x8, wq, cs, b, residual=residual, flags=flags, out=out, rows_per_batch=rows_per_batch,
                                  colstats=bool(colstats), emit_q8=emit_q8, emit_rowstats=emit_rowstats)
        w, b = self.packed()
        if colstats:
            rpb = rows_per_batch if rows_per_batch > 0 else x.shape[0]
            colstats = want_stats(x.shape[0] // rpb, rpb, w.shape[0])
        return ops.linear(x, w, b, residual=residual, flags=flags, out=out, rowvec=rowvec, rows_per_batch=rows_per_batch,
                          colstats=bool(colstats), emit_q8=emit_q8, emit_rowstats=emit_rowstats)


class Conv2d(_Packed):

    def __init__(self, in_channels: int, out_channels: int, kernel_size: int, stride: int = 1, padding: int = 0):
        super().__init__()
        self.in_channels, self.out_channels = in_channels, out_channels
        self.kernel_size, self.stride, self.padding = kernel_size, stride, padding
        self.weight = nn.Parameter(torch.empty(out_channels, in_channels, kernel_size, kernel_size))
        self.bias = nn.Parameter(torch.empty(out_channels))
        fan_in = in_channels * kernel_size * kernel_size
        _init_uniform_(self.weight, fan_in)
        _init_uniform_(self.bias, fan_in)
        self.segments = None
        self.n_pad = 4
        self.emit_colstats = False

    def _pack(self):
        return packing.pack_conv(self.weight, self.segments, self.n_pad), packing.pad_bias(self.bias, self.n_pad)

    def packed(self):
        return layout(self, "plain", self._pack, self.segments, self.n_pad)

    def packed_up4(self):
        return layout(self, "up4", lambda: packing.pack_conv_up4(self.weight, self.n_pad), self.n_pad)

    def forward(self, x, x2=None, residual=None, rowvec=None, upsample: bool = False, flags: int = 0,
                pad: Optional[tuple] = None, out_hw: Optional[tuple] = None, norm: Optional["GroupNorm"] = None,
                norm_silu: bool = False, colstats: Optional[bool] = None):
        if x2 is not None and self.segments is None and (x.shape[-1] % 64 != 0 or x2.shape[-1] % 64 != 0):
            self.segments = (x.shape[-1], x2.shape[-1])
        w, b = self.packed()
        if pad is None:
            pad = (self.padding, self.padding)
        if colstats is None:
            colstats = self.emit_colstats
        if colstats:
            oh, ow = out_hw if out_hw is not None else ((x.shape[1] * (2 if upsample else 1) + 2 * pad[0] - self.kernel_size) // self.stride + 1,
                                                        (x.shape[2] * (2 if upsample else 1) + 2 * pad[1] - self.kernel_size) // self.stride + 1)
            colstats = want_stats(x.shape[0], oh * ow, w.shape[0])
        colstats = bool(colstats)
        kw = dict(ksize=self.kernel_size, stride=self.stride, pad=pad, upsample=upsample, out_hw=out_hw, residual=residual,
                  rowvec=rowvec, flags=flags, n_out=w.shape[0], colstats=colstats)
        if upsample and norm is None and x2 is None and self.kernel_size == 3 and self.stride == 1:
            kw["w_up4"] = self.packed_up4()
        in_scsh = None
        if norm is not None:
            st1, st2 = ops.gn_stats_of(x), ops.gn_stats_of(x2)
            if (FUSE_GN and st1 is not None and (x2 is None or st2 is not None)
                    and ops.conv2d(x, w, b, x2=x2, probe_in_scsh=True, **kw)):
                B = x.shape[0]
                in_scsh = ops.gn_finalize(st1, x.shape[-1], st2, x2.shape[-1] if x2 is not None else 0, norm.weight,
                                          norm.bias, B, x.shape[1] * x.shape[2], norm.num_groups, norm.eps)
                count_flops("fused_gn_convs", 1)
            else:
                x, x2 = norm(x, x2=x2, silu=norm_silu), None
        out = ops.conv2d(x, w, b, x2=x2, in_scsh=in_scsh, in_act=1 if norm_silu else 0, **kw)
        if ops.WORK_COUNTER is not None:
            k = self.kernel_size
            kind = "conv3x3" if k == 3 else "conv1x1"
            npix_out = out.shape[0] * out.shape[1] * out.shape[2]
            count_flops(kind, 2.0 * npix_out * self.out_channels * self.in_channels * k * k)
            nbytes = 2.0 * x.numel() / x.shape[-1] * self.in_channels + 2.0 * self.weight.numel() \
                + npix_out * self.out_channels * (4.0 if (flags & L.GEMM_OUT_F32) else 2.0)
            if residual is not None:
                nbytes += 2.0 * npix_out * self.out_channels
            count_flops(kind + "_bytes", nbytes)
            Hh, Ww = x.shape[1], x.shape[2]
            if (k == 3 and self.stride == 1 and not upsample and tuple(pad) == (1, 1)
                    and self.out_channels > 64 and not (flags & L.GEMM_OUT_F32)
                    and ((Ww % 32 == 0 and Hh % 8 == 0) or (Ww % 16 == 0 and Hh % 16 == 0) or (Ww == 8 and Hh == 8))):
                count_flops("conv3p_bytes", nbytes)
                count_flops("conv3p_launches", 1.0)
        return out


class GroupNorm(nn.Module):
    def __init__(self, num_groups: int, num_channels: int, eps: float = 1e-5):
        super().__init__()
        self.num_groups, self.num_channels, self.eps = num_groups, num_channels, eps
        self.weight = nn.Parameter(torch.ones(num_channels))
        self.bias = nn.Parameter(torch.zeros(num_channels))

    def forward(self, x, x2=None, silu: bool = False):
        if GN_EPI:
            st1, st2 = ops.gn_stats_of(x), ops.gn_stats_of(x2)
            C1, C2 = x.shape[-1], (x2.shape[-1] if x2 is not None else 0)
            HW = x.numel() // (x.shape[0] * C1)
            if (st1 is not None and (x2 is None or st2 is not None)
                    and (ops.gn_strip_ok(x.shape[0], HW, C1, C2, self.num_groups)
                         or ((C1 + C2) % 64 == 0 and (C1 + C2) // self.num_groups <= 128))):
                count_flops("gn_from_epilogue_stats", 1)
                return ops.group_norm_from_stats(x, st1, self.weight, self.bias, self.num_groups, self.eps, silu, x2=x2, st2=st2)
        return ops.group_norm(x, self.weight, self.bias, self.num_groups, self.eps, silu, x2=x2)


class LayerNorm(nn.Module):
    def __init__(self, dim: int, eps: float = 1e-5):
        super().__init__()
        self.dim, self.eps = dim, eps
        self.weight = nn.Parameter(torch.ones(dim))
        self.bias = nn.Parameter(torch.zeros(dim))

    def forward(self, x):
        return ops.layer_norm(x, self.weight, self.bias, self.eps)


def fuse_rows(*weights: torch.Tensor) -> torch.Tensor:
    return packing.pack_linear(torch.cat(list(weights), dim=0))


GEMM_GEGLU = L.GEMM_GEGLU
GEMM_OUT_F32 = L.GEMM_OUT_F32
GEMM_RELU = L.GEMM_RELU
GEMM_TRANSPOSED = L.GEMM_TRANSPOSED
GEMM_SILU_OUT = L.GEMM_SILU_OUT
```

Measured before the change: 10.76 images/s.

## Emit LayerNorm row statistics from producer epilogues for bf16 LN-folded GEMMs

Adds a bf16 path where producer kernels (plain lean GEMM epilogue and fused temporal-attention kernel) write per-row partial sum/sum-of-squares. The downstream LayerNorm-folded GEMMs (GEGLU, optionally QKV) then read these statistics instead of accumulating them inside their main MFMA loop. The aim is to remove the per-k-step dot-product row-stat work from the LN-folded kernels. In exchange, the producers do extra epilogue reductions and stores, and the planner gains new gating conditions. Only the GEGLU consumer is enabled by default for 640/1280 widths; the QKV producer flag stays off.

```diff
diff --git a/udifftext_amd/csrc/gemm.hip b/udifftext_amd/csrc/gemm.hip
--- a/udifftext_amd/csrc/gemm.hip
+++ b/udifftext_amd/csrc/gemm.hip
@@ -763,8 +763,12 @@
     if (d->q8_fixed_col > 0 && (!emit || geglu || d->q8_fixed_col % 32 != 0 || !(d->q8_fixed_mul > 0.f))) return false;
     if ((reinterpret_cast<uintptr_t>(d->q8_out) | reinterpret_cast<uintptr_t>(d->colscale)) & 15) return false;
   } else if (d->rowstat_out || d->rowstat_in) {
-    return false;
-  }
+    if (d->rowstat_in && (!ln || d->rowstat_out || d->rowstat_in_parts <= 0 || (reinterpret_cast<uintptr_t>(d->rowstat_in) & 7))) return false;
+    if (d->rowstat_out && (ln || geglu || want_stats || conv1 || d->N % 64 != 0 || (mode > 0 && mode != 1) ||
+                           (reinterpret_cast<uintptr_t>(d->rowstat_out) & 7))) return false;
+    if (mode == 0 || mode == 7) return false;
+  }
+  const bool bf16_rowstat = !mx8 && !emit && (d->rowstat_out || d->rowstat_in);
   const int KT = mx8 ? 128 : BK;
   if (d->N <= 64 || d->N % 8 != 0 || d->K % KT != 0 || (!conv1 && d->lda % 8 != 0) || (d->ldo % 8 != 0 && d->out)) return false;
   if (d->residual && d->ldr % 8 != 0) return false;
@@ -777,7 +781,7 @@
        reinterpret_cast<uintptr_t>(d->rowvec) | reinterpret_cast<uintptr_t>(d->ln_colsum)) & 15) return false;
   if (d->rowvec && ((d->ld_rowvec > 0 ? d->ld_rowvec : d->N) % 4 != 0)) return false;
   if (mode > 0 && mode != 1 && mode != 6 && mode != 7) return false;
-  if (!mx8 && (!emit || (ln && !geglu && !d->rowstat_out)) && (mode == 7 || (mode < 0 && rowres_on()))) {
+  if (!mx8 && !bf16_rowstat && (!emit || (ln && !geglu && !d->rowstat_out)) && (mode == 7 || (mode < 0 && rowres_on()))) {
     const bool emit_fits = !emit || ((d->q8_fixed_col <= 0 || d->q8_fixed_col % 64 == 0) && (long long)d->M * d->ld_q8 < (1LL << 31) &&
                                      (long long)d->M * (d->out ? d->ldo : 0) * 2 < (1LL << 31) && (long long)((d->N + 127) / 128) * d->M * 4 < (1LL << 31));
     if (ln && !want_stats && d->K == 320 && d->N % 64 == 0 && !d->residual && !d->rowvec && !conv1 && emit_fits &&
@@ -804,6 +808,7 @@
   if (!geglu && d->N % 160 == 0 && d->N % 128 != 0 && t.cfg == 1) t.cfg = 5;
   if (mode <= 0 && d->N >= 768 && (long long)((d->M + 255) / 256) * ((d->N + 255) / 256) >= 2LL * device_cus() &&
       (d->cu_share <= 1 || lean256_under_lanes())) t.cfg = 6;
+  if (bf16_rowstat && t.cfg != 1 && !(t.cfg == 6 && !d->rowstat_out)) return false;
   }
   t.stats_rows = 0;
   if (want_stats) {
@@ -1050,6 +1055,10 @@
 extern "C" int32_t udt_gemm_rowstat_parts(const udt_gemm_desc* d) {
   if (!d || d->M <= 0 || d->N <= 0 || d->K <= 0) return 0;
   udt_gemm_desc t = *d;
+  if (!d->q8_out && d->rowstat_out) {
+    LeanPlan lb;
+    return (lean_plan(d, lb, false) && lb.cfg == 1) ? (d->N + 63) / 64 : 0;
+  }
   alignas(16) static const uint64_t probe_dst[2] = {0, 0};
   if (!t.q8_out) { t.q8_out = const_cast<uint64_t*>(probe_dst); t.q8_scale = const_cast<uint64_t*>(probe_dst); if (t.ld_q8 <= 0) t.ld_q8 = (t.N + 15) / 16 * 16; }
   LeanPlan lt;
diff --git a/udifftext_amd/csrc/lean.h b/udifftext_amd/csrc/lean.h
--- a/udifftext_amd/csrc/lean.h
+++ b/udifftext_amd/csrc/lean.h
@@ -16,6 +16,12 @@
   return __builtin_amdgcn_fdot2_f32_bf16(__builtin_bit_cast(bf2_t, a), __builtin_bit_cast(bf2_t, b), c, false);
 }
 
+#if defined(UDT_MEASURE) && defined(LG_NO_LOOP_ROWSTATS)
+constexpr bool LOOP_ROWSTATS = false;
+#else
+constexpr bool LOOP_ROWSTATS = true;
+#endif
+
 template <int CPR, int RPI>
 UDT_DEVINL void wave_colstats(char* wl, int lane, const float (&cs)[8], const float (&cq)[8], float* dst, bool col_ok) {
 #pragma unroll
@@ -50,8 +56,11 @@
 }
 
 template <int NW, int WGM, int WGN, int TM, int TN, int NST, bool GEGLU, bool LN, int TMB = TM, bool STATS = false, bool FP8 = false,
-          bool EMIT = false>
+          bool EMIT = false, bool STATIN = (LN && FP8), bool ROWSTAT = false>
 __global__ void __launch_bounds__(NW * 64, 2) lgemm_kernel(const LParams p) {
+  static_assert(!STATIN || LN, "row statistics are read by the LayerNorm-folded instances");
+  static_assert(!(LN && FP8) || STATIN, "e4m3 fragments have no packed dot: the statistics come from the producer");
+  static_assert(!ROWSTAT || (!GEGLU && !LN && !FP8 && !EMIT && !STATS), "row statistics without the MX8 twin: the plain bf16 epilogue");
   static_assert(!STATS || (!GEGLU && !LN), "statistics-emitting epilogue: plain linears / 1x1 convolutions");
   static_assert(!FP8 || NST == 2, "the fp8 loop is written for the two-stage ring");
   static_assert(!EMIT || (TN * 4) % 4 == 0, "a 32-column block = 4 lanes of the row layout");
@@ -168,7 +177,11 @@
   float rs[TM], rq[TM];
 #pragma unroll
   for (int i = 0; i < TM; ++i) rs[i] = rq[i] = 0.f;
-  if constexpr (LN && FP8) {
+  if constexpr (LN && !STATIN && !LOOP_ROWSTATS) {
+#pragma unroll
+    for (int i = 0; i < TM; ++i) rq[i] = 8.f * (float)p.K;
+  }
+  if constexpr (LN && STATIN) {
     if (WGN == 1 || wn == 0) {
 #pragma unroll
       for (int tm = 0; tm < TM; ++tm) {
@@ -248,7 +261,7 @@
       for (int tm = 0; tm < TM; ++tm)
 #pragma unroll
         for (int tn = 0; tn < TN; ++tn) acc[tm][tn] = mfma32(wf[ks][tn], xf[ks][tm], acc[tm][tn]);
-      if constexpr (LN) {
+      if constexpr (LN && !STATIN && LOOP_ROWSTATS) {
         if (wn == 0) {
 #pragma unroll
           for (int tm = 0; tm < TM; ++tm) {
@@ -576,6 +589,25 @@
               f32x2 st2 = {ps, pq};
               reinterpret_cast<f32x2*>(p.rowstat_out)[(long long)((n0 + col0) / WCOLS) * p.M + m] = st2;
             }
+          }
+        }
+        if constexpr (ROWSTAT) {
+          static_assert(CPR == 8 || CPR == 16, "row statistics: 64- or 128-column wave blocks");
+          const u32x4 rb = {pack_bf16x2(o[0], o[1]), pack_bf16x2(o[2], o[3]), pack_bf16x2(o[4], o[5]), pack_bf16x2(o[6], o[7])};
+          float ps = 0.f, pq = 0.f;
+#pragma unroll
+          for (int j = 0; j < 4; ++j) {
+            const float a = bf16_lo(rb[j]), bb = bf16_hi(rb[j]);
+            ps += a; pq += a * a;
+            ps += bb; pq += bb * bb;
+          }
+          ps = dpp_add<0xB1>(ps); pq = dpp_add<0xB1>(pq);
+          ps = dpp_add<0x4E>(ps); pq = dpp_add<0x4E>(pq);
+          ps = dpp_add<0x141>(ps); pq = dpp_add<0x141>(pq);
+          if constexpr (CPR == 16) { ps = dpp_add<0x140>(ps); pq = dpp_add<0x140>(pq); }
+          if (ok && c8 == 0) {
+            f32x2 st2 = {ps, pq};
+            reinterpret_cast<f32x2*>(p.rowstat_out)[(long long)((n0 + col0) / WCOLS) * p.M + m] = st2;
           }
         }
         if (ok) {
diff --git a/udifftext_amd/csrc/lean.hip b/udifftext_amd/csrc/lean.hip
--- a/udifftext_amd/csrc/lean.hip
+++ b/udifftext_amd/csrc/lean.hip
@@ -12,11 +12,13 @@
 
 template <int NW, int WGM, int WGN, int TM, int TN, int NST, int TMB = TM>
 hipError_t launch_lean(const lg::LParams& lp, int smem, int G, bool geglu, bool ln, hipStream_t s) {
-  static AttrOnce once[5];
+  static AttrOnce once[8];
   const void* fn;
   const bool stats = lp.colstats != nullptr;
+  const bool statin = lp.rowstat_in != nullptr, rowstat = lp.rowstat_out != nullptr;
   if constexpr (NW == 4 && NST == 2) {
     if (stats) {
+      if (statin || rowstat) return hipErrorInvalidValue;
       fn = (const void*)lg::lgemm_kernel<NW, WGM, WGN, TM, TN, NST, false, false, TMB, true>;
       hipError_t e = once[4].ensure(fn, smem);
       if (e != hipSuccess) return e;
@@ -25,6 +27,28 @@
     }
   }
   if (stats) return hipErrorInvalidValue;
+  if constexpr (TN == 2 && WGN > 1) {
+    if (statin) {
+      if (!ln || rowstat) return hipErrorInvalidValue;
+      fn = geglu ? (const void*)lg::lgemm_kernel<NW, WGM, WGN, TM, TN, NST, true, true, TMB, false, false, false, true>
+                 : (const void*)lg::lgemm_kernel<NW, WGM, WGN, TM, TN, NST, false, true, TMB, false, false, false, true>;
+      hipError_t e = once[geglu ? 6 : 5].ensure(fn, smem);
+      if (e != hipSuccess) return e;
+      void* args[] = {const_cast<lg::LParams*>(&lp)};
+      return hipLaunchKernel(fn, dim3(G), dim3(NW * 64), args, smem, s);
+    }
+    if constexpr (NW == 4) {
+      if (rowstat) {
+        if (ln || geglu) return hipErrorInvalidValue;
+        fn = (const void*)lg::lgemm_kernel<NW, WGM, WGN, TM, TN, NST, false, false, TMB, false, false, false, false, true>;
+        hipError_t e = once[7].ensure(fn, smem);
+        if (e != hipSuccess) return e;
+        void* args[] = {const_cast<lg::LParams*>(&lp)};
+        return hipLaunchKernel(fn, dim3(G), dim3(NW * 64), args, smem, s);
+      }
+    }
+  }
+  if (statin || rowstat) return hipErrorInvalidValue;
   if constexpr (TN == 2) {
     fn = geglu ? (ln ? (const void*)lg::lgemm_kernel<NW, WGM, WGN, TM, TN, NST, true, true, TMB> : (const void*)lg::lgemm_kernel<NW, WGM, WGN, TM, TN, NST, true, false, TMB>)
                : (ln ? (const void*)lg::lgemm_kernel<NW, WGM, WGN, TM, TN, NST, false, true, TMB> : (const void*)lg::lgemm_kernel<NW, WGM, WGN, TM, TN, NST, false, false, TMB>);
diff --git a/udifftext_amd/csrc/tattn.hip b/udifftext_amd/csrc/tattn.hip
--- a/udifftext_amd/csrc/tattn.hip
+++ b/udifftext_amd/csrc/tattn.hip
@@ -30,7 +30,7 @@
   return z;
 }
 
-template <int TT, int NKT, int NKS, bool Q8 = false>
+template <int TT, int NKT, int NKS, bool Q8 = false, bool RS = false>
 __global__ void __launch_bounds__(TA_THREADS) tattn_fused_kernel(const TattnParams p) {
   extern __shared__ __attribute__((aligned(16))) char smem[];
   constexpr int C = NKT * 64, hp = NKS * 16;
@@ -125,8 +125,23 @@
           }
         }
       }
-    }
-    if constexpr (Q8) q8_row_stats();
+      if constexpr (RS) {
+        float ps = 0.f, pq = 0.f;
+#pragma unroll
+        for (int j = 0; j < 4; ++j) {
+          const float a = bf16_lo(o[j]), bb = bf16_hi(o[j]);
+          ps += a; pq += a * a;
+          ps += bb; pq += bb * bb;
+        }
+        ps = dpp_add<0xB1>(ps); pq = dpp_add<0xB1>(pq);
+        ps = dpp_add<0x4E>(ps); pq = dpp_add<0x4E>(pq);
+        if (ok && (ch & 3) == 0) {
+          f32x2 st2 = {ps, pq};
+          *reinterpret_cast<f32x2*>(rst + ((size_t)row * (C >> 5) + (ch >> 2)) * 2) = st2;
+        }
+      }
+    }
+    if constexpr (Q8 || RS) q8_row_stats();
     return;
   }
 
@@ -247,6 +262,7 @@
       const bool rok = tok0 + row < p.M;
       const int swz = (row >> 1) & 7;
       float v[16];
+      float rps = 0.f, rpq = 0.f;
 #pragma unroll
       for (int r4 = 0; r4 < 4; ++r4) {
         const int c = ct * 32 + 8 * r4 + 4 * hi;
@@ -259,6 +275,22 @@
         v[r4 * 4 + 3] = acc[r4 * 4 + 3] + bv[3] + bf16_hi(xr[1]);
         u32x2 pk = {pack_bf16x2(v[r4 * 4 + 0], v[r4 * 4 + 1]), pack_bf16x2(v[r4 * 4 + 2], v[r4 * 4 + 3])};
         if (rok) *reinterpret_cast<u32x2*>(og + (long long)row * C + c) = pk;
+        if constexpr (RS) {
+#pragma unroll
+          for (int j = 0; j < 2; ++j) {
+            const float a = bf16_lo(pk[j]), bb = bf16_hi(pk[j]);
+            rps += a; rpq += a * a;
+            rps += bb; rpq += bb * bb;
+          }
+        }
+      }
+      if constexpr (RS) {
+        rps = xor32_sum(rps);
+        rpq = xor32_sum(rpq);
+        if (rok && hi == 0) {
+          f32x2 st2 = {rps, rpq};
+          *reinterpret_cast<f32x2*>(rst + ((size_t)row * (C >> 5) + ct) * 2) = st2;
+        }
       }
       if constexpr (Q8) {
         uint32_t q[4], sb;
@@ -281,7 +313,7 @@
       }
     }
   }
-  if constexpr (Q8) q8_row_stats();
+  if constexpr (Q8 || RS) q8_row_stats();
 }
 
 __global__ void __launch_bounds__(256) tattn_prepare_a_kernel(const uint16_t* __restrict__ kv, int ldkv, const uint16_t* __restrict__ wq,
@@ -386,6 +418,8 @@
   if (n_tok % TT != 0) return UDT_ERR_BAD_SHAPE;
   const bool q8 = q8_out != nullptr;
   if (q8 && (!q8_scale || !rowstat_out || C % 128 != 0)) return UDT_ERR_BAD_ARG;
+  const bool rs = !q8 && rowstat_out != nullptr;
+  if (rs && (q8_scale || (C != 640 && C != 1280))) return UDT_ERR_BAD_ARG;
   TattnParams p;
   p.x = reinterpret_cast<const uint16_t*>(x); p.out = reinterpret_cast<uint16_t*>(out);
   p.A = reinterpret_cast<const uint16_t*>(A); p.sc = sc; p.BmT = reinterpret_cast<const uint16_t*>(BmT); p.bias = bias;
@@ -393,7 +427,7 @@
   if (!p.zero) return UDT_ERR_HIP;
   p.M = B * n_tok; p.C = C; p.hp = udt_tattn_hp(heads); p.n_tok = n_tok; p.zero_samples = zero_samples; p.eps = eps;
   p.q8_out = reinterpret_cast<uint8_t*>(q8_out); p.q8_scale = reinterpret_cast<uint32_t*>(q8_scale); p.rowstat_out = rowstat_out;
-  const size_t smem = (size_t)TT * C * 2 + (size_t)TT * 2 * sizeof(float) + (size_t)TT * (p.hp * 2 + 16) + (q8 ? (size_t)TT * (C / 32) * 8 : 0);
+  const size_t smem = (size_t)TT * C * 2 + (size_t)TT * 2 * sizeof(float) + (size_t)TT * (p.hp * 2 + 16) + ((q8 || rs) ? (size_t)TT * (C / 32) * 8 : 0);
   hipStream_t s = reinterpret_cast<hipStream_t>(stream);
   UdtProfScope prof(3, s);
   if (prof.rec) {
@@ -401,12 +435,15 @@
     snprintf(tag, sizeof(tag), "tattn_fused%s B=%d n=%d C=%d zero=%d", q8 ? "+q8" : "", B, n_tok, C, zero_samples);
     udt_prof_tag(prof.rec, tag);
   }
-  static bool attr_done[5] = {false, false, false, false, false};
+  static bool attr_done[7] = {false, false, false, false, false, false, false};
   const unsigned grid = (unsigned)(p.M / TT);
   p.nsplit = tattn_nsplit(p.M, TT);
   const void* fn = nullptr;
   int which = -1;
-  if (C == 320 && p.hp == 96 && !q8) { fn = reinterpret_cast<const void*>(tattn_fused_kernel<64, 5, 6>); which = 0; }
+  if (rs && C == 640 && p.hp == 160) { fn = reinterpret_cast<const void*>(tattn_fused_kernel<32, 10, 10, false, true>); which = 5; }
+  else if (rs && C == 1280 && p.hp == 320) { fn = reinterpret_cast<const void*>(tattn_fused_kernel<32, 20, 20, false, true>); which = 6; }
+  else if (rs) return UDT_ERR_BAD_SHAPE;
+  else if (C == 320 && p.hp == 96 && !q8) { fn = reinterpret_cast<const void*>(tattn_fused_kernel<64, 5, 6>); which = 0; }
   else if (C == 640 && p.hp == 160) { fn = q8 ? reinterpret_cast<const void*>(tattn_fused_kernel<32, 10, 10, true>) : reinterpret_cast<const void*>(tattn_fused_kernel<32, 10, 10>); which = q8 ? 3 : 1; }
   else if (C == 1280 && p.hp == 320) { fn = q8 ? reinterpret_cast<const void*>(tattn_fused_kernel<32, 20, 20, true>) : reinterpret_cast<const void*>(tattn_fused_kernel<32, 20, 20>); which = q8 ? 4 : 2; }
   else return UDT_ERR_BAD_SHAPE;
@@ -438,6 +475,6 @@
 extern "C" int udt_tattn_fused_q8(const void* x, void* out, const void* A, const float* sc, const void* BmT, const float* bias,
                                   int32_t B, int32_t n_tok, int32_t C, int32_t heads, int32_t zero_samples, float eps, void* q8_out,
                                   void* q8_scale, float* rowstat_out, void* stream) {
-  if (!q8_out) return UDT_ERR_BAD_ARG;
+  if (!q8_out && (!rowstat_out || q8_scale)) return UDT_ERR_BAD_ARG;
   return tattn_launch(x, out, A, sc, BmT, bias, B, n_tok, C, heads, zero_samples, eps, q8_out, q8_scale, rowstat_out, stream);
 }
diff --git a/udifftext_amd/ops.py b/udifftext_amd/ops.py
--- a/udifftext_amd/ops.py
+++ b/udifftext_amd/ops.py
@@ -149,6 +149,11 @@
 
 def mx8_of(t: Optional[torch.Tensor]) -> Optional[Mx8Act]:
     return getattr(t, "mx8", None) if t is not None else None
+
+
+def _drop_ln_stats(out: Optional[torch.Tensor]) -> None:
+    if out is not None and getattr(out, "ln_stats", None) is not None:
+        del out.ln_stats
 
 
 def _mx8_alloc(M: int, cols: int, device) -> Mx8Act:
@@ -176,7 +181,7 @@
 def linear(x: torch.Tensor, w: torch.Tensor, bias: Optional[torch.Tensor] = None, *, out: Optional[torch.Tensor] = None,
            residual: Optional[torch.Tensor] = None, rowvec: Optional[torch.Tensor] = None, rows_per_batch: int = 0,
            flags: int = 0, alpha: float = 1.0, n_out: Optional[int] = None, colstats: bool = False,
-           emit_q8: bool = False, emit_rowstats: bool = False) -> torch.Tensor:
+           emit_q8: bool = False, emit_rowstats: bool = False, emit_ln_stats: bool = False) -> torch.Tensor:
     _bf16(x); _bf16(w)
     K = x.shape[-1]
     x2 = x.reshape(-1, K) if x.is_contiguous() else x
@@ -202,7 +207,19 @@
     q8 = None
     if emit_q8 and not (flags & (L.GEMM_OUT_F32 | L.GEMM_TRANSPOSED | L.GEMM_GEGLU)) and d.colstats is None and rowvec is None:
         q8 = _attach_q8(d, M, n_cols, x.device, emit_rowstats)
+    _drop_ln_stats(out)
+    ln_st = None
+    if emit_ln_stats and q8 is None and flags == 0 and d.colstats is None and out.dtype == torch.bfloat16:
+        d.rowstat_out = out.data_ptr()
+        parts = L.load().udt_gemm_rowstat_parts(C.byref(d))
+        if parts > 0:
+            ln_st = torch.empty((parts, M, 2), dtype=torch.float32, device=x.device)
+            d.rowstat_out = ln_st.data_ptr()
+        else:
+            d.rowstat_out = None
     run_gemm(d, x.device)
+    if ln_st is not None:
+        out.ln_stats = ln_st
     if getattr(out, "mx8", None) is not None:
         del out.mx8
     if q8 is not None:
@@ -265,7 +282,7 @@
 def ln_linear(x: torch.Tensor, w_folded: torch.Tensor, c: torch.Tensor, s: torch.Tensor, *, eps: float = 1e-5,
               out: Optional[torch.Tensor] = None, residual: Optional[torch.Tensor] = None, flags: int = 0,
               n_out: Optional[int] = None, emit_q8: bool = False, want_bf16: bool = True, q8_fixed: Optional[tuple] = None,
-              q8_or_none: bool = False):
+              q8_or_none: bool = False, rowstats: Optional[torch.Tensor] = None):
     _bf16(x); _bf16(w_folded)
     K = x.shape[-1]
     x2 = x.reshape(-1, K) if x.is_contiguous() else x
@@ -287,12 +304,19 @@
                 return None
             raise L.UdtError(f"udt_ln_gemm_fwd has no MX8-emitting plan for M={M} N={N} K={K}")
     lib = L.load()
+    if rowstats is not None and q8 is None:
+        assert rowstats.dtype == torch.float32 and rowstats.is_contiguous() and rowstats.shape[1:] == (M, 2)
+        d.rowstat_in, d.rowstat_in_parts = rowstats.data_ptr(), rowstats.shape[0]
+    _drop_ln_stats(out)
     need = lib.udt_gemm_workspace_bytes(C.byref(d))
     ws_ptr, ws_bytes = None, 0
     if need:
         ws = _ws(need, x.device)
         ws_ptr, ws_bytes = ws.data_ptr(), ws.numel()
     rc = lib.udt_ln_gemm_fwd(C.byref(d), ws_ptr, ws_bytes, _stream())
+    if rc in (-1, -2) and d.rowstat_in:
+        d.rowstat_in, d.rowstat_in_parts = None, 0
+        rc = lib.udt_ln_gemm_fwd(C.byref(d), ws_ptr, ws_bytes, _stream())
     if rc in (-1, -2) and x.is_cuda:
         raise L.UdtError(f"udt_ln_gemm_fwd declined M={M} N={N} K={K} flags={flags:#x} (status {rc}): the LayerNorm-folded GEMM "
                          "needs the lean kernel family (UDT_LEAN / udt_debug_set('lean') != 0) and 16-byte aligned operands; "
@@ -551,7 +575,7 @@
 
 
 def tattn_fused(x: torch.Tensor, tables: Optional[TattnTables], bias: torch.Tensor, heads: int, zero_samples: int, eps: float,
-                out: Optional[torch.Tensor] = None, emit_q8: bool = False) -> torch.Tensor:
+                out: Optional[torch.Tensor] = None, emit_q8: bool = False, emit_ln_stats: bool = False) -> torch.Tensor:
     _bf16(x)
     assert x.is_contiguous()
     B, N, Cc = x.shape
@@ -562,6 +586,7 @@
         assert tables.A.is_contiguous() and tables.sc.is_contiguous() and tables.BmT.is_contiguous() and tables.A.shape[0] == B
     if getattr(out, "mx8", None) is not None:
         del out.mx8
+    _drop_ln_stats(out)
     parts = L.load().udt_tattn_rowstat_parts(B, N, Cc) if emit_q8 else 0
     if parts > 0:
         q = _mx8_alloc(B * N, Cc, x.device)
@@ -570,6 +595,14 @@
                                             _ptr(tables.BmT) if tables else None, _ptr(bias), B, N, Cc, heads, zero_samples, eps,
                                             _ptr(q.data), _ptr(q.scale), _ptr(q.stats), _stream()), "udt_tattn_fused_q8")
         out.mx8 = q
+        return out
+    parts = L.load().udt_tattn_rowstat_parts(B, N, Cc) if emit_ln_stats else 0
+    if parts > 0:
+        st = torch.empty((parts, B * N, 2), dtype=torch.float32, device=x.device)
+        L.check(L.load().udt_tattn_fused_q8(_ptr(x), _ptr(out), _ptr(tables.A) if tables else None, _ptr(tables.sc) if tables else None,
+                                            _ptr(tables.BmT) if tables else None, _ptr(bias), B, N, Cc, heads, zero_samples, eps,
+                                            None, None, _ptr(st), _stream()), "udt_tattn_fused_q8 (bf16 + row statistics)")
+        out.ln_stats = st
         return out
     L.check(L.load().udt_tattn_fused(_ptr(x), _ptr(out), _ptr(tables.A) if tables else None, _ptr(tables.sc) if tables else None,
                                      _ptr(tables.BmT) if tables else None, _ptr(bias), B, N, Cc, heads, zero_samples, eps, _stream()),
diff --git a/udifftext_amd/sgm/modules/attention.py b/udifftext_amd/sgm/modules/attention.py
--- a/udifftext_amd/sgm/modules/attention.py
+++ b/udifftext_amd/sgm/modules/attention.py
@@ -16,6 +16,9 @@
 
 FF_PROJ = os.environ.get("UDT_FF_PROJ", "1") != "0"
 
+LN_ROWSTATS_QKV = False
+LN_ROWSTATS_GEGLU = True
+
 
 class GEGLU(H._Packed):
     def __init__(self, dim_in: int, dim_out: int):
@@ -37,13 +40,13 @@
     def _pack_ln_mx8(self, gamma, beta):
         return packing.pack_ln_linear_mx8(self.proj.weight, self.proj.bias, gamma, beta, geglu=True)
 
-    def forward(self, x, ln=None, x8=None):
+    def forward(self, x, ln=None, x8=None, rowstats=None):
         if ln is not None and x8 is not None:
             wq, cs, c, s = self.packed_ln_mx8(ln)
             return ops.linear_mx8(x8, wq, cs, ln_c=c, ln_s=s, eps=ln.eps, flags=H.GEMM_GEGLU, emit_q8=True, want_bf16=False)
         if ln is not None:
             wf, c, s = self.packed_ln(ln)
-            return ops.ln_linear(x, wf, c, s, eps=ln.eps, flags=H.GEMM_GEGLU)
+            return ops.ln_linear(x, wf, c, s, eps=ln.eps, flags=H.GEMM_GEGLU, rowstats=rowstats)
         w, b = self.packed()
         return ops.linear(x, w, b, flags=H.GEMM_GEGLU)
 
@@ -56,8 +59,8 @@
         inner = int(dim * mult)
         self.net = nn.Sequential(GEGLU(dim, inner), nn.Identity(), H.Linear(inner, dim_out or dim))
 
-    def forward(self, x, residual=None, ln=None, x8=None, emit_q8: bool = False, emit_rowstats: bool = False):
-        h = self.net[0](x, ln=ln, x8=x8)
+    def forward(self, x, residual=None, ln=None, x8=None, emit_q8: bool = False, emit_rowstats: bool = False, rowstats=None):
+        h = self.net[0](x, ln=ln, x8=x8, rowstats=rowstats)
         if isinstance(h, ops.Mx8Act):
             return self.net[2](None, residual=residual, x8=h, emit_q8=emit_q8, emit_rowstats=emit_rowstats)
         return self.net[2](h, residual=residual)
@@ -167,7 +170,7 @@
         self.v_mul8 = H.v_fixed_mul(wv, pk[2][2 * inner:3 * inner])
         return pk
 
-    def forward(self, x, context=None, mask=None, residual=None, ln=None, x8=None):
+    def forward(self, x, context=None, mask=None, residual=None, ln=None, x8=None, rowstats=None):
         if context is not None or mask is not None:
             raise NotImplementedError("attn1 is pure self-attention on this path (reference attention.py:251-252)")
         inner = self.heads * self.dim_head
@@ -194,7 +197,7 @@
             if qkv8 is not None:
                 o = ops.attention_mx8(qkv8, B, self.heads, scale, self.v_mul)
             else:
-                qkv = ops.ln_linear(x2, wf, c, sv, eps=ln.eps).reshape(B, N, 3 * inner)
+                qkv = ops.ln_linear(x2, wf, c, sv, eps=ln.eps, rowstats=rowstats).reshape(B, N, 3 * inner)
         else:
             qkv = ops.linear(x2, self.packed()[0]).reshape(B, N, 3 * inner)
         if o is None:
@@ -225,12 +228,14 @@
                 t_fused=None, x8=None, emit_rowstats: bool = False, defer_ff_out: bool = False, hw=None):
         fold = H.LN_GEMM
         mx = fold and x8 is not None and H.mx8_width(x.shape[-1])
-        x = self.attn1(x, residual=x, ln=self.norm1, x8=x8 if mx else None) if fold else self.attn1(self.norm1(x), residual=x)
+        hand = fold and not mx and LN_ROWSTATS_GEGLU and x.shape[-1] in (640, 1280)
+        x = (self.attn1(x, residual=x, ln=self.norm1, x8=x8 if mx else None, rowstats=None if mx else H.ln_stats_of(x))
+             if fold else self.attn1(self.norm1(x), residual=x))
         if hasattr(self, "t_attn"):
             n0 = 0 if emit_map else min(int(zero_ctx_rows), x.shape[0])
             if t_fused is not None and not emit_map and n0 < x.shape[0] and self.fused_tattn_ok(x.shape[1]):
                 _, bo = self.t_attn.to_out[0].packed()
-                x = ops.tattn_fused(x, t_fused, bo, self.t_attn.heads, n0, self.t_norm.eps, emit_q8=mx)
+                x = ops.tattn_fused(x, t_fused, bo, self.t_attn.heads, n0, self.t_norm.eps, emit_q8=mx, emit_ln_stats=hand)
             elif n0 > 0 and t_kv is not None:
                 y = torch.empty_like(x)
                 self.t_attn.zero_context_residual(x[:n0], y[:n0])
@@ -242,11 +247,13 @@
                 x = self.t_attn(self.t_norm(x), context=t_context, kv=t_kv, residual=x, emit_map=emit_map, hw=hw)
         B, N, C = x.shape
         x2 = x.reshape(B * N, C)
+        st3 = H.ln_stats_of(x) if hand else None
         if fold:
             x8b = ops.mx8_of(x) if mx else None
             if defer_ff_out and x8b is None:
-                return self.ff.net[0](x2, ln=self.norm3), x2
-            out = self.ff(x2, residual=x2, ln=self.norm3, x8=x8b, emit_q8=x8b is not None, emit_rowstats=emit_rowstats)
+                return self.ff.net[0](x2, ln=self.norm3, rowstats=st3), x2
+            out = self.ff(x2, residual=x2, ln=self.norm3, x8=x8b, emit_q8=x8b is not None, emit_rowstats=emit_rowstats,
+                          rowstats=st3 if x8b is None else None)
             return H.carry_mx8(out.reshape(B, N, C), out)
         return self.ff(self.norm3(x2), residual=x2).reshape(B, N, C)
 
@@ -287,8 +294,11 @@
         B, Hh, Ww, C = x.shape
         N = Hh * Ww
         mx = H.mx8_width(self.proj_in.out_features)
-        t2 = self.proj_in(self.norm(x).reshape(B * N, C), emit_q8=mx, emit_rowstats=mx)
+        hand = H.LN_GEMM and not mx and LN_ROWSTATS_QKV and self.proj_in.out_features in (640, 1280)
+        t2 = self.proj_in(self.norm(x).reshape(B * N, C), emit_q8=mx, emit_rowstats=mx, emit_ln_stats=hand)
         t = H.carry_mx8(t2.reshape(B, N, -1), t2)
+        if H.ln_stats_of(t2) is not None:
+            t.ln_stats = t2.ln_stats
         nb = len(self.transformer_blocks)
         defer = FF_PROJ and H.LN_GEMM and not mx
         for i, blk in enumerate(self.transformer_blocks):
diff --git a/udifftext_amd/sgm/modules/hipnn.py b/udifftext_amd/sgm/modules/hipnn.py
--- a/udifftext_amd/sgm/modules/hipnn.py
+++ b/udifftext_amd/sgm/modules/hipnn.py
@@ -60,6 +60,10 @@
     if q is not None:
         dst.mx8 = q
     return dst
+
+
+def ln_stats_of(t: Optional[torch.Tensor]) -> Optional[torch.Tensor]:
+    return getattr(t, "ln_stats", None) if t is not None else None
 
 
 def _init_uniform_(p: torch.Tensor, fan_in: int) -> None:
@@ -157,7 +161,7 @@
         return wq, cs, packing.pad_bias(self.bias)
 
     def forward(self, x, residual=None, flags: int = 0, out=None, rowvec=None, rows_per_batch: int = 0,
-                colstats: bool = False, x8=None, emit_q8: bool = False, emit_rowstats: bool = False):
+                colstats: bool = False, x8=None, emit_q8: bool = False, emit_rowstats: bool = False, emit_ln_stats: bool = False):
         if x8 is not None:
             wq, cs, b = self.packed_fp8()
             M = x8.data.shape[0]
@@ -171,7 +175,7 @@
             rpb = rows_per_batch if rows_per_batch > 0 else x.shape[0]
             colstats = want_stats(x.shape[0] // rpb, rpb, w.shape[0])
         return ops.linear(x, w, b, residual=residual, flags=flags, out=out, rowvec=rowvec, rows_per_batch=rows_per_batch,
-                          colstats=bool(colstats), emit_q8=emit_q8, emit_rowstats=emit_rowstats)
+                          colstats=bool(colstats), emit_q8=emit_q8, emit_rowstats=emit_rowstats, emit_ln_stats=emit_ln_stats)
 
 
 class Conv2d(_Packed):
```

Result: no change. 10.85 images/s (median of 6 runs) (+0.8%).
